# kennychenfs/KataCoffee

Hardware: AMD Instinct MI355X
Metric: self-play training rows/sec + MCTS playouts/sec, 5x5 Coffee b6c96 @600 visits (higher is better)
Workload: dtype fp16

## Files before the change

### include/katacoffee.h

```cpp
#ifndef KATACOFFEE_H
#define KATACOFFEE_H

#include <stdint.h>

#ifdef __cplusplus
extern "C" {
#endif

#define COFFEE_OK 0
#define COFFEE_EINVAL (-1)
#define COFFEE_EHIP (-2)
#define COFFEE_EIO (-3)
#define COFFEE_EINTERNAL (-4)

#define COFFEE_NUM_SPATIAL 15
#define COFFEE_NUM_GLOBAL_TARGETS 64

const char* coffee_last_error(void);
int coffee_abi_version(void);

int coffee_device_count(int* count);
int coffee_set_device(int device);
int coffee_device_compute_units(int device, int* cus);
int coffee_malloc(void** dev_ptr, uint64_t bytes);
int coffee_free(void* dev_ptr);
int coffee_memcpy(void* dst, const void* src, uint64_t bytes, int kind);
int coffee_synchronize(void);


int coffee_rules_batch(int x, int y, int win_len, int n, const uint8_t* cells, const int8_t* last_cell,
                       const int8_t* last_dir, const uint8_t* pla, uint8_t* legal, uint8_t* has_legal, void* stream);

int coffee_play_batch(int x, int y, int win_len, int n, const uint8_t* cells, const int8_t* last_cell,
                      const int8_t* last_dir, const uint8_t* pla, const int32_t* move, uint8_t* out_cells,
                      uint8_t* finished, uint8_t* winner, int32_t* max_run, uint64_t* pos_hash,
                      uint64_t* state_hash, void* stream);


int coffee_encode_batch(int x, int y, int win_len, int n, const uint8_t* cells, const int8_t* hist_cell,
                        const int8_t* hist_dir, const uint8_t* pla, const int32_t* sym, uint64_t* packed,
                        float* planes, void* stream);


typedef struct coffee_nn coffee_nn;

int coffee_model_write_random(const char* arch, uint64_t seed, const char* path );
int coffee_model_flops(const char* path, int area, double* flops);

int coffee_nn_create(const char* model_path, int x, int y, int win_len, coffee_nn** out);
#define COFFEE_NN_DEFAULT 0
#define COFFEE_NN_ACCURATE 1
#define COFFEE_NN_FAST_LAYERED 2
#define COFFEE_NN_CORRECTED 3
#define COFFEE_NN_ACCURATE_NB2 4
#define COFFEE_NN_FAST 5
int coffee_nn_create2(const char* model_path, int x, int y, int win_len, int precision, coffee_nn** out);
int coffee_nn_is_fused(coffee_nn* h, int* fused);
int coffee_nn_precision(coffee_nn* h, int* precision, float* calib_err);
int coffee_nn_forward(coffee_nn* h, int n, const uint64_t* in, float* out, void* stream);
int coffee_nn_forward2(coffee_nn* h, int n, const uint64_t* in, const int32_t* sym, float* out, void* stream);
int coffee_nn_destroy(coffee_nn* h);

int coffee_fake_net(int x, int y, int win_len, int n, const uint64_t* in, float* out, void* stream);


typedef struct coffee_search_params {
  int32_t max_visits;
  float cpuct_exploration, cpuct_exploration_log, cpuct_exploration_base;
  float fpu_reduction_max, root_fpu_reduction_max, fpu_loss_prop, root_fpu_loss_prop;
  int32_t fpu_parent_weight_by_visited_policy;
  float fpu_parent_weight_by_visited_policy_pow;
  float value_weight_exponent;
  int32_t root_noise_enabled;
  float root_dirichlet_noise_total_concentration, root_dirichlet_noise_weight;
  float root_policy_temperature, root_policy_temperature_early;
  float root_desired_per_child_visits_coeff;
  int32_t root_num_symmetries_to_sample;
  float chosen_move_temperature, chosen_move_temperature_early, chosen_move_temperature_halflife;
  float chosen_move_subtract, chosen_move_prune;
  int32_t use_lcb_for_selection;
  float lcb_stdevs, min_visit_prop_for_lcb;
  float subtree_value_bias_factor, subtree_value_bias_weight_exponent, subtree_value_bias_free_prop;
  int32_t use_graph_search;
  float cheap_search_prob;
  int32_t cheap_search_visits;
  float cheap_search_target_weight;
  int32_t reduce_visits;
  float reduce_visits_threshold;
  int32_t reduce_visits_threshold_lookback;
  int32_t reduced_visits_min;
  float reduced_visits_weight;
  float policy_surprise_data_weight;
  float value_surprise_data_weight;
  int32_t init_games_with_policy;
  float policy_init_area_prop;
  float policy_init_area_temperature;
  float early_fork_game_prob;
  float early_fork_game_expected_move_prop;
  float fork_game_prob;
  int32_t fork_game_min_choices;
  int32_t early_fork_game_max_choices;
  int32_t fork_game_max_choices;
  float side_position_prob;
  int32_t record_tree_positions;
  int32_t record_tree_threshold;
  float record_tree_target_weight;
} coffee_search_params;

void coffee_search_params_default(coffee_search_params* p);

typedef struct coffee_selfplay_config {
  int32_t x, y, win_len;
  int32_t num_games;
  int32_t node_cap;
  int32_t row_capacity;
  uint64_t seed;
  int32_t slot_base;
  int32_t use_fake_net;
  int32_t commit_interval;
  const char* model_path;
  coffee_search_params search;
  int32_t nn_cache_log2;
  int32_t nn_batch_cap;
  int32_t nn_precision;
  int32_t start_stagger;
  int32_t engines_per_device;
} coffee_selfplay_config;

typedef struct coffee_selfplay coffee_selfplay;

typedef struct coffee_selfplay_stats {
  uint64_t rounds;
  uint64_t playouts;
  uint64_t nn_evals;
  uint64_t moves;
  uint64_t games_finished;
  uint64_t rows_written;
  uint64_t rows_pending;
  uint64_t rows_dropped;
  uint64_t games_dropped;
  uint64_t errors;
  uint64_t tree_levels;
  uint64_t tree_children;
  uint64_t errors_node_pool;
  uint64_t errors_edge_pool;
  uint64_t edge_pool_peak;
  uint64_t edge_pool_cap;
  uint64_t nn_precision;
  uint64_t nn_audits;
  uint64_t nn_audit_switches;
  double nn_audit_max_diff;
} coffee_selfplay_stats;

int coffee_selfplay_create(const coffee_selfplay_config* cfg, coffee_selfplay** out);
int coffee_selfplay_step(coffee_selfplay* h, int rounds, void* stream);
int coffee_selfplay_sync(coffee_selfplay* h);
int coffee_selfplay_stats_get(coffee_selfplay* h, coffee_selfplay_stats* out);

int coffee_selfplay_drain_rows(coffee_selfplay* h, int max_rows, uint8_t* bin, float* glob, int16_t* pol,
                               float* gtgt, int8_t* value, int32_t* meta, int* n_out);
int coffee_selfplay_drain_games(coffee_selfplay* h, int max_games, int32_t* header, uint8_t* moves, int* n_out);
#define COFFEE_STAGE_DISCARD_GAMES 1
int coffee_selfplay_stage_rows(coffee_selfplay* h, void* dst, int max_rows, uint64_t* count, int flags);
int coffee_selfplay_row_capacity(coffee_selfplay* h, int* rows);
int coffee_row_bytes(int x, int y, int* bytes);
int coffee_selfplay_stream(coffee_selfplay* h, void** stream);
int coffee_selfplay_set_model(coffee_selfplay* h, const char* model_path);
int coffee_selfplay_set_model_bytes(coffee_selfplay* h, const void* data, uint64_t bytes);
int coffee_selfplay_destroy(coffee_selfplay* h);

int coffee_write_npz(const char* path, int n, int x, int y, const uint8_t* bin, const float* glob,
                     const int16_t* pol, const float* gtgt, const int8_t* value);

int coffee_selfplay_game_info(coffee_selfplay* h, int slot, int64_t* info);
int coffee_selfplay_game_tree(coffee_selfplay* h, int slot, int max_nodes, uint32_t* nodes, uint32_t* edges,
                              int* n_nodes);
int coffee_selfplay_root_policy(coffee_selfplay* h, int slot, float* out);

int coffee_debug_cdf_table(int x, int y, int win_len, float* out );
int coffee_debug_zobrist(int x, int y, int win_len, uint64_t* board, uint64_t* board2, uint64_t* player,
                         uint64_t* init, uint64_t* game_over);

int coffee_selfplay_enable_timing(coffee_selfplay* h, int enable);
int coffee_selfplay_kernel_time(coffee_selfplay* h, int which, double* ms, uint64_t* launches);
int coffee_selfplay_timed_nn_evals(coffee_selfplay* h, uint64_t* evals);

#ifdef __cplusplus
}
#endif

#endif
```

### katacoffee_amd/__init__.py

```python
import ctypes
import os
import subprocess

import numpy as np

HERE = os.path.dirname(os.path.abspath(__file__))
LIB_PATH = os.path.join(HERE, "libkatacoffee.so")
CSRC = os.path.join(HERE, "csrc")

NUM_SPATIAL = 15
COFFEE_OK = 0
PRECISIONS = {"default": 0, "accurate": 1, "fast-layered": 2, "corrected": 3, "accurate-nb2": 4, "fast": 5}
PRECISION_NAMES = {v: k for k, v in PRECISIONS.items()}

_lib = None

c_p = ctypes.c_void_p
c_i = ctypes.c_int
c_u64 = ctypes.c_uint64


class CoffeeError(RuntimeError):
    pass


class SearchParams(ctypes.Structure):
    _fields_ = [
        ("max_visits", ctypes.c_int32),
        ("cpuct_exploration", ctypes.c_float), ("cpuct_exploration_log", ctypes.c_float),
        ("cpuct_exploration_base", ctypes.c_float),
        ("fpu_reduction_max", ctypes.c_float), ("root_fpu_reduction_max", ctypes.c_float),
        ("fpu_loss_prop", ctypes.c_float), ("root_fpu_loss_prop", ctypes.c_float),
        ("fpu_parent_weight_by_visited_policy", ctypes.c_int32),
        ("fpu_parent_weight_by_visited_policy_pow", ctypes.c_float),
        ("value_weight_exponent", ctypes.c_float),
        ("root_noise_enabled", ctypes.c_int32),
        ("root_dirichlet_noise_total_concentration", ctypes.c_float),
        ("root_dirichlet_noise_weight", ctypes.c_float),
        ("root_policy_temperature", ctypes.c_float), ("root_policy_temperature_early", ctypes.c_float),
        ("root_desired_per_child_visits_coeff", ctypes.c_float),
        ("root_num_symmetries_to_sample", ctypes.c_int32),
        ("chosen_move_temperature", ctypes.c_float), ("chosen_move_temperature_early", ctypes.c_float),
        ("chosen_move_temperature_halflife", ctypes.c_float),
        ("chosen_move_subtract", ctypes.c_float), ("chosen_move_prune", ctypes.c_float),
        ("use_lcb_for_selection", ctypes.c_int32),
        ("lcb_stdevs", ctypes.c_float), ("min_visit_prop_for_lcb", ctypes.c_float),
        ("subtree_value_bias_factor", ctypes.c_float), ("subtree_value_bias_weight_exponent", ctypes.c_float),
        ("subtree_value_bias_free_prop", ctypes.c_float),
        ("use_graph_search", ctypes.c_int32),
        ("cheap_search_prob", ctypes.c_float), ("cheap_search_visits", ctypes.c_int32),
        ("cheap_search_target_weight", ctypes.c_float), ("reduce_visits", ctypes.c_int32),
        ("reduce_visits_threshold", ctypes.c_float), ("reduce_visits_threshold_lookback", ctypes.c_int32),
        ("reduced_visits_min", ctypes.c_int32), ("reduced_visits_weight", ctypes.c_float),
        ("policy_surprise_data_weight", ctypes.c_float), ("value_surprise_data_weight", ctypes.c_float),
        ("init_games_with_policy", ctypes.c_int32), ("policy_init_area_prop", ctypes.c_float),
        ("policy_init_area_temperature", ctypes.c_float),
        ("early_fork_game_prob", ctypes.c_float), ("early_fork_game_expected_move_prop", ctypes.c_float),
        ("fork_game_prob", ctypes.c_float), ("fork_game_min_choices", ctypes.c_int32),
        ("early_fork_game_max_choices", ctypes.c_int32), ("fork_game_max_choices", ctypes.c_int32),
        ("side_position_prob", ctypes.c_float),
        ("record_tree_positions", ctypes.c_int32), ("record_tree_threshold", ctypes.c_int32),
        ("record_tree_target_weight", ctypes.c_float),
    ]


class SelfplayConfig(ctypes.Structure):
    _fields_ = [
        ("x", ctypes.c_int32), ("y", ctypes.c_int32), ("win_len", ctypes.c_int32),
        ("num_games", ctypes.c_int32), ("node_cap", ctypes.c_int32), ("row_capacity", ctypes.c_int32),
        ("seed", ctypes.c_uint64), ("slot_base", ctypes.c_int32), ("use_fake_net", ctypes.c_int32),
        ("commit_interval", ctypes.c_int32),
        ("model_path", ctypes.c_char_p),
        ("search", SearchParams),
        ("nn_cache_log2", ctypes.c_int32),
        ("nn_batch_cap", ctypes.c_int32),
        ("nn_precision", ctypes.c_int32),
        ("start_stagger", ctypes.c_int32),
        ("engines_per_device", ctypes.c_int32),
    ]


class SelfplayStats(ctypes.Structure):
    _fields_ = [(n, ctypes.c_uint64) for n in
                ["rounds", "playouts", "nn_evals", "moves", "games_finished", "rows_written", "rows_pending",
                 "rows_dropped", "games_dropped", "errors", "tree_levels", "tree_children", "errors_node_pool",
                 "errors_edge_pool", "edge_pool_peak", "edge_pool_cap", "nn_precision", "nn_audits",
                 "nn_audit_switches"]] + [("nn_audit_max_diff", ctypes.c_double)]


EXPORTS = [
    "coffee_last_error", "coffee_abi_version", "coffee_device_count", "coffee_set_device", "coffee_device_compute_units", "coffee_malloc",
    "coffee_free", "coffee_memcpy", "coffee_synchronize", "coffee_rules_batch", "coffee_play_batch",
    "coffee_encode_batch", "coffee_model_write_random", "coffee_model_flops", "coffee_nn_create",
    "coffee_nn_forward", "coffee_nn_forward2", "coffee_nn_destroy", "coffee_nn_create2", "coffee_nn_is_fused", "coffee_nn_precision", "coffee_fake_net", "coffee_search_params_default",
    "coffee_selfplay_create", "coffee_selfplay_step", "coffee_selfplay_sync", "coffee_selfplay_stats_get",
    "coffee_selfplay_drain_rows", "coffee_selfplay_drain_games", "coffee_selfplay_set_model",
    "coffee_selfplay_stage_rows", "coffee_selfplay_row_capacity", "coffee_row_bytes", "coffee_selfplay_stream",
    "coffee_selfplay_set_model_bytes",
    "coffee_selfplay_destroy", "coffee_selfplay_game_info",
    "coffee_selfplay_game_tree", "coffee_selfplay_root_policy", "coffee_debug_cdf_table", "coffee_debug_zobrist",
    "coffee_selfplay_enable_timing", "coffee_selfplay_kernel_time", "coffee_selfplay_timed_nn_evals",
    "coffee_write_npz",
]


def build(jobs=8):
    subprocess.run(["make", "-s", "-j%d" % jobs, "-C", CSRC], check=True)


def lib():
    global _lib
    if _lib is None:
        if not os.path.exists(LIB_PATH):
            raise CoffeeError("libkatacoffee.so not built (run katacoffee_amd.build()); no CPU fallback exists")
        try:
            import torch
        except ImportError:
            pass
        L = ctypes.CDLL(os.environ.get("KATACOFFEE_LIB", LIB_PATH))
        L.coffee_last_error.restype = ctypes.c_char_p
        L.coffee_model_write_random.argtypes = [ctypes.c_char_p, c_u64, ctypes.c_char_p]
        L.coffee_model_flops.argtypes = [ctypes.c_char_p, c_i, c_p]
        L.coffee_nn_create.argtypes = [ctypes.c_char_p, c_i, c_i, c_i, c_p]
        L.coffee_nn_create2.argtypes = [ctypes.c_char_p, c_i, c_i, c_i, c_i, c_p]
        L.coffee_nn_is_fused.argtypes = [c_p, c_p]
        if hasattr(L, "coffee_nn_precision"):
            L.coffee_nn_precision.argtypes = [c_p, c_p, c_p]
        L.coffee_nn_forward.argtypes = [c_p, c_i, c_p, c_p, c_p]
        L.coffee_nn_forward2.argtypes = [c_p, c_i, c_p, c_p, c_p, c_p]
        L.coffee_nn_destroy.argtypes = [c_p]
        L.coffee_fake_net.argtypes = [c_i, c_i, c_i, c_i, c_p, c_p, c_p]
        L.coffee_rules_batch.argtypes = [c_i, c_i, c_i, c_i] + [c_p] * 7
        L.coffee_play_batch.argtypes = [c_i, c_i, c_i, c_i] + [c_p] * 12
        L.coffee_encode_batch.argtypes = [c_i, c_i, c_i, c_i] + [c_p] * 8
        L.coffee_search_params_default.argtypes = [c_p]
        L.coffee_search_params_default.restype = None
        L.coffee_selfplay_create.argtypes = [c_p, c_p]
        L.coffee_selfplay_step.argtypes = [c_p, c_i, c_p]
        L.coffee_selfplay_sync.argtypes = [c_p]
        L.coffee_selfplay_stats_get.argtypes = [c_p, c_p]
        L.coffee_selfplay_drain_rows.argtypes = [c_p, c_i] + [c_p] * 7
        L.coffee_selfplay_drain_games.argtypes = [c_p, c_i, c_p, c_p, c_p]
        L.coffee_selfplay_stage_rows.argtypes = [c_p, c_p, c_i, c_p, c_i]
        L.coffee_selfplay_row_capacity.argtypes = [c_p, c_p]
        L.coffee_row_bytes.argtypes = [c_i, c_i, c_p]
        L.coffee_selfplay_stream.argtypes = [c_p, c_p]
        L.coffee_selfplay_set_model.argtypes = [c_p, ctypes.c_char_p]
        L.coffee_selfplay_set_model_bytes.argtypes = [c_p, c_p, c_u64]
        L.coffee_selfplay_destroy.argtypes = [c_p]
        L.coffee_selfplay_game_info.argtypes = [c_p, c_i, c_p]
        L.coffee_selfplay_game_tree.argtypes = [c_p, c_i, c_i, c_p, c_p, c_p]
        L.coffee_selfplay_root_policy.argtypes = [c_p, c_i, c_p]
        L.coffee_selfplay_enable_timing.argtypes = [c_p, c_i]
        L.coffee_selfplay_kernel_time.argtypes = [c_p, c_i, c_p, c_p]
        L.coffee_selfplay_timed_nn_evals.argtypes = [c_p, c_p]
        L.coffee_debug_cdf_table.argtypes = [c_i, c_i, c_i, c_p]
        L.coffee_debug_zobrist.argtypes = [c_i, c_i, c_i] + [c_p] * 5
        L.coffee_write_npz.argtypes = [ctypes.c_char_p, c_i, c_i, c_i] + [c_p] * 5
        _lib = L
    return _lib


def check(rc):
    if rc != COFFEE_OK:
        msg = lib().coffee_last_error()
        raise CoffeeError("libkatacoffee error %d: %s" % (rc, msg.decode() if msg else ""))


def _ptr(a):
    return ctypes.c_void_p(a.ctypes.data)


def default_search_params(**over):
    p = SearchParams()
    lib().coffee_search_params_default(ctypes.byref(p))
    for k, v in over.items():
        setattr(p, k, v)
    return p



def _torch_cuda():
    import torch
    if not torch.cuda.is_available():
        raise CoffeeError("no GPU visible: the HIP path is the only implementation")
    return torch


def _dev(torch, a, dtype=None):
    a = np.ascontiguousarray(a if dtype is None else np.asarray(a, dtype=dtype))
    return torch.from_numpy(a).to("cuda")


def _dp(t):
    return ctypes.c_void_p(t.data_ptr())


def _sync(torch):
    torch.cuda.synchronize()


def rules_batch(X, Y, W, cells, last_cell, last_dir, pla):
    torch = _torch_cuda()
    n = len(pla)
    A = X * Y
    dc, dl, dd, dp_ = (_dev(torch, cells, np.uint8), _dev(torch, last_cell, np.int8), _dev(torch, last_dir, np.int8),
                       _dev(torch, pla, np.uint8))
    legal = torch.zeros((n, 4 * A), dtype=torch.uint8, device="cuda")
    has = torch.zeros(n, dtype=torch.uint8, device="cuda")
    _sync(torch)
    check(lib().coffee_rules_batch(X, Y, W, n, _dp(dc), _dp(dl), _dp(dd), _dp(dp_), _dp(legal), _dp(has), None))
    _sync(torch)
    return legal.cpu().numpy(), has.cpu().numpy()


def play_batch(X, Y, W, cells, last_cell, last_dir, pla, move):
    torch = _torch_cuda()
    n = len(pla)
    A = X * Y
    ins = [_dev(torch, cells, np.uint8), _dev(torch, last_cell, np.int8), _dev(torch, last_dir, np.int8),
           _dev(torch, pla, np.uint8), _dev(torch, move, np.int32)]
    out_cells = torch.zeros((n, A), dtype=torch.uint8, device="cuda")
    fin = torch.zeros(n, dtype=torch.uint8, device="cuda")
    win = torch.zeros(n, dtype=torch.uint8, device="cuda")
    mr = torch.zeros(n, dtype=torch.int32, device="cuda")
    ph = torch.zeros((n, 2), dtype=torch.int64, device="cuda")
    sh = torch.zeros((n, 2), dtype=torch.int64, device="cuda")
    _sync(torch)
    check(lib().coffee_play_batch(X, Y, W, n, *[_dp(t) for t in ins], _dp(out_cells), _dp(fin), _dp(win), _dp(mr),
                                  _dp(ph), _dp(sh), None))
    _sync(torch)
    u = lambda t: t.cpu().numpy().view(np.uint64)
    return (out_cells.cpu().numpy(), fin.cpu().numpy(), win.cpu().numpy(), mr.cpu().numpy(), u(ph), u(sh))


def encode_batch(X, Y, W, cells, hist_cell, hist_dir, pla, sym, want_planes=True):
    torch = _torch_cuda()
    n = len(pla)
    A = X * Y
    words = (NUM_SPATIAL * A + 63) // 64
    ins = [_dev(torch, cells, np.uint8), _dev(torch, hist_cell, np.int8), _dev(torch, hist_dir, np.int8),
           _dev(torch, pla, np.uint8), _dev(torch, sym, np.int32)]
    packed = torch.zeros((n, words), dtype=torch.int64, device="cuda")
    planes = torch.zeros((n, NUM_SPATIAL, A), dtype=torch.float32, device="cuda") if want_planes else None
    _sync(torch)
    check(lib().coffee_encode_batch(X, Y, W, n, *[_dp(t) for t in ins], _dp(packed),
                                    _dp(planes) if planes is not None else None, None))
    _sync(torch)
    pk = packed.cpu().numpy().view(np.uint64)
    return pk, (planes.cpu().numpy() if planes is not None else None)


def write_random_model(arch, seed, path):
    check(lib().coffee_model_write_random(arch.encode(), seed, path.encode()))


def model_flops(path, area):
    f = ctypes.c_double()
    check(lib().coffee_model_flops(path.encode(), area, ctypes.byref(f)))
    return f.value


class Network:

    def __init__(self, model_path, X, Y, W, precision="default"):
        self.X, self.Y, self.W = X, Y, W
        self.h = ctypes.c_void_p()
        check(lib().coffee_nn_create2(model_path.encode(), X, Y, W, PRECISIONS[precision], ctypes.byref(self.h)))

    @property
    def fused(self):
        f = ctypes.c_int()
        check(lib().coffee_nn_is_fused(self.h, ctypes.byref(f)))
        return bool(f.value)

    @property
    def precision(self):
        p, e = ctypes.c_int(), ctypes.c_float()
        check(lib().coffee_nn_precision(self.h, ctypes.byref(p), ctypes.byref(e)))
        return PRECISION_NAMES[p.value], float(e.value)

    def forward_device(self, n, packed_dev, out_dev, stream=None):
        check(lib().coffee_nn_forward(self.h, n, _dp(packed_dev), _dp(out_dev), stream))

    def forward(self, packed):
        torch = _torch_cuda()
        n = packed.shape[0]
        P = 4 * self.X * self.Y
        din = _dev(torch, np.ascontiguousarray(packed).view(np.int64))
        out = torch.zeros((n, P + 4), dtype=torch.float32, device="cuda")
        _sync(torch)
        self.forward_device(n, din, out)
        _sync(torch)
        return out.cpu().numpy()

    def forward_canonical(self, packed, sym):
        torch = _torch_cuda()
        n = packed.shape[0]
        P = 4 * self.X * self.Y
        din = _dev(torch, np.ascontiguousarray(packed).view(np.int64))
        dsym = _dev(torch, sym, np.int32)
        out = torch.zeros((n, P + 4), dtype=torch.float32, device="cuda")
        _sync(torch)
        check(lib().coffee_nn_forward2(self.h, n, _dp(din), _dp(dsym), _dp(out), None))
        _sync(torch)
        return out.cpu().numpy()

    def close(self):
        if self.h:
            lib().coffee_nn_destroy(self.h)
            self.h = ctypes.c_void_p()

    def __del__(self):
        try:
            self.close()
        except Exception:
            pass


def fake_net(X, Y, W, packed):
    torch = _torch_cuda()
    n = packed.shape[0]
    P = 4 * X * Y
    din = _dev(torch, np.ascontiguousarray(packed).view(np.int64))
    out = torch.zeros((n, P + 4), dtype=torch.float32, device="cuda")
    _sync(torch)
    check(lib().coffee_fake_net(X, Y, W, n, _dp(din), _dp(out), None))
    _sync(torch)
    return out.cpu().numpy()


def cdf_table(X=5, Y=5, W=4):
    out = np.zeros(2000, np.float32)
    check(lib().coffee_debug_cdf_table(X, Y, W, _ptr(out)))
    return out


def row_bytes(X, Y):
    b = ctypes.c_int()
    check(lib().coffee_row_bytes(X, Y, ctypes.byref(b)))
    return b.value


def write_npz(path, rows, X, Y):
    n = len(rows["globalInputNC"])
    arrs = [np.ascontiguousarray(rows[k], dtype=t) for k, t in
            [("binaryInputNCHWPacked", np.uint8), ("globalInputNC", np.float32), ("policyTargetsNCMove", np.int16),
             ("globalTargetsNC", np.float32), ("valueTargetsNCHW", np.int8)]]
    check(lib().coffee_write_npz(path.encode(), n, X, Y, *[_ptr(a) for a in arrs]))


def zobrist_tables(X, Y, W):
    A = X * Y
    out = dict(board=np.zeros((A, 3, 2), np.uint64), board2=np.zeros((A, 4, 2), np.uint64),
               player=np.zeros((3, 2), np.uint64), init=np.zeros(2, np.uint64), game_over=np.zeros(2, np.uint64))
    check(lib().coffee_debug_zobrist(X, Y, W, *[_ptr(out[k]) for k in ["board", "board2", "player", "init",
                                                                          "game_over"]]))
    return out


class Selfplay:

    def __init__(self, X=5, Y=5, W=4, num_games=4096, max_visits=600, seed=1, slot_base=0, model_path=None,
                 node_cap=0, row_capacity=0, commit_interval=0, nn_cache_log2=0, nn_batch_cap=0, nn_precision="default",
                 start_stagger=0, engines_per_device=0, **search_over):
        _torch_cuda()
        self.X, self.Y, self.W = X, Y, W
        self.A, self.P = X * Y, 4 * X * Y
        self.num_games = num_games
        cfg = SelfplayConfig()
        cfg.x, cfg.y, cfg.win_len = X, Y, W
        cfg.num_games = num_games
        cfg.node_cap = node_cap
        cfg.row_capacity = row_capacity
        cfg.seed = seed
        cfg.slot_base = slot_base
        cfg.use_fake_net = 1 if model_path is None else 0
        cfg.commit_interval = commit_interval
        cfg.nn_cache_log2 = nn_cache_log2
        cfg.nn_batch_cap = nn_batch_cap
        cfg.nn_precision = PRECISIONS[nn_precision]
        cfg.start_stagger = start_stagger
        cfg.engines_per_device = engines_per_device
        self._model = model_path.encode() if model_path else None
        cfg.model_path = self._model
        cfg.search = default_search_params(max_visits=max_visits, **search_over)
        self.cfg = cfg
        self.h = ctypes.c_void_p()
        check(lib().coffee_selfplay_create(ctypes.byref(cfg), ctypes.byref(self.h)))

    def step(self, rounds, stream=None):
        check(lib().coffee_selfplay_step(self.h, rounds, stream))

    def sync(self):
        check(lib().coffee_selfplay_sync(self.h))

    def stats(self):
        s = SelfplayStats()
        check(lib().coffee_selfplay_stats_get(self.h, ctypes.byref(s)))
        return {k: getattr(s, k) for k, _ in SelfplayStats._fields_}

    def drain_rows(self, max_rows=1 << 30):
        st = self.stats()
        n = min(max_rows, st["rows_pending"])
        A, P, pb = self.A, self.P, (self.A + 7) // 8
        rows = {
            "binaryInputNCHWPacked": np.zeros((n, NUM_SPATIAL, pb), np.uint8),
            "globalInputNC": np.zeros((n, 1), np.float32),
            "policyTargetsNCMove": np.zeros((n, 2, P), np.int16),
            "globalTargetsNC": np.zeros((n, 64), np.float32),
            "valueTargetsNCHW": np.zeros((n, 5, self.Y, self.X), np.int8),
            "meta": np.zeros((n, 4), np.int32),
        }
        got = ctypes.c_int()
        order = ["binaryInputNCHWPacked", "globalInputNC", "policyTargetsNCMove", "globalTargetsNC",
                 "valueTargetsNCHW", "meta"]
        check(lib().coffee_selfplay_drain_rows(self.h, n, *[_ptr(rows[k]) for k in order], ctypes.byref(got)))
        assert got.value == n
        return rows

    def row_capacity(self):
        n = ctypes.c_int()
        check(lib().coffee_selfplay_row_capacity(self.h, ctypes.byref(n)))
        return n.value

    def stream_ptr(self):
        p = ctypes.c_void_p()
        check(lib().coffee_selfplay_stream(self.h, ctypes.byref(p)))
        return p.value

    def stage_rows(self, dst, count, discard_games=True):
        assert dst.is_cuda and dst.dtype.itemsize == 1 and dst.is_contiguous()
        assert dst.dim() == 2 and dst.shape[1] == row_bytes(self.X, self.Y), \
            "dst must be [rows][row_bytes(X, Y)] uint8, got %s" % (tuple(dst.shape),)
        import torch
        assert dst.device.index == torch.cuda.current_device(), "dst must be on the engine's (current) device"
        assert count.is_pinned() and count.dtype.itemsize == 8
        check(lib().coffee_selfplay_stage_rows(self.h, ctypes.c_void_p(dst.data_ptr()), dst.shape[0],
                                               ctypes.c_void_p(count.data_ptr()), 1 if discard_games else 0))

    def drain_games(self, max_games=1 << 20):
        cap = min(max_games, 2 * self.num_games)
        header = np.zeros((cap, 4), np.int32)
        moves = np.zeros((cap, self.A, 2), np.uint8)
        got = ctypes.c_int()
        check(lib().coffee_selfplay_drain_games(self.h, cap, _ptr(header), _ptr(moves), ctypes.byref(got)))
        return header[:got.value], moves[:got.value]

    def set_model(self, model_path):
        self._model = model_path.encode()
        check(lib().coffee_selfplay_set_model(self.h, self._model))

    def set_model_bytes(self, data):
        buf = np.frombuffer(bytes(data), dtype=np.uint8)
        check(lib().coffee_selfplay_set_model_bytes(self.h, _ptr(buf), buf.size))

    def game_info(self, slot):
        info = np.zeros(16, np.int64)
        check(lib().coffee_selfplay_game_info(self.h, slot, _ptr(info)))
        keys = ["phase", "rootK", "liveCount", "rootIdx", "gameNum", "turn", "pla", "finished", "winner",
                "playouts", "nnEvals", "moves", "gamesFinished", "lastCell", "lastDir", "rngCtr"]
        return dict(zip(keys, info.tolist()))

    def game_tree(self, slot, max_nodes=4096):
        nodes = np.zeros((max_nodes, 24), np.uint32)
        edges = np.zeros((max_nodes, self.P, 3), np.uint32)
        n = ctypes.c_int()
        check(lib().coffee_selfplay_game_tree(self.h, slot, max_nodes, _ptr(nodes), _ptr(edges), ctypes.byref(n)))
        return nodes[:n.value], edges[:n.value]

    def root_policy(self, slot):
        out = np.zeros(self.P, np.float32)
        check(lib().coffee_selfplay_root_policy(self.h, slot, _ptr(out)))
        return out

    def enable_timing(self, every=1):
        check(lib().coffee_selfplay_enable_timing(self.h, int(every)))

    def timed_nn_evals(self):
        n = ctypes.c_uint64()
        check(lib().coffee_selfplay_timed_nn_evals(self.h, ctypes.byref(n)))
        return n.value

    def kernel_time(self, which):
        ms = ctypes.c_double()
        n = ctypes.c_uint64()
        check(lib().coffee_selfplay_kernel_time(self.h, which, ctypes.byref(ms), ctypes.byref(n)))
        return ms.value, n.value

    def close(self):
        if self.h:
            lib().coffee_selfplay_destroy(self.h)
            self.h = ctypes.c_void_p()

    def __del__(self):
        try:
            self.close()
        except Exception:
            pass
```

### katacoffee_amd/csrc/capi.cpp

```cpp
#include <cstring>
#include <map>
#include <mutex>
#include <string>
#include <tuple>

#include "../../include/katacoffee.h"
#include "engine.h"
#include "model.h"
#include "npzwrite.h"
#include "selfplay.h"

namespace kc {

namespace {
std::mutex gTablesMu;
std::map<std::tuple<int, int, int, int>, std::pair<DTables*, DTables*>> gTables;
}

static std::pair<DTables*, DTables*> tablesFor(int X, int Y, int W) {
  int dev = 0;
  KC_HIP(hipGetDevice(&dev));
  std::lock_guard<std::mutex> lk(gTablesMu);
  auto key = std::make_tuple(dev, X, Y, W);
  auto it = gTables.find(key);
// ... 163 lines not shown
    ModelHost m = loadModel(model_path);
    (void)deviceTables(x, y, win_len);
    coffee_nn* h = new coffee_nn{nullptr, x, y, win_len};
    try {
      h->eng = new NNEngine(m, x, y, win_len, precision);
    } catch(...) {
      delete h;
      throw;
    }
    *out = h;
  });
}

int coffee_nn_forward(coffee_nn* h, int n, const uint64_t* in, float* out, void* stream) {
  return guarded([&] {
    need(h && h->eng, "NULL handle");
    need(n >= 0, "n must be >= 0");
    need(n == 0 || (in && out), "NULL buffer");
    h->eng->forward(n, in, out, (hipStream_t)stream);
  });
}

int coffee_nn_forward2(coffee_nn* h, int n, const uint64_t* in, const int32_t* sym, float* out, void* stream) {
  return guarded([&] {
    need(h && h->eng, "NULL handle");
    need(n >= 0, "n must be >= 0");
    need(n == 0 || (in && sym && out), "NULL buffer");
    h->eng->forward(n, in, out, (hipStream_t)stream);
    launchCanonicalRows(deviceTables(h->x, h->y, h->w), n, sym, out, (hipStream_t)stream);
  });
}

int coffee_nn_is_fused(coffee_nn* h, int* fused) {
  return guarded([&] {
    need(h && h->eng && fused, "NULL argument");
    *fused = h->eng->fused() ? 1 : 0;
  });
}

int coffee_nn_precision(coffee_nn* h, int* precision, float* calib_err) {
  return guarded([&] {
    need(h && h->eng && precision, "NULL argument");
    *precision = h->eng->precision();
    if(calib_err)
      *calib_err = h->eng->calibrationError();
  });
}

int coffee_nn_destroy(coffee_nn* h) {
  return guarded([&] {
    if(h) {
      delete h->eng;
      delete h;
    }
  });
}

int coffee_fake_net(int x, int y, int win_len, int n, const uint64_t* in, float* out, void* stream) {
  return guarded([&] {
    checkGeom(x, y, win_len);
    need(n >= 0, "n must be >= 0");
    need(n == 0 || (in && out), "NULL buffer");
    launchFakeNet(deviceTables(x, y, win_len), n, in, out, (hipStream_t)stream);
  });
}

void coffee_search_params_default(coffee_search_params* p) {
  if(!p)
    return;
  p->max_visits = 600;
  p->cpuct_exploration = 1.1f;
  p->cpuct_exploration_log = 0.0f;
  p->cpuct_exploration_base = 500.0f;
  p->fpu_reduction_max = 0.2f;
  p->root_fpu_reduction_max = 0.0f;
  p->fpu_loss_prop = 0.0f;
  p->root_fpu_loss_prop = 0.0f;
  p->fpu_parent_weight_by_visited_policy = 1;
  p->fpu_parent_weight_by_visited_policy_pow = 2.0f;
  p->value_weight_exponent = 0.5f;
  p->root_noise_enabled = 1;
  p->root_dirichlet_noise_total_concentration = 10.83f;
  p->root_dirichlet_noise_weight = 0.25f;
  p->root_policy_temperature = 1.1f;
  p->root_policy_temperature_early = 1.25f;
  p->root_desired_per_child_visits_coeff = 2.0f;
  p->root_num_symmetries_to_sample = 4;
  p->chosen_move_temperature = 0.15f;
  p->chosen_move_temperature_early = 0.75f;
  p->chosen_move_temperature_halflife = 19.0f;
  p->chosen_move_subtract = 0.0f;
  p->chosen_move_prune = 1.0f;
  p->use_lcb_for_selection = 1;
  p->lcb_stdevs = 5.0f;
  p->min_visit_prop_for_lcb = 0.15f;
  p->subtree_value_bias_factor = 0.30f;
  p->subtree_value_bias_weight_exponent = 0.8f;
  p->subtree_value_bias_free_prop = 0.8f;
  p->use_graph_search = 1;
  p->cheap_search_prob = 0.0f;
  p->cheap_search_visits = 100;
  p->cheap_search_target_weight = 0.0f;
  p->reduce_visits = 0;
  p->reduce_visits_threshold = 0.9f;
  p->reduce_visits_threshold_lookback = 3;
  p->reduced_visits_min = 100;
  p->reduced_visits_weight = 0.1f;
  p->policy_surprise_data_weight = 0.0f;
  p->value_surprise_data_weight = 0.0f;
  p->init_games_with_policy = 0;
  p->policy_init_area_prop = 0.04f;
  p->policy_init_area_temperature = 1.0f;
  p->early_fork_game_prob = 0.0f;
  p->early_fork_game_expected_move_prop = 0.025f;
  p->fork_game_prob = 0.0f;
  p->fork_game_min_choices = 3;
  p->early_fork_game_max_choices = 12;
  p->fork_game_max_choices = 36;
  p->side_position_prob = 0.0f;
  p->record_tree_positions = 0;
  p->record_tree_threshold = 0;
  p->record_tree_target_weight = 0.0f;
}

struct coffee_selfplay {
  SelfplayEngine* eng;
};

int coffee_selfplay_create(const coffee_selfplay_config* cfg, coffee_selfplay** out) {
  return guarded([&] {
    need(cfg && out, "NULL argument");
    checkGeom(cfg->x, cfg->y, cfg->win_len);
    coffee_selfplay* h = new coffee_selfplay{nullptr};
    try {
      h->eng = new SelfplayEngine(*cfg);
    } catch(...) {
      delete h;
      throw;
    }
    *out = h;
  });
}

int coffee_selfplay_step(coffee_selfplay* h, int rounds, void* stream) {
  return guarded([&] {
    need(h && h->eng, "NULL handle");
    need(rounds >= 0, "rounds must be >= 0");
    h->eng->step(rounds, (hipStream_t)stream);
  });
}

int coffee_selfplay_sync(coffee_selfplay* h) {
  return guarded([&] {
    need(h && h->eng, "NULL handle");
    h->eng->sync();
  });
}

int coffee_selfplay_stats_get(coffee_selfplay* h, coffee_selfplay_stats* out) {
  return guarded([&] {
    need(h && h->eng && out, "NULL argument");
    h->eng->stats(*out);
  });
}

int coffee_selfplay_drain_rows(coffee_selfplay* h, int max_rows, uint8_t* bin, float* glob, int16_t* pol,
                               float* gtgt, int8_t* value, int32_t* meta, int* n_out) {
  return guarded([&] {
    need(h && h->eng && n_out, "NULL argument");
    *n_out = h->eng->drain(max_rows, bin, glob, pol, gtgt, value, meta);
  });
}

int coffee_row_bytes(int x, int y, int* bytes) {
  return guarded([&] {
    need(bytes != nullptr, "NULL argument");
    need(x >= 2 && y >= 2 && x <= MAX_LEN && y <= MAX_LEN, "bad shape");
    *bytes = rowBytes(x * y);
  });
}

int coffee_selfplay_row_capacity(coffee_selfplay* h, int* rows) {
  return guarded([&] {
    need(h && h->eng && rows, "NULL argument");
    *rows = h->eng->dev().rowCap;
  });
}

int coffee_selfplay_stream(coffee_selfplay* h, void** stream) {
  return guarded([&] {
    need(h && h->eng && stream, "NULL argument");
    *stream = (void*)h->eng->stream();
  });
}

int coffee_selfplay_stage_rows(coffee_selfplay* h, void* dst, int max_rows, uint64_t* count, int flags) {
  return guarded([&] {
    need(h && h->eng && dst && count, "NULL argument");
    need((flags & ~COFFEE_STAGE_DISCARD_GAMES) == 0, "unknown flags");
    h->eng->stageRows((uint8_t*)dst, max_rows, (unsigned long long*)count, (flags & COFFEE_STAGE_DISCARD_GAMES) != 0);
  });
}

int coffee_selfplay_drain_games(coffee_selfplay* h, int max_games, int32_t* header, uint8_t* moves, int* n_out) {
  return guarded([&] {
    need(h && h->eng && n_out, "NULL argument");
    need(max_games >= 0, "max_games must be >= 0");
    *n_out = h->eng->drainGames(max_games, header, moves);
  });
}

int coffee_selfplay_set_model(coffee_selfplay* h, const char* model_path) {
  return guarded([&] {
    need(h && h->eng && model_path, "NULL argument");
    h->eng->setModel(model_path);
  });
}

int coffee_selfplay_set_model_bytes(coffee_selfplay* h, const void* data, uint64_t bytes) {
  return guarded([&] {
    need(h && h->eng && data, "NULL argument");
    h->eng->setModelBytes(data, (size_t)bytes);
  });
}

int coffee_selfplay_destroy(coffee_selfplay* h) {
  return guarded([&] {
    if(h) {
      delete h->eng;
      delete h;
    }
  });
}

int coffee_write_npz(const char* path, int n, int x, int y, const uint8_t* bin, const float* glob,
                     const int16_t* pol, const float* gtgt, const int8_t* value) {
  return guarded([&] {
    need(path != nullptr, "NULL path");
    need(n >= 0 && x >= 2 && y >= 2 && x <= MAX_LEN && y <= MAX_LEN, "bad shape");
    writeNpz(path, n, x, y, bin, glob, pol, gtgt, value);
  });
}

int coffee_selfplay_game_info(coffee_selfplay* h, int slot, int64_t* info) {
  return guarded([&] {
    need(h && h->eng && info, "NULL argument");
    h->eng->gameInfo(slot, info);
  });
}

int coffee_selfplay_game_tree(coffee_selfplay* h, int slot, int max_nodes, uint32_t* nodes, uint32_t* edges,
                              int* n_nodes) {
  return guarded([&] {
    need(h && h->eng && n_nodes, "NULL argument");
    *n_nodes = h->eng->gameTree(slot, max_nodes, nodes, edges);
  });
}

int coffee_selfplay_root_policy(coffee_selfplay* h, int slot, float* out) {
  return guarded([&] {
    need(h && h->eng && out, "NULL argument");
    h->eng->rootPolicy(slot, out);
  });
}

int coffee_debug_cdf_table(int x, int y, int win_len, float* out) {
  return guarded([&] {
    need(out != nullptr, "NULL argument");
    checkGeom(x, y, win_len);
    DTables t = buildTables(x, y, win_len);
    memcpy(out, t.cdf, sizeof(float) * CDF_SIZE);
  });
}

int coffee_debug_zobrist(int x, int y, int win_len, uint64_t* board, uint64_t* board2, uint64_t* player,
                         uint64_t* init, uint64_t* game_over) {
  return guarded([&] {
    need(board && board2 && player && init && game_over, "NULL argument");
    checkGeom(x, y, win_len);
    DTables t = buildTables(x, y, win_len);
    memcpy(board, t.zBoard, sizeof(uint64_t) * t.A * 3 * 2);
    memcpy(board2, t.zBoard2, sizeof(uint64_t) * t.A * 4 * 2);
    memcpy(player, t.zPlayer, sizeof(t.zPlayer));
    memcpy(init, t.zInit, sizeof(t.zInit));
    memcpy(game_over, t.zGameOver, sizeof(t.zGameOver));
  });
}

int coffee_selfplay_enable_timing(coffee_selfplay* h, int enable) {
  return guarded([&] {
    need(h && h->eng, "NULL handle");
    need(enable >= 0, "enable must be >= 0");
    h->eng->setTiming(enable);
  });
}

int coffee_selfplay_timed_nn_evals(coffee_selfplay* h, uint64_t* evals) {
  return guarded([&] {
    need(h && h->eng && evals, "NULL argument");
    *evals = h->eng->timedNNEvals();
  });
}

int coffee_selfplay_kernel_time(coffee_selfplay* h, int which, double* ms, uint64_t* launches) {
  return guarded([&] {
    need(h && h->eng && ms && launches, "NULL argument");
    h->eng->kernelTime(which, *ms, *launches);
  });
}

}
```

### katacoffee_amd/csrc/search.h

```cpp
#pragma once
#include "kc_common.h"

namespace kc {

constexpr int MAX_DEPTH = MAX_AREA + 2;
constexpr int INLINE_EDGES = 16;
KC_HD int edgeBlockCap(int k, int P) {
  return (P > 64 && k <= 64) ? 64 - INLINE_EDGES : P - INLINE_EDGES;
}
inline int edgePoolCapFor(int cap, int P) {
  const double perEdge = (32.0 + P) / 65.0 > 48.0 / 17.0 ? (32.0 + P) / 65.0 : 48.0 / 17.0;
  return (int)(perEdge * 1.5 * cap) + 2 * P;
}
enum { ERR_NODE_POOL = 1, ERR_NO_CANDIDATE = 2, ERR_EDGE_POOL = 3 };
constexpr int MAX_LANE_ITEMS = (MAX_P + 63) / 64;

enum LeafKind {
  LEAF_NONE = 0,
  LEAF_NN = 1,
  LEAF_TERMINAL = 2,
  LEAF_CATCHUP = 3,
  LEAF_NOCHILD = 4,
  LEAF_ROOTEVAL = 5,
  LEAF_CACHED = 6,
  LEAF_INIT = 7,
  LEAF_FORK = 8,
  LEAF_SIDE = 9,
  LEAF_PENDING = 10
};

KC_HD uint32_t cacheSlot(uint64_t k0, uint64_t k1, uint32_t mask) {
  const uint64_t h = k0 ^ ((k1 << 29) | (k1 >> 35));
  return (uint32_t)(h ^ (h >> 32)) & mask;
}
enum Phase { PH_ROOTEVAL = 0, PH_SEARCH = 1, PH_COMMIT = 2, PH_INIT = 3, PH_FORK = 4, PH_SIDEEVAL = 5 };

struct SP {
  int maxVisits;
  float cpuct, cpuctLog, cpuctBase;
  float fpuRedMax, rootFpuRedMax, fpuLossProp, rootFpuLossProp;
  int fpuByVisited;
  float fpuByVisitedPow;
  float valueWeightExp;
  int rootNoise;
  float dirConc, dirWeight;
  float rootTemp, rootTempEarly;
  float rootDesiredCoeff;
  int rootSyms;
  float moveTemp, moveTempEarly, moveTempHalflife;
  float moveSubtract, movePrune;
  int useLcb;
  float lcbStdevs, minVisitPropLcb;
  float svbFactor, svbExp, svbFreeProp;
  int useGraph;
  float cheapProb;
  int cheapVisits;
  float cheapWeight;
  int reduceVisits;
  float reduceThreshold;
  int reduceLookback, reducedMin;
  float reducedWeight;
  float policySurpriseWeight, valueSurpriseWeight;
  int initPolicy;
  float initAreaProp, initTemp;
  float earlyForkProb, earlyForkMoveProp, forkProb;
  int forkMinChoices, earlyForkMaxChoices, forkMaxChoices;
  float sideProb;
  int recordTree, recordTreeThreshold;
  float recordTreeWeight;
};

inline SP cheapSearchSP(const SP& p) {
  SP c = p;
  c.rootNoise = 0;
  c.rootTemp = 1.0f;
  c.rootTempEarly = 1.0f;
  c.rootFpuLossProp = p.fpuLossProp;
  c.rootFpuRedMax = p.fpuRedMax;
  c.rootDesiredCoeff = 0.0f;
  c.rootSyms = 1;
  return c;
}

struct Node {
  uint32_t visits;
  float weightSum, weightSqSum, utilityAvg, utilitySqAvg, winLossAvg;
  float nnWin, nnLoss;
  float lastSvbDelta, lastSvbWeight;
  int32_t svbEntry;
  uint16_t numChildren;
  uint8_t nextPla;
  uint8_t flags;
  float nextPrior;
  uint16_t nextPos;
  uint16_t pad0;
  uint32_t edgeBase;
  uint32_t pad1;
};
static_assert(sizeof(Node) == 64, "Node layout");

struct Edge {
  uint32_t child, visits;
  float prior;
  uint32_t move;
};

struct GameRec {
  int32_t slot, gameNum, numMoves, winner;
  uint8_t cell[MAX_AREA], dir[MAX_AREA];
};

struct TurnRec {
  float whiteWin, whiteLoss, rawWhiteWL, rawPolicyEntropy;
  float policySurprise, policyEntropy, searchEntropy;
  uint32_t visits;
  float rootWL;
  float rootNNWin, rootNNLoss;
  float targetWeight;
  int8_t cell, dir;
  uint8_t rows;
  uint8_t gen;
  int8_t pad[4];
};
static_assert(sizeof(TurnRec) == 56, "TurnRec layout");

constexpr int MAX_SIDE = 8;

constexpr int MAX_FORK_CHOICES = 100;
struct ForkRec {
  DBoard board;
  int32_t numChoices, next, best, prefix;
  float bestWinrate;
  int32_t pad;
  uint16_t moves[MAX_FORK_CHOICES];
};

struct FinRec {
  uint64_t rngSeed, rngCtr;
  uint64_t gameHash0, gameHash1;
  unsigned long long rowBase;
  int32_t numMoves, winner, gameNum, pending;
  int32_t numRows, startTurn;
  int32_t gameMode;
  int32_t genStart, genEnd;
  int32_t pad;
};

struct GameDev {
  DBoard root;
  DBoard leaf;
  uint64_t rngSeed, rngCtr;
  uint64_t gameHash0, gameHash1;
  uint64_t playouts, nnEvals, moves, gamesFinished;
  uint64_t treeLevels, treeChildren;
  int32_t phase, rootK;
  uint32_t syms;
  int32_t cSlot;
  float cHitWin, cHitLoss;
  int32_t noNoise;
  int32_t visitLimit;
  float moveWeight;
  int32_t initLeft;
  int32_t startTurn;
  int32_t gameMode;
  int32_t sideCount, sideNext;
  int32_t sideMode;
  int32_t startDelay;
  int32_t startGen;
  int32_t leafKind, leafNode, leafSym, nnSlot;
  int32_t rootIdx, liveCount, freeTop, pathLen;
  int32_t gameNum, numTurns, svbSel, err;
  int32_t edgeSel, edgeTop;
  int32_t edgePeak, pad0;
  float accWin, accLoss, rawWin, rawLoss;
};

template <class T>
KC_HD T* asGlobal(T* p) {
#if defined(__HIP_DEVICE_COMPILE__)
  __attribute__((address_space(1))) T* q = (__attribute__((address_space(1))) T*)p;
  asm volatile("" : "+s"(q));
  return (T*)q;
#else
  return p;
#endif
}
template <class T>
struct DPtr {
  T* p;
  DPtr() = default;
  KC_HD DPtr(T* q) : p(q) {}
  KC_HD operator T*() const { return asGlobal(p); }
  KC_HD T* operator->() const { return asGlobal(p); }
};

struct SearchDev {
  DPtr<const DTables> T;
  SP sp;
  SP spCheap;
  int G, cap, ttCap, svbCap, P, A, inWords, maxTurns;
  int rowCap, slotBase;
  int startStagger;
  DPtr<int32_t> modelGen;
  uint64_t seed;
  DPtr<GameDev> games;
  DPtr<Node> nodes;
  DPtr<Edge> edges;
  DPtr<Edge> edgePool;
  int edgePoolCap;
  DPtr<uint64_t> nodeKey;
  DPtr<float> policy;
  DPtr<uint32_t> freeList;
  DPtr<uint32_t> allocBits;
  DPtr<uint64_t> ttKey;
  DPtr<int32_t> ttNode;
  DPtr<uint64_t> svbKey;
  DPtr<int64_t> svbD;
  DPtr<int64_t> svbW;
  DPtr<float> accPolicy;
  DPtr<float> rawPolicy;
  DPtr<float> rootNoised;
  DPtr<int32_t> pathNode;
  DPtr<int32_t> pathSlot;
  DPtr<TurnRec> turns;
  DPtr<int16_t> turnPol;
  DPtr<uint64_t> nnIn;
  DPtr<float> nnOut;
  DPtr<int32_t> nnNeed;
  DPtr<int32_t> nnIdx;
  DPtr<int32_t> nnCount;
  DPtr<int32_t> nnDefer;
  DPtr<uint32_t> nnBid;
  int nnCap;
  DPtr<int32_t> nnRR;
  DPtr<unsigned long long> nnTimedEvals;
  uint32_t cacheMask;
  int32_t cacheOn;
  DPtr<uint64_t> cKey;
  DPtr<float> cPol;
  DPtr<float> cVal;
  DPtr<uint32_t> cTag;
  DPtr<uint32_t> cClear;
  DPtr<int32_t> pendList;
  DPtr<int32_t> pendCount;
  DPtr<FinRec> fin;
  DPtr<ForkRec> fork;
  DPtr<DBoard> side;
  DPtr<int16_t> sidePol;
  DPtr<int32_t> commitList;
  DPtr<int32_t> commitCount;
  DPtr<uint8_t> rBin;
  DPtr<float> rGlob;
  DPtr<int16_t> rPol;
  DPtr<float> rGt;
  DPtr<int8_t> rVal;
  DPtr<int32_t> rMeta;
  DPtr<unsigned long long> rCount;
  DPtr<unsigned long long> rDropped;
  DPtr<unsigned long long> rStaged;
  int gCap;
  DPtr<GameRec> gRec;
  DPtr<unsigned long long> gCount;
  DPtr<unsigned long long> gDropped;
};

void launchSelfplayInit(const SearchDev& d, const SearchDev* dd, hipStream_t st);
void launchSelect(const SearchDev& d, const SearchDev* dd, hipStream_t st, hipEvent_t e0 = nullptr,
                  hipEvent_t e1 = nullptr, bool resetCommit = false);
void launchCompact(const SearchDev& d, const SearchDev* dd, hipStream_t st, bool accumulate, bool resolve = false);
void launchStageRows(const SearchDev& d, const SearchDev* dd, uint8_t* dst, unsigned long long* countOut,
                     bool discardGames, hipStream_t st);
int rowBytes(int A);
void launchBackup(const SearchDev& d, const SearchDev* dd, hipStream_t st, hipEvent_t e0 = nullptr,
                  hipEvent_t e1 = nullptr);
void launchBackupSelect(const SearchDev& d, const SearchDev* dd, hipStream_t st, hipEvent_t e0 = nullptr,
                        hipEvent_t e1 = nullptr);
void launchResolve(const SearchDev& d, const SearchDev* dd, hipStream_t st);
void launchCommit(const SearchDev& d, const SearchDev* dd, hipStream_t st);
void launchGameTree(const SearchDev* dd, int slot, int maxNodes, uint32_t* nodesOut, uint32_t* edgesOut,
                    int32_t* count, hipStream_t st);
size_t commitLdsBytes(int cap);

}
```

### katacoffee_amd/csrc/search.hip

```cpp
#include <hip/hip_runtime.h>
#include <hip/hip_ext.h>

#include "detmath.h"
#include "engine.h"
#include "kc_board.h"
#include "search.h"

namespace kc {

static constexpr int SVB_IDX_MOVE1 = MAX_P + 1;
static constexpr int SVB_IDX_PLA = 2 * (MAX_P + 1);
static constexpr int SVB_IDX_PAT = 2 * (MAX_P + 1) + 3;
static constexpr int BIG = 0x7fffffff;

KC_D int64_t svbQ(float x) { return llrintf(x * 4294967296.0f); }
KC_D float svbF(int64_t v) { return (float)v * (1.0f / 4294967296.0f); }

KC_D void waveSync() {
  __builtin_amdgcn_wave_barrier();
  asm volatile("" ::: "memory");
}

#ifdef KC_SEARCH_PROFILE
constexpr int SPROF_N = 32;
// ... 697 lines not shown
    int si = v.lane;
    waveArgmax(sv, si);
    const int sc = sv >= 0.0f ? bcastLane((int)e0.child, si) : -1;
    *specChild = sc;
    if(sc >= 0) {
      *specE0 = v.lane < SPEC_EDGES && v.lane < v.d.P ? v.inlineEdges(sc)[v.lane] : Edge{0u, 0u, 0.0f, 0u};
      *specN = NS[sc];
    }
  }
  const float probMass = tsum<NI>(probs, k, v.lane);
  const float total = tsum<NI>(cw, k, v.lane);
  const float fpu = fpuValue(sp, n, pla, isRoot, probMass);
  const float scaling = exploreScaling(sp, total);
  float best = -__builtin_inff();
  int bestIdx = BIG;
#pragma unroll
  for(int j = 0; j < NI; j++) {
    int i = v.lane + 64 * j;
    if((j > 0 && 64 * j >= k) || i >= k)
      continue;
    float p = pv[j];
    float val;
    if(p < 0.0f)
      val = -__builtin_inff();
    else {
      float w = cw[j];
      float u = (cvis[j] == 0 || w <= 0.0f) ? fpu : cu[j];
      if(isRoot && sp.rootDesiredCoeff > 0.0f && p > 0.0f && w < sqrtf((p * total) * sp.rootDesiredCoeff))
        val = 1e20f;
      else
        val = (scaling * p) / (1.0f + w) + (pla == 2 ? u : -u);
    }
    if(val > best) {
      best = val;
      bestIdx = i;
    }
  }
  waveArgmax(best, bestIdx);
  int bestSlot = best > -__builtin_inff() ? bestIdx : -1;
  if(bestSlot >= 0) {
    Edge me{0u, 0u, 0.0f, 0u};
    uint32_t mv = 0, mf = 0;
#pragma unroll
    for(int j = 0; j < NI; j++)
      if(j == (bestSlot >> 6)) {
        me = ev[j];
        mv = cvis[j];
        mf = cfl[j];
      }
    const int bl = bestSlot & 63;
    ce.child = (uint32_t)bcastLane((int)me.child, bl);
    ce.visits = (uint32_t)bcastLane((int)me.visits, bl);
    ce.move = (uint32_t)bcastLane((int)me.move, bl);
    ce.prior = 0.0f;
    cVisits = (uint32_t)bcastLane((int)mv, bl);
    cFlags = (uint32_t)bcastLane((int)mf, bl);
  }
  float bp = -1.0f;
  int bpos = BIG;
  if(isRoot) {
    waveSync();
    for(int pos = v.lane; pos < P; pos += 64) {
      if((hasBits[pos >> 5] >> (pos & 31)) & 1u)
        continue;
      float p = pol[pos];
      if(p < 0.0f)
        continue;
      if(p > bp) {
        bp = p;
        bpos = pos;
      }
    }
    waveArgmax(bp, bpos);
  } else if(n.nextPos != 0xFFFF) {
    bp = n.nextPrior;
    bpos = n.nextPos;
  }
  newPos = -1;
  if(bpos != BIG) {
    float val = (scaling * bp) / 1.0f + (pla == 2 ? fpu : -fpu);
    if(val > best) {
      bestSlot = k;
      newPos = bpos;
    }
  }
  return bestSlot;
}

template <int NI>
KC_D void nextExpansion(const GV& v, const float (&pv)[NI], float curPrior, int curPos, float& nPrior, int& nPos) {
  const int P = v.d.P;
  float best = -1.0f;
  int bi = BIG;
#pragma unroll
  for(int j = 0; j < NI; j++) {
    const int p = v.lane + 64 * j;
    const float x = pv[j];
    if(p < P && x >= 0.0f && (x < curPrior || (x == curPrior && p > curPos)) && x > best) {
      best = x;
      bi = p;
    }
  }
  waveArgmax(best, bi);
  nPrior = bi != BIG ? best : -1.0f;
  nPos = bi != BIG ? bi : 0xFFFF;
}

#ifndef KC_TT_EARLY
#define KC_TT_EARLY 0
#endif
template <int NI>
KC_D void descend(const GV& v, GameDev& s, uint32_t* hasBits, float* rootPol ) {
  const SP& sp = *v.sp;
  const DTables& T = v.T;
  s.pathLen = 0;
  DBoard b = s.root;
  int ni = s.rootIdx;
  uint32_t scanned = 0;
  auto loadE0 = [&](int node) {
    return v.lane < SPEC_EDGES && v.lane < v.d.P ? v.inlineEdges(node)[v.lane] : Edge{0u, 0u, 0.0f, 0u};
  };
  Edge e0 = loadE0(ni);
  Node n = v.nodes()[ni];
  const int freeIdx = s.freeTop > 0 ? (int)v.freeList()[s.freeTop - 1] : -1;
  {
    const float* rn = v.rootNoised();
    float pr[NI];
#pragma unroll
    for(int j = 0; j < NI; j++) {
      const int p = v.lane + 64 * j;
      pr[j] = p < v.d.P ? rn[p] : 0.0f;
    }
#pragma unroll
    for(int j = 0; j < NI; j++) {
      const int p = v.lane + 64 * j;
      if(p < v.d.P)
        rootPol[p] = pr[j];
    }
    waveSync();
  }
  while(true) {
    if(n.flags & 2) {
      s.leafKind = LEAF_TERMINAL;
      s.leafNode = ni;
      s.leaf = b;
      break;
    }
    const bool isRoot = ni == s.rootIdx;
    const float* pol = isRoot ? rootPol : v.pol(ni);
    int newPos = -1;
    scanned += n.numChildren;
    const unsigned long long tSel = SPROF_NOW();
    Edge ce{0u, 0u, 0.0f, 0u};
    uint32_t cVisits = 0, cFlags = 0;
    int specChild = -1;
    Edge specE0{0u, 0u, 0.0f, 0u};
    Node specN;
    int slot = KC_SPEC_NEXT ? selectBest<NI>(v, ni, n, pol, isRoot, newPos, hasBits, e0, ce, cVisits, cFlags, &specChild,
                                             &specE0, &specN)
                            : selectBest<NI>(v, ni, n, pol, isRoot, newPos, hasBits, e0, ce, cVisits, cFlags);
    SPROF_ADD(5, SPROF_NOW() - tSel);
    (void)tSel;
    if(slot < 0) {
      s.leafKind = LEAF_NOCHILD;
      s.leafNode = ni;
      break;
    }
    if(slot == n.numChildren) {
      const unsigned long long tExp = SPROF_NOW();
      (void)tExp;
      float pvn[NI];
      float rootPrior = 0.0f;
      {
        const float* pp = v.pol(ni);
#pragma unroll
        for(int j = 0; j < NI; j++) {
          const int p = v.lane + 64 * j;
          pvn[j] = !isRoot && p < v.d.P ? pp[p] : -1.0f;
        }
        if(isRoot)
          rootPrior = pp[newPos];
      }
      uint32_t ebase = n.edgeBase;
      int reserved = 0;
      if(slot == INLINE_EDGES || (slot == 64 && v.d.P > 64)) {
        const int need = edgeBlockCap(slot + 1, v.d.P);
        if(s.edgeTop + need > v.d.edgePoolCap) {
          s.err = ERR_EDGE_POOL;
          s.leafKind = LEAF_NOCHILD;
          s.leafNode = ni;
          break;
        }
        const uint32_t nb = (uint32_t)s.edgeTop;
        s.edgeTop += need;
        s.edgePeak = max(s.edgePeak, s.edgeTop);
        reserved = need;
        if(slot > INLINE_EDGES) {
          Edge* pool = v.edgePool();
          for(int i = v.lane; i < slot - INLINE_EDGES; i += 64)
            pool[nb + i] = pool[ebase + i];
        }
        ebase = nb;
      }
      const float prior = isRoot ? rootPrior : n.nextPrior;
      const int cell = newPos % T.A, dir = newPos / T.A;
      const bool svbKeyed = sp.svbFactor != 0.0f && hCell(b, 0) >= 0;
      uint64_t svbKey = 0, svbFirst = 0;
      if(svbKeyed) {
        svbKey = svbKeyOf(v, b, hDir(b, 0) * T.A + hCell(b, 0), newPos, b.pla);
        svbFirst = svbProbe(v, s.svbSel, svbKey);
      }
      playMoveWave(T, b, cell, dir);
      uint64_t k0, k1;
      stateHash(T, b, k0, k1);
      int ttSlot = -1;
      int child = sp.useGraph ? ttFind(v, k0, k1, ttSlot) : -1;
      const bool fresh = child < 0;
      uint32_t tVisits = 0u, tFlags = 0u;
      if(KC_TT_EARLY && !fresh) {
        const Node& cn = v.nodes()[child];
        tVisits = cn.visits;
        tFlags = (uint32_t)cn.flags;
      }
      float nxtPrior = -1.0f;
      int nxtPos = 0xFFFF;
      if(!isRoot)
        nextExpansion<NI>(v, pvn, n.nextPrior, n.nextPos, nxtPrior, nxtPos);
      if(fresh) {
        child = allocNode(v, s, b.pla, k0, k1, b.finished != 0, freeIdx);
        if(child < 0) {
          s.edgeTop -= reserved;
          s.leafKind = LEAF_NOCHILD;
          s.leafNode = ni;
          break;
        }
        if(svbKeyed) {
          int e = svbFindOrInsert(v, s.svbSel, svbKey, svbFirst);
          waveSync();
          if(v.lane == 0)
            v.nodes()[child].svbEntry = e;
        }
        if(sp.useGraph)
          ttInsertAt(v, ttSlot, k0, k1, child);
      }
      waveSync();
      if(v.lane == 0) {
        v.edges(ni, ebase)[slot] = Edge{(uint32_t)child, 0u, prior, (uint32_t)newPos};
        v.nodes()[ni].numChildren = (uint16_t)(slot + 1);
        v.nodes()[ni].edgeBase = ebase;
        if(!isRoot) {
          v.nodes()[ni].nextPos = (uint16_t)nxtPos;
          v.nodes()[ni].nextPrior = nxtPrior;
        }
        v.pathNode()[s.pathLen] = ni;
        v.pathSlot()[s.pathLen] = slot;
      }
      s.pathLen++;
      waveSync();
      SPROF_ADD(6, SPROF_NOW() - tExp);
      const uint32_t cv = fresh ? 0u : (KC_TT_EARLY ? tVisits : v.nodes()[child].visits);
      const uint32_t cf = fresh ? (b.finished ? 2u : 0u) : (KC_TT_EARLY ? tFlags : (uint32_t)v.nodes()[child].flags);
      if(cv > 0) {
        s.leafKind = LEAF_CATCHUP;
        s.leafNode = child;
        break;
      }
      s.leafNode = child;
      s.leaf = b;
      s.leafKind = (cf & 2) ? LEAF_TERMINAL : LEAF_NN;
      break;
    }
    const int child = (int)ce.child;
    if(v.lane == 0) {
      v.pathNode()[s.pathLen] = ni;
      v.pathSlot()[s.pathLen] = slot;
    }
    s.pathLen++;
    if(ce.visits < cVisits) {
      s.leafKind = LEAF_CATCHUP;
      s.leafNode = child;
      break;
    }
    const int mv = (int)ce.move, mover = b.pla;
    applyMove(T, b, mv % T.A, mv / T.A);
    if(cFlags & 2) {
      b.finished = 1;
      b.winner = maxRun(T, b, mv % T.A) >= T.W ? mover : 0;
    }
    ni = child;
    if(KC_SPEC_NEXT && child == specChild) {
      e0 = specE0;
      n = specN;
    } else {
      e0 = loadE0(ni);
      n = v.nodes()[ni];
    }
  }
  s.treeLevels += (uint64_t)s.pathLen;
  s.treeChildren += scanned;
}


template <int NI>
KC_D void cacheLookup(const GV& v, GameDev& s, bool fused) {
  const SearchDev& d = v.d;
  const uint64_t k0 = v.nodeKey(s.leafNode)[0], k1 = v.nodeKey(s.leafNode)[1];
  const uint32_t slot = cacheSlot(k0, k1, d.cacheMask);
  const int P = d.P;
  const float* cp = d.cPol + (size_t)slot * P;
  float pv[NI];
#pragma unroll
  for(int j = 0; j < NI; j++) {
    const int pos = v.lane + 64 * j;
    pv[j] = pos < P ? cp[pos] : 0.0f;
  }
  const float cw = d.cVal[2 * (size_t)slot], cl = d.cVal[2 * (size_t)slot + 1];
  const uint32_t tag = fused ? d.cTag[slot] : 0u;
  s.cSlot = (int32_t)slot;
  if(tag != 0u) {
    s.leafKind = LEAF_PENDING;
    if(v.lane == 0)
      d.pendList[atomicAdd(d.pendCount, 1)] = v.g;
    return;
  }
  if(d.cKey[2 * (size_t)slot] == k0 && d.cKey[2 * (size_t)slot + 1] == k1) {
    s.leafKind = LEAF_CACHED;
    s.cHitWin = cw;
    s.cHitLoss = cl;
    float* pol = v.pol(s.leafNode);
#pragma unroll
    for(int j = 0; j < NI; j++) {
      const int pos = v.lane + 64 * j;
      if(pos < P)
        pol[pos] = pv[j];
    }
  }
}

KC_D void finishSelect(const GV& v, GameDev& s, DRng& rng) {
  const SearchDev& d = v.d;
  const int g = v.g;
  if(s.leafKind == LEAF_NN)
    s.leafSym = (int)rng.below(8);
  s.rngCtr = rng.ctr;
  const bool needNN =
      s.leafKind == LEAF_NN || s.leafKind == LEAF_ROOTEVAL || s.leafKind == LEAF_INIT || s.leafKind == LEAF_FORK ||
      s.leafKind == LEAF_SIDE;
  if(v.lane == 0) {
    d.nnNeed[g] = needNN ? 1 : 0;
    if(needNN)
      d.nnBid[g] = s.leafKind == LEAF_NN && d.cacheOn ? (uint32_t)s.cSlot : ~0u;
  }
  if(needNN) {
    const int slot = g;
    s.nnSlot = slot;
    s.nnEvals++;
    encodePackedWave(v.T, s.leaf, s.leafSym, d.nnIn + (size_t)slot * d.inWords);
  }
  waveSync();
  storeGame(v, s);
}

template <int NI>
KC_D void selectBody(const SearchDev& d, const DTables& T, int g, GameDev& s, bool loaded, bool fused,
                     uint32_t* hasBits, float* rootPol) {
  GV v(d, T, g);
  SPROF_INIT();
  const unsigned long long t0 = SPROF_NOW();
  if(d.nnDefer[g]) {
    if(v.lane == 0)
      d.nnNeed[g] = 1;
    return;
  }
  if(loaded)
    bindGame(v, s);
  else
    loadGame(v, s);
  if(s.phase == PH_COMMIT || s.startDelay > 0) {
    s.leafKind = LEAF_NONE;
    if(loaded) {
      if(s.startDelay > 0)
        s.startDelay = s.startDelay - 1;
      storeGame(v, s);
      if(v.lane == 0)
        d.nnNeed[g] = 0;
      return;
    }
    if(v.lane == 0) {
      d.games[g].leafKind = LEAF_NONE;
      if(s.startDelay > 0)
        d.games[g].startDelay = s.startDelay - 1;
      d.nnNeed[g] = 0;
    }
    return;
  }
  const unsigned long long t1 = SPROF_NOW();
  (void)t0;
  (void)t1;
  DRng rng = DRng{s.rngSeed, s.rngCtr};
  if(s.phase == PH_INIT) {
    s.leafKind = LEAF_INIT;
    s.leafSym = (int)rng.below(8);
    s.leaf = s.root;
  } else if(s.phase == PH_SIDEEVAL) {
    s.leafKind = LEAF_SIDE;
    s.leafSym = (int)rng.below(8);
  } else if(s.phase == PH_FORK) {
    const ForkRec* f = d.fork + g;
    const int mv = f->moves[f->next];
    s.leaf = f->board;
    playMoveWave(v.T, s.leaf, mv % v.T.A, mv / v.T.A);
    s.leafKind = LEAF_FORK;
    s.leafSym = (int)rng.below(8);
  } else if(s.phase == PH_ROOTEVAL) {
    if(s.rootK == 0) {
      uint32_t idx = 0x76543210u;
#pragma unroll
      for(int k = 0; k < 4; k++) {
        int j = k + (int)rng.below((uint32_t)(8 - k));
        uint32_t a = (idx >> (4 * k)) & 15u, b = (idx >> (4 * j)) & 15u;
        idx = (idx & ~(15u << (4 * k)) & ~(15u << (4 * j))) | (b << (4 * k)) | (a << (4 * j));
      }
      s.syms = idx & 0xFFFFu;
    }
    s.leafKind = LEAF_ROOTEVAL;
    s.leafSym = (int)((s.syms >> (4 * s.rootK)) & 15u);
    s.leaf = s.root;
  } else {
    descend<NI>(v, s, hasBits, rootPol);
    if(s.leafKind == LEAF_NN && d.cacheOn)
      cacheLookup<NI>(v, s, fused);
  }
  const unsigned long long t2 = SPROF_NOW();
  (void)t2;
  finishSelect(v, s, rng);
  SPROF_ADD(0, 1);
  SPROF_MAX(24, SPROF_NOW() - t0);
  SPROF_MAX(25, s.pathLen);
  SPROF_ADD(1, SPROF_NOW() - t0);
  SPROF_ADD(2, t1 - t0);
  SPROF_ADD(3, t2 - t1);
  SPROF_ADD(4, s.pathLen);
  SPROF_ADD(7, SPROF_NOW() - t2);
  SPROF_FLUSH();
}

template <int NI>
__global__ void __launch_bounds__(64, NI <= 2 ? 4 : 2) kSelect(const SearchDev* __restrict__ dp, const DTables* __restrict__ Tp,
                                                                int resetCommit) {
  const SearchDev& d = *dp;
  const int g = blockIdx.x;
  if(resetCommit && g == 0 && threadIdx.x == 0)
    *d.commitCount = 0;
  if(g >= d.G)
    return;
  __shared__ uint32_t hasBits[(MAX_P + 31) / 32];
  __shared__ GameDev s;
  __shared__ float rootPol[MAX_P];
  selectBody<NI>(d, *Tp, g, s, false, false, hasBits, rootPol);
}

constexpr int RESOLVE_GRID = 64;
KC_D void clearRoundTags(const SearchDev& d, int first, int stride) {
  for(int i = first; i < d.G; i += stride) {
    const uint32_t cc = d.cClear[i];
    if(cc != 0u) {
      d.cTag[cc - 1u] = 0u;
      d.cClear[i] = 0u;
    }
  }
}
template <int NI>
KC_D void completePending(const SearchDev& d, const DTables& T, int first, int stride, GameDev& s) {
  const int np = *d.pendCount;
  for(int k = first; k < np; k += stride) {
    const int g = __builtin_amdgcn_readfirstlane(d.pendList[k]);
    GV v(d, T, g);
    loadGame(v, s);
    s.leafKind = LEAF_NN;
    cacheLookup<NI>(v, s, false);
    DRng rng = DRng{s.rngSeed, s.rngCtr};
    finishSelect(v, s, rng);
  }
}
template <int NI>
__global__ void __launch_bounds__(64) kResolve(const SearchDev* __restrict__ dp, const DTables* __restrict__ Tp) {
  const SearchDev& d = *dp;
  clearRoundTags(d, blockIdx.x * 64 + laneId(), RESOLVE_GRID * 64);
  __shared__ GameDev s;
  completePending<NI>(d, *Tp, blockIdx.x, RESOLVE_GRID, s);
}

template <int NI>
KC_D void postprocess(const GV& v, const DBoard& b, int sym, const float* out, float* polDst, float& whiteWin,
                      float& whiteLoss, float* stage, float (&pv)[NI]) {
  const DTables& T = v.T;
  const int P = T.P, A = T.A;
  if(T.X != T.Y)
    sym &= 3;
  float raw[NI + 1];
#pragma unroll
  for(int j = 0; j <= NI; j++) {
    const int i = v.lane + 64 * j;
    raw[j] = i < P + 4 ? out[i] : 0.0f;
  }
  int src[NI];
  bool legal[NI];
#pragma unroll
  for(int j = 0; j < NI; j++) {
    const int pos = v.lane + 64 * j;
    legal[j] = false;
    src[j] = 0;
    if(pos < P) {
      const int dd = pos / A, cell = pos % A;
      legal[j] = isLegal(T, b, cell, dd);
      src[j] = T.symDir[sym][dd] * A + T.symCell[sym][cell];
    }
  }
  waveSync();
#pragma unroll
  for(int j = 0; j <= NI; j++) {
    const int i = v.lane + 64 * j;
    if(i < P + 4)
      stage[i] = raw[j];
  }
  waveSync();
  float logit[NI];
  float mx = -1e25f;
  int legalCount = 0;
#pragma unroll
  for(int j = 0; j < NI; j++) {
    const int pos = v.lane + 64 * j;
    logit[j] = -1e30f;
    if(pos < P) {
      logit[j] = legal[j] ? stage[src[j]] : -1e30f;
      mx = logit[j] > mx ? logit[j] : mx;
    }
    legalCount += __popcll(ballot(legal[j]));
  }
  const float wlg = stage[P], llg = stage[P + 1];
  waveSync();
  mx = waveMax(mx);
  float e[NI];
#pragma unroll
  for(int j = 0; j < NI; j++)
    e[j] = dexp(logit[j] - mx);
  const float sum = tsum<NI>(e, P, v.lane);
#pragma unroll
  for(int j = 0; j < NI; j++) {
    int pos = v.lane + 64 * j;
    pv[j] = legal[j] ? (sum <= 0.0f ? 1.0f / (float)legalCount : e[j] / sum) : -1.0f;
    if(pos < P)
      polDst[pos] = pv[j];
  }
  float m = wlg > llg ? wlg : llg;
  float wp = dexp(wlg - m), lp = dexp(llg - m);
  float ps = wp + lp;
  wp = wp / ps;
  lp = lp / ps;
  if(b.pla == 2) {
    whiteWin = wp;
    whiteLoss = lp;
  } else {
    whiteWin = lp;
    whiteLoss = wp;
  }
}

KC_D float interpolateEarly(const DTables& T, int turn, float halflife, float earlyValue, float value) {
  float rawHalflives = (float)turn / halflife;
  float halflives = rawHalflives * (19.0f / sqrtf((float)(T.X * T.Y)));
  return value + (earlyValue - value) * dpow(0.5f, halflives);
}

KC_D float seqSum(float* lds, int n, int lane) {
  waveSync();
  float acc = 0.0f;
  if(lane == 0)
    for(int i = 0; i < n; i++)
      acc = acc + lds[i];
  return bcastLaneF(acc, 0);
}

KC_D void noiseAndTemp(const GV& v, GameDev& s, DRng& rng, const float* raw, float* out, float* scratch) {
  const SP& sp = *v.sp;
  const int P = v.d.P;
  for(int pos = v.lane; pos < P; pos += 64)
    out[pos] = raw[pos];
  waveSync();
  if(sp.rootTemp != 1.0f || sp.rootTempEarly != 1.0f) {
    float t = interpolateEarly(v.T, s.root.turn, sp.moveTempHalflife, sp.rootTempEarly, sp.rootTemp);
    float mx = 0.0f;
    for(int pos = v.lane; pos < P; pos += 64)
      mx = out[pos] > mx ? out[pos] : mx;
    mx = waveMax(mx);
    float logMax = dlog(mx);
    float invTemp = 1.0f / t;
    for(int pos = v.lane; pos < P; pos += 64) {
      float o = out[pos];
      float p = 0.0f;
      if(o > 0.0f) {
        p = dexp((dlog(o) - logMax) * invTemp);
        out[pos] = p;
      }
      scratch[pos] = p;
    }
    float sum = seqSum(scratch, P, v.lane);
    waveSync();
    for(int pos = v.lane; pos < P; pos += 64)
      if(out[pos] >= 0.0f)
        out[pos] = out[pos] / sum;
    waveSync();
  }
  if(sp.rootNoise) {
    int legalCount = 0;
    for(int base = 0; base < P; base += 64) {
      int pos = base + v.lane;
      legalCount += __popcll(ballot(pos < P && out[pos] >= 0.0f));
    }
    float* alpha = scratch;
    float* r = scratch + MAX_P;
    for(int pos = v.lane; pos < P; pos += 64)
      alpha[pos] = out[pos] >= 0.0f ? dlog(fminf(0.01f, out[pos]) + 1e-20f) : 0.0f;
    float logSum = seqSum(alpha, P, v.lane);
    float logMean = logSum / (float)legalCount;
    waveSync();
    for(int pos = v.lane; pos < P; pos += 64)
      alpha[pos] = out[pos] >= 0.0f ? fmaxf(0.0f, alpha[pos] - logMean) : 0.0f;
    float propSum = seqSum(alpha, P, v.lane);
    float uniform = 1.0f / (float)legalCount;
    waveSync();
    for(int pos = v.lane; pos < P; pos += 64)
      if(out[pos] >= 0.0f)
        alpha[pos] = propSum <= 0.0f ? uniform : 0.5f * (alpha[pos] / propSum + uniform);
    const uint64_t base = rng.next();
    for(int pos = v.lane; pos < P; pos += 64) {
      float rv = 0.0f;
      if(out[pos] >= 0.0f) {
        DRng sub{mix64(base ^ ((uint64_t)(pos + 1) * 0x9e3779b97f4a7c15ULL)), 0};
        rv = sub.gamma(alpha[pos] * sp.dirConc);
      }
      r[pos] = rv;
    }
    float rSum = seqSum(r, P, v.lane);
    waveSync();
    float w = sp.dirWeight;
    for(int pos = v.lane; pos < P; pos += 64) {
      float rr = r[pos] / rSum;
      if(out[pos] >= 0.0f)
        out[pos] = rr * w + out[pos] * (1.0f - w);
    }
    waveSync();
  }
}

template <int NI>
KC_D void firstExpansion(const GV& v, int ni, const float (&pv)[NI]) {
  float pr;
  int pos;
  nextExpansion<NI>(v, pv, __builtin_inff(), -1, pr, pos);
  if(v.lane == 0) {
    v.nodes()[ni].nextPos = (uint16_t)pos;
    v.nodes()[ni].nextPrior = pr;
  }
  waveSync();
}

KC_D bool setMoveLimits(const GV& v, GameDev& s, DRng& rng, float lastWL);
KC_D void finishGameRecord(const GV& v, const GameDev& s, DRng& rng, float* scratch);
KC_D void startGame(const GV& v, GameDev& s);
template <int NI>
KC_D void forkEval(const GV& v, GameDev& s, const float* o, float* scratch);
template <int NI>
KC_D void sideEval(const GV& v, GameDev& s, const float* o, float* scratch);

template <int NI>
KC_D bool initMove(const GV& v, GameDev& s, const float* o, float* scratch ) {
  const SP& b = v.d.sp;
  const int P = v.d.P, A = v.T.A;
  float* pol = scratch;
  float w, l;
  float pv[NI];
  postprocess<NI>(v, s.root, s.leafSym, o, pol, w, l, scratch, pv);
  waveSync();
  int* cpos = reinterpret_cast<int*>(scratch + MAX_P);
  float* cval = scratch;
  int n = 0;
  const float invT = 1.0f / b.initTemp;
  for(int base = 0; base < P; base += 64) {
    const int p = base + v.lane;
    const float q = p < P ? pol[p] : -1.0f;
    const bool ok = q > 0.0f;
    const uint64_t m = ballot(ok);
    waveSync();
    if(ok) {
      const int i = n + __popcll(m & ((1ULL << v.lane) - 1ULL));
      cpos[i] = p;
      cval[i] = b.initTemp == 1.0f ? q : dpow(q, invT);
    }
    n += __popcll(m);
    waveSync();
  }
  DRng rng{s.rngSeed, s.rngCtr};
  int idx = 0;
  if(rng.uni() < 0.0002f) {
    idx = (int)rng.below((uint32_t)n);
  } else {
    const float sum = seqSum(cval, n, v.lane);
    const float dd = rng.uni() * sum;
    idx = n - 1;
    if(v.lane == 0) {
      float acc = 0.0f;
      for(int i = 0; i < n; i++) {
        acc = acc + cval[i];
        if(acc > dd) {
          idx = i;
          break;
        }
      }
    }
    idx = bcastI(idx, 0);
  }
  s.rngCtr = rng.ctr;
  const int chosen = cpos[idx];
  waveSync();
  if(v.lane == 0) {
    TurnRec rec;
    memset(&rec, 0, sizeof(rec));
    rec.gen = (uint8_t)*v.d.modelGen;
    rec.cell = (int8_t)(chosen % A);
    rec.dir = (int8_t)(chosen / A);
    v.turns()[s.numTurns] = rec;
  }
  s.numTurns++;
  s.startTurn++;
  s.initLeft--;
  playMoveWave(v.T, s.root, chosen % A, chosen / A);
  waveSync();
  if(s.root.finished)
    return true;
  if(s.initLeft == 0) {
    DRng r2{s.rngSeed, s.rngCtr};
    setMoveLimits(v, s, r2, 0.0f);
    s.rngCtr = r2.ctr;
    s.phase = PH_ROOTEVAL;
    s.rootK = 0;
  }
  return false;
}

template <int NI>
KC_D bool backupBody(const SearchDev& d, const DTables& T, int g, GameDev& s, bool fused, float* scratch) {
  if(d.nnDefer[g])
    return false;
  GV v(d, T, g);
  SPROF_INIT();
  const unsigned long long t0 = SPROF_NOW();
  (void)t0;
  loadGame(v, s);
  if(s.leafKind == LEAF_NONE)
    return true;
  unsigned long long tPost = 0, tLeaf = 0, tPath = 0;
  (void)tPost;
  (void)tLeaf;
  (void)tPath;
  const SP& sp = *v.sp;
  const int P = d.P;
  const float* o = d.nnOut + (size_t)s.nnSlot * (P + 4);
  bool needCommit = false;
  if(s.leafKind == LEAF_INIT) {
    needCommit = initMove<NI>(v, s, o, scratch);
  } else if(s.leafKind == LEAF_FORK) {
    forkEval<NI>(v, s, o, scratch);
  } else if(s.leafKind == LEAF_SIDE) {
    sideEval<NI>(v, s, o, scratch);
  } else if(s.leafKind == LEAF_ROOTEVAL) {
    float* pol = scratch;
    float w, l;
    float pv[NI];
    postprocess<NI>(v, s.root, s.leafSym, o, pol, w, l, scratch, pv);
    waveSync();
    float* acc = v.accPolicy();
    if(s.rootK == 0) {
      for(int p = v.lane; p < P; p += 64) {
        v.rawPolicy()[p] = pol[p];
        acc[p] = 0.0f + pol[p];
      }
      s.rawWin = w;
      s.rawLoss = l;
      s.accWin = 0.0f + w;
      s.accLoss = 0.0f + l;
    } else {
      for(int p = v.lane; p < P; p += 64)
        acc[p] = acc[p] + pol[p];
      s.accWin = s.accWin + w;
      s.accLoss = s.accLoss + l;
    }
    s.rootK++;
    if(s.rootK == sp.rootSyms) {
      const float fl = (float)sp.rootSyms;
      const bool fresh = s.rootIdx < 0;
      if(fresh) {
        uint64_t k0, k1;
        stateHash(v.T, s.root, k0, k1);
        s.rootIdx = allocNode(v, s, s.root.pla, k0, k1, false);
      }
      waveSync();
      float* rp = v.pol(s.rootIdx);
      for(int p = v.lane; p < P; p += 64)
        rp[p] = acc[p] / fl;
      if(v.lane == 0) {
        Node* r = &v.nodes()[s.rootIdx];
        r->nnWin = s.accWin / fl;
        r->nnLoss = s.accLoss / fl;
        r->flags |= 1;
      }
      waveSync();
      if(fresh) {
        const Node& r = v.nodes()[s.rootIdx];
        addLeafValue(v, s, s.rootIdx, r.nnWin - r.nnLoss, false, true);
      }
      DRng rng{s.rngSeed, s.rngCtr};
      noiseAndTemp(v, s, rng, rp, v.rootNoised(), scratch);
      s.rngCtr = rng.ctr;
      s.phase = PH_SEARCH;
      needCommit = v.nodes()[s.rootIdx].visits >= (uint32_t)s.visitLimit;
    }
  } else {
    NStats leafSt{0u, 0.0f, 0.0f, 0.0f, 0.0f, 0.0f};
    bool haveLeaf = false;
    if(s.leafKind == LEAF_NN || s.leafKind == LEAF_CACHED) {
      float w, l;
      float* pol = v.pol(s.leafNode);
      const unsigned long long ta = SPROF_NOW();
      (void)ta;
      float pv[NI];
#ifdef KC_SEARCH_PROFILE
      if(v.lane == 0)
        probeLeafKey(v.nodeKey(s.leafNode)[0], v.nodeKey(s.leafNode)[1]);
#endif
      if(s.leafKind == LEAF_CACHED) {
#pragma unroll
        for(int j = 0; j < NI; j++) {
          const int pos = v.lane + 64 * j;
          pv[j] = pos < P ? pol[pos] : -1.0f;
        }
        w = s.cHitWin;
        l = s.cHitLoss;
      } else {
        postprocess<NI>(v, s.leaf, s.leafSym, o, pol, w, l, scratch, pv);
        if(d.cacheOn) {
          const uint32_t slot = (uint32_t)s.cSlot;
          if(d.cTag[slot] == (uint32_t)g + 1u) {
            float* cp = d.cPol + (size_t)slot * P;
#pragma unroll
            for(int j = 0; j < NI; j++)
              if(v.lane + 64 * j < P)
                cp[v.lane + 64 * j] = pv[j];
            if(v.lane == 0) {
              d.cVal[2 * (size_t)slot] = w;
              d.cVal[2 * (size_t)slot + 1] = l;
              d.cKey[2 * (size_t)slot] = v.nodeKey(s.leafNode)[0];
              d.cKey[2 * (size_t)slot + 1] = v.nodeKey(s.leafNode)[1];
              if(fused)
                d.cClear[g] = slot + 1u;
              else
                d.cTag[slot] = 0;
            }
          }
        }
      }
      firstExpansion<NI>(v, s.leafNode, pv);
      if(v.lane == 0) {
        Node* n = &v.nodes()[s.leafNode];
        n->nnWin = w;
        n->nnLoss = l;
        n->flags |= 1;
      }
      waveSync();
      const unsigned long long tb = SPROF_NOW();
      (void)tb;
      leafSt = addLeafValue(v, s, s.leafNode, w - l, false, true);
      haveLeaf = true;
      tPost = tb - ta;
      tLeaf = SPROF_NOW() - tb;
    } else if(s.leafKind == LEAF_TERMINAL) {
      float val = s.leaf.winner == 2 ? 1.0f : (s.leaf.winner == 1 ? -1.0f : 0.0f);
      leafSt = addLeafValue(v, s, s.leafNode, val, true, false);
      haveLeaf = true;
    } else if(s.leafKind == LEAF_NOCHILD) {
      const Node& n = v.nodes()[s.leafNode];
      leafSt = addLeafValue(v, s, s.leafNode, n.nnWin - n.nnLoss, false, false);
      haveLeaf = true;
    }
    const unsigned long long tp0 = SPROF_NOW();
    (void)tp0;
    backupPath<NI>(v, s, s.pathLen, leafSt, haveLeaf);
    tPath = SPROF_NOW() - tp0;
    s.playouts++;
    needCommit = v.nodes()[s.rootIdx].visits >= (uint32_t)s.visitLimit;
  }
  if(needCommit) {
    s.phase = PH_COMMIT;
    if(v.lane == 0)
      d.commitList[atomicAdd(d.commitCount, 1)] = g;
  }
  s.leafKind = LEAF_NONE;
  waveSync();
  if(!fused)
    storeGame(v, s);
  SPROF_ADD(10, 1);
  SPROF_MAX(26, SPROF_NOW() - t0);
  SPROF_ADD(11, SPROF_NOW() - t0);
  SPROF_ADD(12, tPost);
  SPROF_ADD(13, tPath);
  SPROF_ADD(14, tLeaf);
  SPROF_FLUSH();
  return true;
}

template <int NI>
__global__ void __launch_bounds__(64, NI <= 4 ? 4 : 3) kBackup(const SearchDev* __restrict__ dp, const DTables* __restrict__ Tp) {
  const SearchDev& d = *dp;
  const int g = blockIdx.x;
  if(g >= d.G)
    return;
  __shared__ __attribute__((aligned(16))) float scratch[3 * MAX_P];
  __shared__ GameDev s;
  backupBody<NI>(d, *Tp, g, s, false, scratch);
}

#ifndef KC_FUSED_OCC
#define KC_FUSED_OCC 4
#endif
#ifndef KC_SEARCH_PRIO
#define KC_SEARCH_PRIO 0
#endif
template <int NI>
__global__ void __launch_bounds__(64, NI <= 2 ? KC_FUSED_OCC : 2) kBackupSelect(const SearchDev* __restrict__ dp,
                                                                      const DTables* __restrict__ Tp) {
  const SearchDev& d = *dp;
  const int g = blockIdx.x;
  if(g >= d.G)
    return;
  if constexpr(KC_SEARCH_PRIO > 0)
    __builtin_amdgcn_s_setprio(KC_SEARCH_PRIO);
  __shared__ __attribute__((aligned(16))) float scratch[3 * MAX_P];
  __shared__ uint32_t hasBits[(MAX_P + 31) / 32];
  __shared__ GameDev s;
  const bool loaded = backupBody<NI>(d, *Tp, g, s, true, scratch);
  selectBody<NI>(d, *Tp, g, s, loaded, true, hasBits, scratch);
}

#ifdef KC_SEARCH_PROFILE
}
#include <algorithm>
#include <vector>
namespace kc {
extern "C" void coffee_debug_probe_table(void* keys, unsigned long long cap ) {
  unsigned long long* k = (unsigned long long*)keys;
  unsigned long long m = cap ? cap - 1 : 0;
  KC_HIP(hipMemcpyToSymbol(HIP_SYMBOL(g_probeKeys), &k, sizeof(k)));
  KC_HIP(hipMemcpyToSymbol(HIP_SYMBOL(g_probeMask), &m, sizeof(m)));
}

extern "C" void coffee_debug_search_profile(unsigned long long* out, int reset) {
  std::vector<unsigned long long> all((size_t)SPROF_MAXG * SPROF_N);
  KC_HIP(hipDeviceSynchronize());
  KC_HIP(hipMemcpyFromSymbol(all.data(), HIP_SYMBOL(g_searchProf), all.size() * 8));
  for(int i = 0; i < SPROF_N; i++)
    out[i] = 0;
  for(size_t k = 0; k < all.size(); k++) {
    const int i = (int)(k % SPROF_N);
    if(i < 24)
      out[i] += all[k];
    else if(i <= 26)
      out[i] = std::max(out[i], all[k]);
    if(i == 24)
      out[27] += all[k];
    if(i == 26)
      out[28] += all[k];
  }
  if(reset) {
    std::fill(all.begin(), all.end(), 0ull);
    KC_HIP(hipMemcpyToSymbol(HIP_SYMBOL(g_searchProf), all.data(), all.size() * 8));
  }
}
#endif


KC_D void lcbAndRadius(const SP& sp, int pla, uint32_t cVisits, float cWs, float cWsq, float cU, float cUsq,
                       uint32_t ev, float& lcb, float& radius) {
  radius = 2.0f * 1.0f * sp.lcbStdevs;
  lcb = -radius;
  float ws = childWeight(ev, cVisits, cWs);
  float wsq = childWeight(ev, cVisits, cWsq);
  if(cVisits == 0 || ws <= 0.0f || wsq <= 0.0f)
    return;
  float u = cU, usq = cUsq;
  float ess = (ws * ws) / wsq;
  float priorWeight = ws / ((ess * ess) * ess);
  usq = fmaxf(usq, u * u + 1e-8f);
  usq = (usq * ws + (usq + 1.0f) * priorWeight) / (ws + priorWeight);
  ws = ws + priorWeight;
  wsq = wsq + priorWeight * priorWeight;
  ess = (ws * ws) / wsq;
  float selfU = pla == 2 ? u : -u;
  float variance = usq - u * u;
  float stdev = sqrtf(variance / ess);
  radius = stdev * sp.lcbStdevs;
  lcb = selfU - radius;
}

template <int NI>
KC_D int playSelectionValuesAt(const GV& v, const SP& sp, const GameDev& s, int ri, const float* pol, bool isRoot,
                               float scaleMaxToAtLeast, bool allowDirect, int* posOut, float* vals, bool useLcb) {
  const Node& n = v.nodes()[ri];
  const int k = n.numChildren;
  const int pla = n.nextPla;
  const NodeEdges E = v.edges(ri, n.edgeBase);
  float cw[NI], val[NI];
  uint32_t ev[NI];
  int posv[NI];
  uint32_t cvis[NI];
  float cws[NI], cwsq[NI], cu[NI], cusq[NI];
#pragma unroll
  for(int j = 0; j < NI; j++) {
    int i = v.lane + 64 * j;
    cw[j] = val[j] = 0.0f;
    ev[j] = 0;
    posv[j] = 0;
    cvis[j] = 0;
    cws[j] = cwsq[j] = cu[j] = cusq[j] = 0.0f;
    if(i < k) {
      Edge e = E[i];
      const Node& c = v.nodes()[e.child];
      cvis[j] = c.visits;
      cws[j] = c.weightSum;
      cwsq[j] = c.weightSqSum;
      cu[j] = c.utilityAvg;
      cusq[j] = c.utilitySqAvg;
      ev[j] = e.visits;
      cw[j] = childWeight(e.visits, cvis[j], cws[j]);
      posv[j] = (int)e.move;
      val[j] = cw[j];
    }
  }
  const float total = tsum<NI>(cw, k, v.lane);
  int numChildren = k;
  float maxGood = -1e30f;
  int bestIdx = BIG;
#pragma unroll
  for(int j = 0; j < NI; j++) {
    int i = v.lane + 64 * j;
    if(i >= k)
      continue;
    float evf = (float)ev[j];
    float gdn = val[j] * fmaxf(0.0f, evf - 1.0f) / fmaxf(1.0f, evf) + 2.0f * pol[posv[j]];
    if(gdn > maxGood) {
      maxGood = gdn;
      bestIdx = i;
    }
  }
  waveArgmax(maxGood, bestIdx);
  if(bestIdx == BIG)
    bestIdx = 0;
  const int bestLane = bestIdx & 63, bestJ = bestIdx >> 6;
  float bestWeight = -1e30f;
  if(k > 0) {
    float bw = 0.0f;
#pragma unroll
    for(int j = 0; j < NI; j++)
      if(j == bestJ)
        bw = cw[j];
    bestWeight = bcastLaneF(bw, bestLane);
  }
  if(isRoot && k > 0) {
    const float fpu = fpuValue(sp, n, pla, true, 1.0f);
    const float scaling = exploreScaling(sp, total);
    float bp = 0.0f, bu = 0.0f;
    uint32_t bvis = 0;
#pragma unroll
    for(int j = 0; j < NI; j++)
      if(j == bestJ) {
        bp = pol[posv[j]];
        bu = cu[j];
        bvis = cvis[j];
      }
    bp = bcastLaneF(bp, bestLane);
    bu = bcastLaneF(bu, bestLane);
    bvis = (uint32_t)bcastLane((int)bvis, bestLane);
    const float bw = bestWeight;
    const float buu = (bvis == 0 || bw <= 0.0f) ? fpu : bu;
    const float bestValue = bp < 0.0f ? -__builtin_inff() : (scaling * bp) / (1.0f + bw) + (pla == 2 ? buu : -buu);
#pragma unroll
    for(int j = 0; j < NI; j++) {
      int i = v.lane + 64 * j;
      if(i >= k || i == bestIdx)
        continue;
      float w = cw[j];
      float reduced;
      if(cvis[j] == 0 || w <= 0.0f)
        reduced = 0.0f;
      else {
        float p = pol[posv[j]];
        float wanted;
        if(p < 0.0f)
          wanted = 0.0f;
        else {
          float valueComponent = pla == 2 ? cu[j] : -cu[j];
          float exploreComponent = bestValue - valueComponent;
          float exploreComponentScaling = scaling * p;
          if(exploreComponent <= 0.0f)
            wanted = __builtin_inff();
          else {
            wanted = exploreComponentScaling / exploreComponent - 1.0f;
            if(wanted < 0.0f)
              wanted = 0.0f;
          }
        }
        reduced = w > wanted ? wanted : w;
      }
      val[j] = ceilf(reduced);
    }
  }
  if(useLcb && k > 0) {
    float lcb[NI], rad[NI];
    float bestLcb = -1e10f;
    int bestLcbIdx = BIG;
#pragma unroll
    for(int j = 0; j < NI; j++) {
      int i = v.lane + 64 * j;
      lcb[j] = rad[j] = 0.0f;
      if(i >= k)
        continue;
      lcbAndRadius(sp, pla, cvis[j], cws[j], cwsq[j], cu[j], cusq[j], ev[j], lcb[j], rad[j]);
      float w = val[j];
      if(w > 0.0f && w >= sp.minVisitPropLcb * bestWeight && lcb[j] > bestLcb) {
        bestLcb = lcb[j];
        bestLcbIdx = i;
      }
    }
    waveArgmax(bestLcb, bestLcbIdx);
    if(bestLcbIdx != BIG) {
      float adj = 0.0f;
#pragma unroll
      for(int j = 0; j < NI; j++)
        if(j == (bestLcbIdx >> 6))
          adj = val[j];
      adj = bcastLaneF(adj, bestLcbIdx & 63);
      float lb = adj;
#pragma unroll
      for(int j = 0; j < NI; j++) {
        int i = v.lane + 64 * j;
        if(i >= k || i == bestLcbIdx)
          continue;
        float excess = bestLcb - lcb[j];
        if(excess < 0.0f)
          continue;
        float rf = (rad[j] + excess) / (rad[j] + 0.20f * excess);
        float lbound = (rf * rf) * val[j];
        if(lbound > lb)
          lb = lbound;
      }
      lb = waveMax(lb);
#pragma unroll
      for(int j = 0; j < NI; j++)
        if(v.lane + 64 * j == bestLcbIdx)
          val[j] = lb;
    }
  }
#pragma unroll
  for(int j = 0; j < NI; j++) {
    int i = v.lane + 64 * j;
    if(i < k) {
      posOut[i] = posv[j];
      vals[i] = val[j];
    }
  }
  waveSync();
  if(numChildren == 0) {
    if(!allowDirect || !isRoot)
      return 0;
    const int P = v.d.P;
    for(int base = 0; base < P; base += 64) {
      int p = base + v.lane;
      bool ok = p < P && isLegal(v.T, s.root, p % v.T.A, p / v.T.A) && pol[p] >= 0.0f;
      uint64_t m = ballot(ok);
      if(ok) {
        int idx = numChildren + __popcll(m & ((1ULL << v.lane) - 1ULL));
        posOut[idx] = p;
        vals[idx] = pol[p];
      }
      numChildren += __popcll(m);
    }
    waveSync();
    if(numChildren == 0)
      return 0;
  }
  float mx = 0.0f;
  for(int i = v.lane; i < numChildren; i += 64)
    mx = vals[i] > mx ? vals[i] : mx;
  mx = waveMax(mx);
  if(mx <= 0.0f)
    return 0;
  const float amountToSubtract = fminf(sp.moveSubtract, mx / 64.0f);
  const float amountToPrune = fminf(sp.movePrune, mx / 64.0f);
  const float newMax = mx - amountToSubtract;
  for(int i = v.lane; i < numChildren; i += 64) {
    float x = vals[i];
    if(x < amountToPrune)
      x = 0.0f;
    else {
      x = x - amountToSubtract;
      if(x <= 0.0f)
        x = 0.0f;
    }
    if(newMax < scaleMaxToAtLeast)
      x = x * (scaleMaxToAtLeast / newMax);
    vals[i] = x;
  }
  waveSync();
  return numChildren;
}

template <int NI>
KC_D int playSelectionValues(const GV& v, const SP& sp, const GameDev& s, float scaleMaxToAtLeast, bool allowDirect,
                             int* posOut, float* vals, bool useLcb) {
  return playSelectionValuesAt<NI>(v, sp, s, s.rootIdx, v.rootNoised(), true, scaleMaxToAtLeast, allowDirect, posOut,
                                   vals, useLcb);
}

KC_D int chooseIndex(const GV& v, DRng& rng, const float* vals, int n, float temperature, float* pr) {
  float mx = 0.0f;
  for(int i = v.lane; i < n; i += 64)
    mx = vals[i] > mx ? vals[i] : mx;
  mx = waveMax(mx);
  if(temperature <= 1.0e-4f) {
    float best = -__builtin_inff();
    int bi = BIG;
    for(int i = v.lane; i < n; i += 64)
      if(vals[i] > best) {
        best = vals[i];
        bi = i;
      }
    waveArgmax(best, bi);
    return bi == BIG ? 0 : bi;
  }
  const float logMax = dlog(mx);
  for(int i = v.lane; i < n; i += 64)
    pr[i] = vals[i] <= 0.0f ? 0.0f : dexp((dlog(vals[i]) - logMax) / temperature);
  const float sum = seqSum(pr, n, v.lane);
  const float dd = rng.uni() * sum;
  int chosen = n - 1;
// ... 936 lines not shown
  FinRec* fp = d.fin + g;
  if(fp->pending != 1)
    return;
  const FinRec f = *fp;
  const DTables& T = *Tp;
  const int wave = threadIdx.x >> 6, lane = threadIdx.x & 63;
  GV v(d, T, g);
  __shared__ DBoard boards[MAX_AREA + 1];
  __shared__ float tWin[MAX_AREA + 1], tLoss[MAX_AREA + 1];
  __shared__ int8_t finRun[MAX_AREA];
  __shared__ uint8_t hMask[2 * MAX_AREA];
  __shared__ uint8_t rowTurn[2 * MAX_AREA];
  __shared__ uint8_t tCell[MAX_AREA], tDir[MAX_AREA], tRows[MAX_AREA];
  const int numMoves = f.numMoves, numRows = min(f.numRows, 2 * MAX_AREA);
  const int A = T.A, P = T.P, pb = (A + 7) / 8;
  const TurnRec* tr = v.turns();
  const float finalWin = f.winner == 2 ? 1.0f : (f.winner == 1 ? 0.0f : 0.5f);
  for(int t = threadIdx.x; t < numMoves; t += 64 * ROWS_WAVES) {
    const TurnRec rec = tr[t];
    tWin[t] = rec.whiteWin;
    tLoss[t] = rec.whiteLoss;
    tCell[t] = (uint8_t)rec.cell;
    tDir[t] = (uint8_t)rec.dir;
    tRows[t] = rec.rows;
  }
  __syncthreads();
  if(threadIdx.x == 0) {
    tWin[numMoves] = finalWin;
    tLoss[numMoves] = 1.0f - finalWin;
    DBoard b;
    boardInit(T, b);
    boards[0] = b;
    for(int t = 0; t < numMoves; t++) {
      applyMove(T, b, tCell[t], tDir[t]);
      boards[t + 1] = b;
    }
    int j = 0;
    for(int t = 0; t < numMoves; t++)
      for(int c = 0; c < (int)tRows[t] && j < 2 * MAX_AREA; c++)
        rowTurn[j++] = (uint8_t)t;
    DRng rng{f.rngSeed, f.rngCtr};
    for(int r = 0; r < numRows; r++) {
      bool h = true;
      uint32_t hm = 0;
      for(int i = 0; i < 5; i++) {
        h = h && rng.uni() < 0.98f;
        hm |= (h ? 1u : 0u) << i;
      }
      hMask[r] = (uint8_t)hm;
    }
  }
  __syncthreads();
  const DBoard& fin = boards[numMoves];
  for(int c = threadIdx.x; c < A; c += 64 * ROWS_WAVES)
    finRun[c] = colorAt(fin, c) == 0 ? 0 : (int8_t)maxRun(T, fin, c);
  __syncthreads();
  const float nowF1 = 1.0f / (1.0f + (float)A * 0.176f), nowF2 = 1.0f / (1.0f + (float)A * 0.056f),
              nowF3 = 1.0f / (1.0f + (float)A * 0.016f);
  for(int row = wave; row < numRows; row += ROWS_WAVES) {
    const int t = rowTurn[row];
    const uint32_t hm = hMask[row];
    const size_t r = (size_t)f.rowBase + row;
    const DBoard& b = boards[t];
    const int pla = b.pla, opp = 3 - pla;
    packRowBinWave(T, b, d.rBin + r * NUM_SPATIAL * pb);
    if(lane == 0)
      d.rGlob[r] = (float)T.W;
    const int16_t* p0 = v.turnPol(t);
    const int16_t* p1 = t + 1 < numMoves ? v.turnPol(t + 1) : nullptr;
    int16_t* pol = d.rPol + r * 2 * P;
    for(int p = lane; p < P; p += 64) {
      pol[p] = p0[p];
      pol[P + p] = p1 ? p1[p] : (int16_t)1;
    }
    float gval = 0.0f;
    const int li = lane;
    if(li < 10) {
      const int fi = li >> 1;
      const float nf = fi == 0 ? 0.0f : (fi == 1 ? nowF1 : (fi == 2 ? nowF2 : (fi == 3 ? nowF3 : 1.0f)));
      float win = 0.0f, loss = 0.0f, left = 1.0f;
      for(int i = t; i <= numMoves; i++) {
        float now;
        if(i == numMoves) {
          now = left;
          left = 0.0f;
        } else {
          now = left * nf;
          left = left * (1.0f - nf);
        }
        win = win + now * (pla == 2 ? tWin[i] : tLoss[i]);
        loss = loss + now * (pla == 2 ? tLoss[i] : tWin[i]);
      }
      gval = (li & 1) ? loss : win;
    } else if(li == 22) {
      float sum = 0.0f;
      for(int i = t + 1; i <= numMoves; i++) {
        float prevWL = tWin[i - 1] - tLoss[i - 1], nextWL = tWin[i] - tLoss[i];
        float var = (nextWL - prevWL) * (nextWL - prevWL);
        sum = sum + (float)(i - t) * var;
      }
      gval = sum;
    } else if(li == 25 || li == 26 || li == 27 || li == 33 || li == 63) {
      gval = 1.0f;
    } else if(li == 28) {
      gval = t + 1 < numMoves ? 1.0f : 0.0f;
    } else if(li == 30) {
      gval = tr[t].policySurprise;
    } else if(li == 31) {
      gval = tr[t].policyEntropy;
    } else if(li == 32) {
      gval = tr[t].searchEntropy;
    } else if(li >= 36 && li <= 40) {
      gval = ((hm >> (li - 36)) & 1u) ? 1.0f : 0.0f;
    } else if(li == 41) {
      gval = (float)(f.gameHash0 & 0x3FFFFF);
    } else if(li == 42) {
      gval = (float)((f.gameHash0 >> 22) & 0x3FFFFF);
    } else if(li == 43) {
      gval = (float)((f.gameHash0 >> 44) & 0xFFFFF);
    } else if(li == 44) {
      gval = (float)(f.gameHash1 & 0x3FFFFF);
    } else if(li == 45) {
      gval = (float)((f.gameHash1 >> 22) & 0x3FFFFF);
    } else if(li == 46) {
      gval = (float)((f.gameHash1 >> 44) & 0xFFFFF);
    } else if(li == 51) {
      gval = (float)t;
    } else if(li == 53) {
      gval = (float)f.startTurn;
    } else if(li == 49) {
      gval = f.genEnd != f.genStart ? 1.0f : 0.0f;
    } else if(li == 50) {
      gval = (float)(uint8_t)((uint32_t)f.genEnd - (uint32_t)tr[t].gen);
    } else if(li == 55) {
      gval = (float)f.gameMode;
    } else if(li == 57) {
      gval = pla == 2 ? tr[t].rawWhiteWL : -tr[t].rawWhiteWL;
    } else if(li == 59) {
      gval = tr[t].rawPolicyEntropy;
    } else if(li == 60) {
      gval = (float)tr[t].visits;
    }
    d.rGt[r * 64 + li] = gval;
    int8_t* vt = d.rVal + r * 5 * A;
    const DBoard& b2 = boards[min(t + 2, numMoves)];
    const DBoard& b3 = boards[min(t + 6, numMoves)];
    for(int c = lane; c < A; c += 64) {
      int fc = colorAt(fin, c), c2 = colorAt(b2, c), c3 = colorAt(b3, c);
      vt[c] = fc == pla ? 1 : (fc == opp ? -1 : 0);
      vt[A + c] = 0;
      vt[2 * A + c] = c2 == pla ? 1 : (c2 == opp ? -1 : 0);
      vt[3 * A + c] = c3 == pla ? 1 : (c3 == opp ? -1 : 0);
      vt[4 * A + c] = finRun[c];
    }
    if(lane < 4) {
      int m = lane == 0 ? d.slotBase + g : (lane == 1 ? f.gameNum : (lane == 2 ? t : numMoves));
      d.rMeta[r * 4 + lane] = m;
    }
  }
  __syncthreads();
  if(threadIdx.x == 0)
    fp->pending = 0;
}

template <int NI>
__global__ void __launch_bounds__(64) kCommit(const SearchDev* __restrict__ dp, const DTables* __restrict__ Tp) {
  const SearchDev& d = *dp;
  if((int)blockIdx.x >= *d.commitCount)
    return;
  const int g = d.commitList[blockIdx.x];
  extern __shared__ __attribute__((aligned(16))) char lds[];
  int* posv = reinterpret_cast<int*>(lds);
  float* vals = reinterpret_cast<float*>(posv + MAX_P);
  float* tmp = vals + MAX_P;
  float* tmp2 = tmp + MAX_P;
  int* qtail = reinterpret_cast<int*>(tmp2 + MAX_P);
  uint32_t* liveBits = reinterpret_cast<uint32_t*>(qtail + 4);
  uint16_t* queue = reinterpret_cast<uint16_t*>(liveBits + d.cap / 32);
  __shared__ GameDev s;
  GV v(d, *Tp, g);
  SPROF_INIT();
  [[maybe_unused]] const unsigned long long t0 = SPROF_NOW();
  loadGame(v, s);
  const SP& sp = d.sp;
  const int P = d.P, A = d.A;
  DRng rng{s.rngSeed, s.rngCtr};
  if(s.root.finished) {
    finishGameRecord(v, s, rng, reinterpret_cast<float*>(lds) + 2 * MAX_P);
    s.gamesFinished++;
    s.gameNum++;
    s.sideNext = 0;
    afterGame(v, s, rng, reinterpret_cast<uint16_t*>(lds));
    waveSync();
    storeGame(v, s);
    return;
  }
  const bool side = s.sideMode != 0;
  int n = playSelectionValues<NI>(v, *v.sp, s, 0.0f, true, posv, vals, side ? sp.useLcb != 0 : false);
  if(n <= 0) {
    s.err = ERR_NO_CANDIDATE;
    n = 1;
    posv[0] = 0;
  }
  const float temp = interpolateEarly(v.T, s.root.turn, sp.moveTempHalflife, sp.moveTempEarly, sp.moveTemp);
  int ci = chooseIndex(v, rng, vals, n, temp, tmp);
  waveSync();
  const int chosen = posv[ci];
  const Node& r = v.nodes()[s.rootIdx];
  TurnRec rec;
  valueTargets(r, rec);
  rec.visits = r.visits;
  rec.rootNNWin = r.nnWin;
  rec.rootNNLoss = r.nnLoss;
  rec.targetWeight = s.moveWeight;
  rec.rows = 0;
  rec.gen = (uint8_t)*v.d.modelGen;
  const int t = s.numTurns;
  int16_t* pt = side ? d.sidePol + (size_t)g * P : v.turnPol(t);
  waveSync();
  searchTargets<NI>(v, sp, s, s.rootIdx, v.rootNoised(), true, pt, rec, posv, vals, tmp, tmp2);
  rawStats(v, s.rawWin, s.rawLoss, v.rawPolicy(), rec, tmp);
  const bool recordTree = sp.recordTree != 0 && sp.recordTreeWeight > 0.0f;
  if(side) {
    emitSideRow(v, s, rec, rng, s.root, s.gameNum - 1);
    if(recordTree)
      recordTreePositions<NI>(v, sp, s, rng, -1, -1, r.visits, s.gameNum - 1, posv, vals, tmp, tmp2);
    if(rng.uni() < 0.25f) {
      DBoard b2 = s.root;
      playMoveWave(v.T, b2, chosen % A, chosen / A);
      if(!b2.finished) {
        s.leaf = b2;
        s.phase = PH_SIDEEVAL;
        s.rngCtr = rng.ctr;
        waveSync();
        storeGame(v, s);
        return;
      }
    }
    s.sideNext++;
    afterGame(v, s, rng, reinterpret_cast<uint16_t*>(posv));
    waveSync();
    storeGame(v, s);
    return;
  }
  int forkMove = -1;
  if(sp.sideProb > 0.0f && rng.uni() < sp.sideProb) {
    const int fm = forkingMove(v, rng, v.pol(s.rootIdx), s.root, chosen, posv, vals, tmp);
    forkMove = fm;
    if(fm >= 0) {
      DBoard b2 = s.root;
      playMoveWave(v.T, b2, fm % A, fm / A);
      pushSide(v, s, b2);
    }
  }
  if(recordTree) {
    waveSync();
    recordTreePositions<NI>(v, sp, s, rng, chosen, forkMove, r.visits, s.gameNum, posv, vals, tmp, tmp2);
  }
  rec.cell = (int8_t)(chosen % A);
  rec.dir = (int8_t)(chosen / A);
  for(int i = 0; i < 5; i++)
    rec.pad[i] = 0;
  waveSync();
  if(v.lane == 0)
    v.turns()[t] = rec;
  s.numTurns++;
  [[maybe_unused]] const unsigned long long t1 = SPROF_NOW();
  SPROF_ADD(18, t1 - t0);
  playMoveWave(v.T, s.root, chosen % A, chosen / A);
  s.moves++;
  waveSync();
  if(s.root.finished) {
    [[maybe_unused]] const unsigned long long t3 = SPROF_NOW();
    finishGameRecord(v, s, rng, tmp);
    [[maybe_unused]] const unsigned long long t4 = SPROF_NOW();
    s.gamesFinished++;
    s.gameNum++;
    s.sideNext = 0;
    waveSync();
    afterGame(v, s, rng, reinterpret_cast<uint16_t*>(posv));
    SPROF_ADD(20, t4 - t3);
    SPROF_ADD(21, SPROF_NOW() - t4);
    SPROF_ADD(23, 1);
  } else {
    if(setMoveLimits(v, s, rng, rec.rootWL))
      clearTables(v, s);
    else
      reuseTree(v, s, chosen, liveBits, queue, qtail);
    [[maybe_unused]] const unsigned long long t2 = SPROF_NOW();
    SPROF_ADD(19, t2 - t1);
    SPROF_ADD(22, s.liveCount);
    s.rngCtr = rng.ctr;
    s.phase = PH_ROOTEVAL;
    s.rootK = 0;
  }
  waveSync();
  storeGame(v, s);
  SPROF_ADD(16, 1);
  SPROF_ADD(17, SPROF_NOW() - t0);
  SPROF_FLUSH();
}

constexpr int CP_CH = 32;
constexpr int CP_RESOLVE_WAVES = 4;
template <int NI, bool RESOLVE>
__global__ void __launch_bounds__(1024) kCompact(const SearchDev* __restrict__ dp, const DTables* __restrict__ Tp,
                                                 int accumulate) {
  const SearchDev& d = *dp;
  __shared__ uint32_t wsum[16], wpre[17];
  const int nt = blockDim.x, nw = nt >> 6;
  const int t = threadIdx.x, lane = t & 63, w = t >> 6;
  if constexpr(RESOLVE) {
    __shared__ GameDev rs[CP_RESOLVE_WAVES];
    clearRoundTags(d, t, nt);
    if(w < CP_RESOLVE_WAVES)
      completePending<NI>(d, *Tp, w, CP_RESOLVE_WAVES, rs[w]);
    __syncthreads();
  }
  const int nch = (d.G + 63) >> 6;
  const int cpw = (nch + nw - 1) / nw;
  const int g0 = w * cpw * 64 + lane;
  const int p = *d.nnRR;
  const bool vec = cpw <= CP_CH;
  uint64_t need = 0;
  uint32_t bids[CP_CH];
  if(vec) {
#pragma unroll
    for(int k = 0; k < CP_CH; k++) {
      bids[k] = ~0u;
      if(k < cpw) {
        const int i = g0 + 64 * k;
        const int ic = i < d.G ? i : 0;
        bids[k] = d.nnBid[ic];
        need |= (uint64_t)(i < d.G && d.nnNeed[ic] ? 1u : 0u) << k;
      }
    }
  } else {
    for(int k = 0; k < cpw; k++) {
      const int i = g0 + 64 * k;
      need |= (uint64_t)(i < d.G && d.nnNeed[i] ? 1u : 0u) << k;
    }
  }
  const uint64_t atOrPast = p <= g0 ? ~0ull : (p - g0 > 64 * 63 ? 0ull : ~0ull << ((p - g0 + 63) / 64));
  uint32_t c = ((uint32_t)__popcll(need & atOrPast) << 16) + (uint32_t)__popcll(need & ~atOrPast);
#pragma unroll
  for(int off = 32; off >= 1; off >>= 1)
    c += (uint32_t)__shfl_xor((int)c, off, 64);
  if(lane == 0)
    wsum[w] = c;
  __syncthreads();
  if(t < 64) {
    uint32_t x = t < nw ? wsum[t] : 0u, xi = x;
#pragma unroll
    for(int off = 1; off < 16; off <<= 1) {
      const uint32_t v = (uint32_t)__shfl_up((int)xi, off, 64);
      if(t >= off)
        xi += v;
    }
    if(t < 16)
      wpre[t] = xi - x;
    if(t == 15)
      wpre[16] = xi;
  }
  __syncthreads();
  const uint32_t all = wpre[16], excl = wpre[w];
  const int totalHi = (int)(all >> 16), total = totalHi + (int)(all & 0xFFFFu), cap = d.nnCap;
  int oh = (int)(excl >> 16), ol = totalHi + (int)(excl & 0xFFFFu);
  const uint64_t below = (1ull << lane) - 1ull;
  auto chunk = [&](int k, uint32_t bid) {
    const int i = g0 + 64 * k;
    const bool nd = (need >> k) & 1u;
    const uint64_t b = ballot(nd), ge = ballot(nd && i >= p);
    if(nd) {
      const int pos = i >= p ? oh + __popcll(ge & below) : ol + __popcll(b & ~ge & below);
      const bool in = pos < cap;
      if(in) {
        d.nnIdx[pos] = i;
        if(bid != ~0u)
          atomicMax(&d.cTag[bid], (uint32_t)i + 1u);
      }
      d.nnDefer[i] = in ? 0 : 1;
      if(total > cap && pos == cap - 1)
        *d.nnRR = i + 1 < d.G ? i + 1 : 0;
    } else if(i < d.G) {
      d.nnDefer[i] = 0;
    }
    oh += __popcll(ge);
    ol += __popcll(b & ~ge);
  };
  if(vec) {
#pragma unroll
    for(int k = 0; k < CP_CH; k++)
      if(k < cpw)
        chunk(k, bids[k]);
  } else {
    for(int k = 0; k < cpw; k++) {
      const int i = g0 + 64 * k;
      chunk(k, i < d.G ? d.nnBid[i] : ~0u);
    }
  }
  if(t == nt - 1) {
    const int count = min(total, cap);
    *d.nnCount = count;
    *d.pendCount = 0;
    if(accumulate)
      *d.nnTimedEvals += (unsigned long long)count;
  }
}

__global__ void __launch_bounds__(64) kInit(const SearchDev* __restrict__ dp, const DTables* __restrict__ Tp) {
  const SearchDev& d = *dp;
  const int g = blockIdx.x;
  if(g >= d.G)
    return;
  __shared__ GameDev s;
  GV v(d, *Tp, g);
  for(int i = v.lane; i < (int)(sizeof(GameDev) / 4); i += 64)
    reinterpret_cast<uint32_t*>(&s)[i] = 0;
  waveSync();
  s.svbSel = 0;
  s.gameNum = 0;
  startGame(v, s);
  s.startDelay = d.startStagger > 0
                     ? (int32_t)(mix64(d.seed ^ 0x5a5a5a5a5a5a5a5aULL ^ (uint64_t)(d.slotBase + g)) %
                                 (uint64_t)d.startStagger)
                     : 0;
  waveSync();
  storeGame(v, s);
}

__global__ void kGameTree(const SearchDev* __restrict__ dp, int g, int maxNodes, uint32_t* nodesOut,
                          uint32_t* edgesOut, int32_t* count) {
  const SearchDev& d = *dp;
  if(threadIdx.x != 0)
    return;
  const GameDev& s = d.games[g];
  const Node* NS = d.nodes + (size_t)g * d.cap;
  if(s.rootIdx < 0) {
    *count = 0;
    return;
  }
  int n = 0;
  int head = 0;
  nodesOut[23] = (uint32_t)s.rootIdx;
  n = 1;
  while(head < n && head < maxNodes) {
    const int idx = (int)nodesOut[(size_t)head * 24 + 23];
    const Node& x = NS[idx];
    uint32_t* o = nodesOut + (size_t)head * 24;
    o[0] = x.visits;
    o[1] = f2u(x.weightSum);
    o[2] = f2u(x.weightSqSum);
    o[3] = f2u(x.utilityAvg);
    o[4] = f2u(x.utilitySqAvg);
    o[5] = f2u(x.winLossAvg);
    o[6] = f2u(x.nnWin);
    o[7] = f2u(x.nnLoss);
    o[8] = f2u(x.lastSvbDelta);
    o[9] = f2u(x.lastSvbWeight);
    o[10] = (uint32_t)x.numChildren | ((uint32_t)x.nextPla << 16) | ((uint32_t)x.flags << 24);
    const uint64_t* nk = d.nodeKey + ((size_t)g * d.cap + idx) * 2;
    o[11] = (uint32_t)nk[0];
    o[12] = (uint32_t)(nk[0] >> 32);
    o[13] = (uint32_t)nk[1];
    o[14] = (uint32_t)(nk[1] >> 32);
    uint64_t sk = 0;
    int64_t sd = 0, sw = 0;
    if(x.svbEntry >= 0) {
      size_t e = ((size_t)g * 2 + s.svbSel) * d.svbCap + x.svbEntry;
      sk = d.svbKey[e];
      sd = d.svbD[e];
      sw = d.svbW[e];
    }
    o[15] = (uint32_t)sk;
    o[16] = (uint32_t)(sk >> 32);
    o[17] = (uint32_t)(uint64_t)sd;
    o[18] = (uint32_t)((uint64_t)sd >> 32);
    o[19] = (uint32_t)(uint64_t)sw;
    o[20] = (uint32_t)((uint64_t)sw >> 32);
    o[21] = 0;
    o[22] = 0;
    const NodeEdges E{d.edges + ((size_t)g * d.cap + idx) * INLINE_EDGES,
                      d.edgePool + ((size_t)g * 2 + d.games[g].edgeSel) * d.edgePoolCap + x.edgeBase};
    for(int i = 0; i < x.numChildren; i++) {
      const int c = (int)E[i].child;
      int ci = -1;
      for(int q = 0; q < n; q++)
        if((int)nodesOut[(size_t)q * 24 + 23] == c) {
          ci = q;
          break;
        }
      if(ci < 0 && n < maxNodes) {
        nodesOut[(size_t)n * 24 + 23] = (uint32_t)c;
        ci = n++;
      }
      uint32_t* eo = edgesOut + ((size_t)head * d.P + i) * 3;
      eo[0] = (uint32_t)ci;
      eo[1] = E[i].visits;
      eo[2] = E[i].move;
    }
    head++;
  }
  for(int q = 0; q < n; q++)
    nodesOut[(size_t)q * 24 + 23] = 0;
  *count = n;
}

static int laneItems(int P) { return P <= 128 ? 2 : (P <= 256 ? 4 : 7); }

__global__ void __launch_bounds__(256) kStageRows(const SearchDev* __restrict__ dp, uint8_t* __restrict__ dst,
                                                  int rb) {
  const SearchDev& d = *dp;
  const int A = d.A, P = d.P, pb = (A + 7) / 8;
  const unsigned long long n = *d.rCount;
  const int lane = threadIdx.x & 63;
  const int sz[6] = {NUM_SPATIAL * pb, 4, 4 * P, 256, 5 * A, 16};
  for(unsigned long long r = blockIdx.x * 4ull + (threadIdx.x >> 6); r < n; r += gridDim.x * 4ull) {
    const uint8_t* src[6] = {d.rBin + r * sz[0], reinterpret_cast<const uint8_t*>(d.rGlob + r),
                             reinterpret_cast<const uint8_t*>(d.rPol + r * 2 * P),
                             reinterpret_cast<const uint8_t*>(d.rGt + r * 64), reinterpret_cast<const uint8_t*>((const int8_t*)d.rVal) + r * sz[4],
                             reinterpret_cast<const uint8_t*>(d.rMeta + r * 4)};
    uint8_t* o = dst + r * (unsigned long long)rb;
#pragma unroll
    for(int f = 0; f < 6; f++) {
      for(int i = lane; i < sz[f]; i += 64)
        o[i] = src[f][i];
      o += sz[f];
    }
  }
}

__global__ void kStageDone(const SearchDev* __restrict__ dp, int discardGames) {
  const SearchDev& d = *dp;
  *d.rStaged += *d.rCount;
  *d.rCount = 0;
  if(discardGames)
    *d.gCount = 0;
}

void launchStageRows(const SearchDev& d, const SearchDev* dd, uint8_t* dst, unsigned long long* countOut,
                     bool discardGames, hipStream_t st) {
  hipLaunchKernelGGL(kStageRows, dim3(1024), dim3(256), 0, st, dd, dst, rowBytes(d.A));
  KC_HIP(hipGetLastError());
  KC_HIP(hipMemcpyAsync(countOut, d.rCount, 8, hipMemcpyDeviceToHost, st));
  hipLaunchKernelGGL(kStageDone, dim3(1), dim3(1), 0, st, dd, discardGames ? 1 : 0);
  KC_HIP(hipGetLastError());
}

void launchSelfplayInit(const SearchDev& d, const SearchDev* dd, hipStream_t st) {
  hipLaunchKernelGGL(kInit, dim3(d.G), dim3(64), 0, st, dd, d.T);
  KC_HIP(hipGetLastError());
}

void launchCompact(const SearchDev& d, const SearchDev* dd, hipStream_t st, bool accumulate, bool resolve) {
  const int nt = d.G <= 4 * 64 * CP_CH ? 256 : 1024;
  const DTables* T = d.T;
  const int a = accumulate ? 1 : 0;
  if(!resolve)
    hipLaunchKernelGGL((kCompact<2, false>), dim3(1), dim3(nt), 0, st, dd, T, a);
  else
    switch(laneItems(d.P)) {
      case 2: hipLaunchKernelGGL((kCompact<2, true>), dim3(1), dim3(nt), 0, st, dd, T, a); break;
      case 4: hipLaunchKernelGGL((kCompact<4, true>), dim3(1), dim3(nt), 0, st, dd, T, a); break;
      default: hipLaunchKernelGGL((kCompact<7, true>), dim3(1), dim3(nt), 0, st, dd, T, a); break;
    }
  KC_HIP(hipGetLastError());
}

template <class K, class... Args>
static void launchEv(K kernel, dim3 grid, dim3 block, uint32_t lds, hipStream_t st, hipEvent_t e0, hipEvent_t e1,
                     Args... args) {
  if(e0)
    hipExtLaunchKernelGGL(kernel, grid, block, lds, st, e0, e1, 0, args...);
  else
    hipLaunchKernelGGL(kernel, grid, block, lds, st, args...);
}

void launchSelect(const SearchDev& d, const SearchDev* dd, hipStream_t st, hipEvent_t e0, hipEvent_t e1,
                  bool resetCommit) {
  const DTables* T = d.T;
  const int rc = resetCommit ? 1 : 0;
  switch(laneItems(d.P)) {
    case 2: launchEv(kSelect<2>, dim3(d.G), dim3(64), 0, st, e0, e1, dd, T, rc); break;
    case 4: launchEv(kSelect<4>, dim3(d.G), dim3(64), 0, st, e0, e1, dd, T, rc); break;
    default: launchEv(kSelect<7>, dim3(d.G), dim3(64), 0, st, e0, e1, dd, T, rc); break;
  }
  KC_HIP(hipGetLastError());
}

void launchBackup(const SearchDev& d, const SearchDev* dd, hipStream_t st, hipEvent_t e0, hipEvent_t e1) {
  const DTables* T = d.T;
  switch(laneItems(d.P)) {
    case 2: launchEv(kBackup<2>, dim3(d.G), dim3(64), 0, st, e0, e1, dd, T); break;
    case 4: launchEv(kBackup<4>, dim3(d.G), dim3(64), 0, st, e0, e1, dd, T); break;
    default: launchEv(kBackup<7>, dim3(d.G), dim3(64), 0, st, e0, e1, dd, T); break;
  }
  KC_HIP(hipGetLastError());
}

void launchBackupSelect(const SearchDev& d, const SearchDev* dd, hipStream_t st, hipEvent_t e0, hipEvent_t e1) {
  const DTables* T = d.T;
  switch(laneItems(d.P)) {
    case 2: launchEv(kBackupSelect<2>, dim3(d.G), dim3(64), 0, st, e0, e1, dd, T); break;
    case 4: launchEv(kBackupSelect<4>, dim3(d.G), dim3(64), 0, st, e0, e1, dd, T); break;
    default: launchEv(kBackupSelect<7>, dim3(d.G), dim3(64), 0, st, e0, e1, dd, T); break;
  }
  KC_HIP(hipGetLastError());
}

void launchResolve(const SearchDev& d, const SearchDev* dd, hipStream_t st) {
  const DTables* T = d.T;
  switch(laneItems(d.P)) {
    case 2: hipLaunchKernelGGL(kResolve<2>, dim3(RESOLVE_GRID), dim3(64), 0, st, dd, T); break;
    case 4: hipLaunchKernelGGL(kResolve<4>, dim3(RESOLVE_GRID), dim3(64), 0, st, dd, T); break;
    default: hipLaunchKernelGGL(kResolve<7>, dim3(RESOLVE_GRID), dim3(64), 0, st, dd, T); break;
  }
  KC_HIP(hipGetLastError());
}

void launchCommit(const SearchDev& d, const SearchDev* dd, hipStream_t st) {
  const size_t lds = commitLdsBytes(d.cap);
  switch(laneItems(d.P)) {
    case 2: hipLaunchKernelGGL(kCommit<2>, dim3(d.G), dim3(64), lds, st, dd, d.T); break;
    case 4: hipLaunchKernelGGL(kCommit<4>, dim3(d.G), dim3(64), lds, st, dd, d.T); break;
    default: hipLaunchKernelGGL(kCommit<7>, dim3(d.G), dim3(64), lds, st, dd, d.T); break;
  }
  KC_HIP(hipGetLastError());
  hipLaunchKernelGGL(kRows, dim3(d.G), dim3(64 * ROWS_WAVES), 0, st, dd, d.T);
  KC_HIP(hipGetLastError());
}

void launchGameTree(const SearchDev* dd, int slot, int maxNodes, uint32_t* nodesOut, uint32_t* edgesOut,
                    int32_t* count, hipStream_t st) {
  hipLaunchKernelGGL(kGameTree, dim3(1), dim3(64), 0, st, dd, slot, maxNodes, nodesOut, edgesOut, count);
  KC_HIP(hipGetLastError());
}

}
```

### katacoffee_amd/csrc/selfplay.cpp

```cpp
#include "selfplay.h"

#include <algorithm>
#include <cstring>

namespace kc {

static int nextPow2(int v) {
  int p = 1;
  while(p < v)
    p <<= 1;
  return p;
}

SP toSP(const coffee_search_params& p) {
  SP s;
  s.maxVisits = p.max_visits;
  s.cpuct = p.cpuct_exploration;
  s.cpuctLog = p.cpuct_exploration_log;
  s.cpuctBase = p.cpuct_exploration_base;
  s.fpuRedMax = p.fpu_reduction_max;
  s.rootFpuRedMax = p.root_fpu_reduction_max;
  s.fpuLossProp = p.fpu_loss_prop;
  s.rootFpuLossProp = p.root_fpu_loss_prop;
  s.fpuByVisited = p.fpu_parent_weight_by_visited_policy;
  s.fpuByVisitedPow = p.fpu_parent_weight_by_visited_policy_pow;
  s.valueWeightExp = p.value_weight_exponent;
  s.rootNoise = p.root_noise_enabled;
  s.dirConc = p.root_dirichlet_noise_total_concentration;
  s.dirWeight = p.root_dirichlet_noise_weight;
  s.rootTemp = p.root_policy_temperature;
  s.rootTempEarly = p.root_policy_temperature_early;
  s.rootDesiredCoeff = p.root_desired_per_child_visits_coeff;
  s.rootSyms = p.root_num_symmetries_to_sample;
  s.moveTemp = p.chosen_move_temperature;
  s.moveTempEarly = p.chosen_move_temperature_early;
  s.moveTempHalflife = p.chosen_move_temperature_halflife;
  s.moveSubtract = p.chosen_move_subtract;
  s.movePrune = p.chosen_move_prune;
  s.useLcb = p.use_lcb_for_selection;
  s.lcbStdevs = p.lcb_stdevs;
  s.minVisitPropLcb = p.min_visit_prop_for_lcb;
  s.svbFactor = p.subtree_value_bias_factor;
  s.svbExp = p.subtree_value_bias_weight_exponent;
  s.svbFreeProp = p.subtree_value_bias_free_prop;
  s.useGraph = p.use_graph_search;
  s.cheapProb = p.cheap_search_prob;
  s.cheapVisits = p.cheap_search_visits;
  s.cheapWeight = p.cheap_search_target_weight;
  s.reduceVisits = p.reduce_visits;
  s.reduceThreshold = p.reduce_visits_threshold;
  s.reduceLookback = p.reduce_visits_threshold_lookback;
  s.reducedMin = p.reduced_visits_min;
  s.reducedWeight = p.reduced_visits_weight;
  s.policySurpriseWeight = p.policy_surprise_data_weight;
  s.valueSurpriseWeight = p.value_surprise_data_weight;
  s.initPolicy = p.init_games_with_policy;
  s.initAreaProp = p.policy_init_area_prop;
  s.initTemp = p.policy_init_area_temperature;
  s.earlyForkProb = p.early_fork_game_prob;
  s.earlyForkMoveProp = p.early_fork_game_expected_move_prop;
  s.forkProb = p.fork_game_prob;
  s.forkMinChoices = p.fork_game_min_choices;
  s.earlyForkMaxChoices = p.early_fork_game_max_choices;
  s.forkMaxChoices = p.fork_game_max_choices;
  s.sideProb = p.side_position_prob;
  s.recordTree = p.record_tree_positions;
  s.recordTreeThreshold = p.record_tree_threshold;
  s.recordTreeWeight = p.record_tree_target_weight;
  return s;
}

int rowBytes(int A) {
  const int pb = (A + 7) / 8;
  return NUM_SPATIAL * pb + 4 + 2 * 4 * A * 2 + 64 * 4 + 5 * A + 16;
}

size_t commitLdsBytes(int cap) {
  size_t b = (size_t)MAX_P * 4 * 4 + 16;
  b += (size_t)(cap / 32) * 4 + (size_t)cap * 2;
  return (b + 15) / 16 * 16;
}

template <class T>
static T* devAlloc(std::vector<void*>& owned, size_t count, bool zero = true) {
  void* p = nullptr;
  size_t bytes = std::max<size_t>(count * sizeof(T), 16);
  KC_HIP(hipMalloc(&p, bytes));
  owned.push_back(p);
  if(zero)
    KC_HIP(hipMemset(p, 0, bytes));
  return reinterpret_cast<T*>(p);
}

SelfplayEngine::SelfplayEngine(const coffee_selfplay_config& c) {
  if(c.num_games <= 0)
    throw std::invalid_argument("num_games must be positive");
  if(c.num_games > 65535)
    throw std::invalid_argument("num_games must be <= 65535 per device");
  const coffee_search_params& sp = c.search;
  if(sp.max_visits < 1 || sp.root_num_symmetries_to_sample < 1 || sp.root_num_symmetries_to_sample > 4)
    throw std::invalid_argument("search params: max_visits >= 1 and 1 <= root_num_symmetries_to_sample <= 4");
  if(sp.cheap_search_prob > 0.0f && (sp.cheap_search_visits <= 0 || sp.cheap_search_visits > sp.max_visits))
    throw std::invalid_argument("cheap_search_visits must be in [1, max_visits]");
  if(sp.reduce_visits && (sp.reduced_visits_min <= 0 || sp.reduced_visits_min > sp.max_visits))
    throw std::invalid_argument("reduced_visits_min must be in [1, max_visits]");
  if(sp.reduce_visits && (sp.reduce_visits_threshold < 0.0f || sp.reduce_visits_threshold >= 1.0f ||
                          sp.reduce_visits_threshold_lookback < 1 || sp.reduce_visits_threshold_lookback > 100))
    throw std::invalid_argument("reduce_visits_threshold must be in [0, 1) and lookback in [1, 100]");
  auto unit = [](float x) { return x >= 0.0f && x <= 1.0f; };
  if(!unit(sp.cheap_search_prob) || !unit(sp.cheap_search_target_weight) || !unit(sp.reduced_visits_weight) ||
     !unit(sp.policy_surprise_data_weight) || !unit(sp.value_surprise_data_weight) ||
     sp.policy_surprise_data_weight + sp.value_surprise_data_weight > 1.0f)
    throw std::invalid_argument("play settings: probabilities and weights in [0, 1], surprise weights sum <= 1");
  if(sp.init_games_with_policy && (!unit(sp.policy_init_area_prop) || sp.policy_init_area_temperature < 0.1f ||
                                   sp.policy_init_area_temperature > 5.0f))
    throw std::invalid_argument("policy_init_area_prop in [0, 1], policy_init_area_temperature in [0.1, 5]");
  if(sp.early_fork_game_prob < 0.0f || sp.early_fork_game_prob > 0.5f || sp.fork_game_prob < 0.0f ||
     sp.fork_game_prob > 0.5f || !unit(sp.early_fork_game_expected_move_prop) || sp.fork_game_min_choices < 1 ||
     sp.early_fork_game_max_choices < sp.fork_game_min_choices || sp.fork_game_max_choices < sp.fork_game_min_choices ||
     sp.early_fork_game_max_choices > MAX_FORK_CHOICES || sp.fork_game_max_choices > MAX_FORK_CHOICES)
    throw std::invalid_argument("fork settings: probabilities in [0, 0.5], min <= max choices <= 100");
  if(!unit(sp.side_position_prob))
    throw std::invalid_argument("side_position_prob must be in [0, 1]");
  if(sp.record_tree_positions && sp.record_tree_target_weight > 1.0f)
    throw std::invalid_argument("record_tree_target_weight > 1");
  const DTables& ht = hostTables(c.x, c.y, c.win_len);
  T_ = deviceTables(c.x, c.y, c.win_len);
  commitInterval_ = c.commit_interval > 0 ? c.commit_interval : 8;
  int cap = c.node_cap > 0 ? c.node_cap : std::max(2048, 3 * sp.max_visits);
  cap = (cap + 63) / 64 * 64;
  if(cap > 65535)
    throw std::invalid_argument("node_cap must be <= 65535");
  if(cap < sp.max_visits + 4)
    throw std::invalid_argument("node_cap must exceed max_visits + 3");
  const int G = c.num_games, P = ht.P, A = ht.A;
  const int ttCap = nextPow2(2 * cap);
  const int rowCap = c.row_capacity > 0 ? c.row_capacity : 4 * G * A;
  if(!c.use_fake_net) {
    if(!c.model_path)
      throw std::invalid_argument("model_path required unless use_fake_net");
    model_.reset(new ModelHost(loadModel(c.model_path)));
    nn_.reset(new NNEngine(*model_, c.x, c.y, c.win_len, c.nn_precision));
  }
  nnPath_ = c.nn_precision;
  xLen_ = c.x;
  yLen_ = c.y;
  winLen_ = c.win_len;
  SearchDev& d = hd_;
  memset(&d, 0, sizeof(d));
  d.T = T_;
  d.sp = toSP(sp);
  d.spCheap = cheapSearchSP(d.sp);
  d.G = G;
  d.cap = cap;
  d.ttCap = ttCap;
  d.svbCap = ttCap;
  d.P = P;
  d.A = A;
  d.inWords = ht.inWords;
  d.maxTurns = A + 1;
  d.rowCap = rowCap;
  d.slotBase = c.slot_base;
  if(c.start_stagger < 0)
    throw std::invalid_argument("start_stagger must be >= 0");
  d.startStagger = c.start_stagger;
  d.seed = c.seed;
  d.games = devAlloc<GameDev>(owned_, G);
  d.nodes = devAlloc<Node>(owned_, (size_t)G * cap, false);
  d.edges = devAlloc<Edge>(owned_, (size_t)G * cap * INLINE_EDGES, false);
  d.edgePoolCap = edgePoolCapFor(cap, P);
  d.edgePool = devAlloc<Edge>(owned_, (size_t)G * 2 * d.edgePoolCap, false);
  d.policy = devAlloc<float>(owned_, (size_t)G * cap * P, false);
  d.nodeKey = devAlloc<uint64_t>(owned_, (size_t)G * cap * 2, false);
  d.freeList = devAlloc<uint32_t>(owned_, (size_t)G * cap, false);
  d.allocBits = devAlloc<uint32_t>(owned_, (size_t)G * (cap / 32));
  d.ttKey = devAlloc<uint64_t>(owned_, (size_t)G * ttCap * 2, false);
  d.ttNode = devAlloc<int32_t>(owned_, (size_t)G * ttCap, false);
  d.svbKey = devAlloc<uint64_t>(owned_, (size_t)G * 2 * ttCap);
  d.svbD = devAlloc<int64_t>(owned_, (size_t)G * 2 * ttCap);
  d.svbW = devAlloc<int64_t>(owned_, (size_t)G * 2 * ttCap);
  d.accPolicy = devAlloc<float>(owned_, (size_t)G * P);
  d.rawPolicy = devAlloc<float>(owned_, (size_t)G * P);
  d.rootNoised = devAlloc<float>(owned_, (size_t)G * P);
  d.pathNode = devAlloc<int32_t>(owned_, (size_t)G * MAX_DEPTH);
  d.pathSlot = devAlloc<int32_t>(owned_, (size_t)G * MAX_DEPTH);
  d.turns = devAlloc<TurnRec>(owned_, (size_t)G * d.maxTurns);
  d.turnPol = devAlloc<int16_t>(owned_, (size_t)G * d.maxTurns * P);
  d.nnIn = devAlloc<uint64_t>(owned_, (size_t)G * ht.inWords);
  d.nnOut = devAlloc<float>(owned_, (size_t)G * (P + 4));
  d.fin = devAlloc<FinRec>(owned_, G);
  d.fork = devAlloc<ForkRec>(owned_, G);
  d.side = devAlloc<DBoard>(owned_, (size_t)G * MAX_SIDE);
  d.sidePol = devAlloc<int16_t>(owned_, (size_t)G * P);
  d.commitList = devAlloc<int32_t>(owned_, G);
  d.nnTimedEvals = devAlloc<unsigned long long>(owned_, 1);
  d.commitCount = devAlloc<int32_t>(owned_, 1);
  const int pb = (A + 7) / 8;
  d.rBin = devAlloc<uint8_t>(owned_, (size_t)rowCap * NUM_SPATIAL * pb, false);
  d.rGlob = devAlloc<float>(owned_, (size_t)rowCap, false);
  d.rPol = devAlloc<int16_t>(owned_, (size_t)rowCap * 2 * P, false);
  d.rGt = devAlloc<float>(owned_, (size_t)rowCap * 64, false);
  d.rVal = devAlloc<int8_t>(owned_, (size_t)rowCap * 5 * A, false);
  d.rMeta = devAlloc<int32_t>(owned_, (size_t)rowCap * 4, false);
  d.rCount = devAlloc<unsigned long long>(owned_, 1);
  d.rDropped = devAlloc<unsigned long long>(owned_, 1);
  d.rStaged = devAlloc<unsigned long long>(owned_, 1);
  d.nnNeed = devAlloc<int32_t>(owned_, G);
  d.nnDefer = devAlloc<int32_t>(owned_, G);
  d.nnBid = devAlloc<uint32_t>(owned_, G);
  d.nnRR = devAlloc<int32_t>(owned_, 1);
  if(c.nn_batch_cap < 0)
    throw std::invalid_argument("nn_batch_cap must be >= 0");
  if(c.engines_per_device < 0)
    throw std::invalid_argument("engines_per_device must be >= 0");
  userCap_ = c.nn_batch_cap;
  enginesPerDevice_ = std::max(1, c.engines_per_device);
  {
    int dev = 0;
    KC_HIP(hipGetDevice(&dev));
    KC_HIP(hipDeviceGetAttribute(&cus_, hipDeviceAttributeMultiprocessorCount, dev));
    cus_ = std::max(1, cus_);
  }
  d.nnCap = nnCapFor(G);
  d.nnIdx = devAlloc<int32_t>(owned_, G);
  d.modelGen = devAlloc<int32_t>(owned_, 1);
  d.nnCount = devAlloc<int32_t>(owned_, 1);
  if(c.nn_cache_log2 < 0 || c.nn_cache_log2 > 26)
    throw std::invalid_argument("nn_cache_log2 must be in 0..26");
  d.cacheOn = c.nn_cache_log2 > 0 ? 1 : 0;
  {
    const size_t entries = d.cacheOn ? (size_t)1 << c.nn_cache_log2 : 1;
    d.cacheMask = (uint32_t)(entries - 1);
    d.cKey = devAlloc<uint64_t>(owned_, entries * 2);
    d.cPol = devAlloc<float>(owned_, entries * P, false);
    d.cVal = devAlloc<float>(owned_, entries * 2, false);
    d.cTag = devAlloc<uint32_t>(owned_, entries);
  }
  d.cClear = devAlloc<uint32_t>(owned_, G);
  d.pendList = devAlloc<int32_t>(owned_, G, false);
  d.pendCount = devAlloc<int32_t>(owned_, 1);
  {
    const char* f = getenv("COFFEE_FUSED_ROUNDS");
    fuseRounds_ = f && f[0] == '0' ? 0 : (f && f[0] == '1' ? 1 : -1);
    const char* r = getenv("COFFEE_SEPARATE_RESOLVE");
    resolveInCompact_ = !(r && r[0] == '1');
  }
  {
    const char* e = getenv("COFFEE_NN_AUDIT_EVERY");
    if(e)
      auditEvery_ = std::max(0, atoi(e));
    const char* t = getenv("COFFEE_NN_AUDIT_TOL");
    if(t)
      auditTol_ = (float)atof(t);
  }
  auditOut_ = devAlloc<float>(owned_, (size_t)G * (P + 4), false);
  auditMax_ = devAlloc<unsigned>(owned_, 1);
  d.gCap = 2 * G;
  d.gRec = devAlloc<GameRec>(owned_, (size_t)d.gCap, false);
  d.gCount = devAlloc<unsigned long long>(owned_, 1);
  d.gDropped = devAlloc<unsigned long long>(owned_, 1);
  dd_ = devAlloc<SearchDev>(owned_, 1);
  KC_HIP(hipMemcpy(dd_, &d, sizeof(SearchDev), hipMemcpyHostToDevice));
  KC_HIP(hipStreamCreateWithFlags(&stream_, hipStreamNonBlocking));
  const size_t lds = commitLdsBytes(cap);
  if(lds > 64 * 1024)
    throw std::invalid_argument("node_cap too large for the commit kernel's LDS");
  launchSelfplayInit(d, dd_, stream_);
  KC_HIP(hipStreamSynchronize(stream_));
}

SelfplayEngine::~SelfplayEngine() {
  if(stream_)
    (void)hipStreamSynchronize(stream_);
  for(const PendingTiming& p : pending_) {
    (void)hipEventDestroy(p.a);
    (void)hipEventDestroy(p.b);
  }
  for(hipEvent_t e : evPool_)
    (void)hipEventDestroy(e);
  nn_.reset();
  for(void* p : owned_)
    (void)hipFree(p);
  if(stream_)
    (void)hipStreamDestroy(stream_);
}

hipEvent_t SelfplayEngine::takeEvent() {
  if(evPool_.empty()) {
    hipEvent_t e;
    KC_HIP(hipEventCreate(&e));
    return e;
  }
  hipEvent_t e = evPool_.back();
  evPool_.pop_back();
  return e;
}

void SelfplayEngine::timed(int which, hipStream_t st, const std::function<void()>& f, bool on) {
  if(!on) {
    f();
    return;
  }
  hipEvent_t a = takeEvent(), b = takeEvent();
  KC_HIP(hipEventRecord(a, st));
  f();
  KC_HIP(hipEventRecord(b, st));
  pending_.push_back({which, a, b});
}

void SelfplayEngine::timedKernel(int which, bool on, const std::function<void(hipEvent_t, hipEvent_t)>& f) {
  if(!on) {
    f(nullptr, nullptr);
    return;
  }
  hipEvent_t a = takeEvent(), b = takeEvent();
  f(a, b);
  pending_.push_back({which, a, b});
}

void SelfplayEngine::resolveTiming() {
  for(const PendingTiming& p : pending_) {
    KC_HIP(hipEventSynchronize(p.b));
    float ms = 0.0f;
    KC_HIP(hipEventElapsedTime(&ms, p.a, p.b));
    kernelMs_[p.which] += ms;
    kernelLaunches_[p.which]++;
    evPool_.push_back(p.a);
    evPool_.push_back(p.b);
  }
  pending_.clear();
}

bool SelfplayEngine::fuseNow() const {
  if(fuseRounds_ >= 0)
    return fuseRounds_ == 1;
  return !nn_ || (nn_->fused() && nn_->precision() == NN_FAST);
}

void SelfplayEngine::step(int rounds, hipStream_t st) {
  if(!st)
    st = stream_;
  const SearchDev& d = hd_;
  const bool fuse = fuseNow();
  bool selected = false;
  for(int r = 0; r < rounds; r++) {
    const bool t1 = sampleNow(1);
    if(selected) {
      if(!resolveInCompact_)
        launchResolve(d, dd_, st);
    } else {
      const bool t0 = sampleNow(0);
      timedKernel(0, t0, [&](hipEvent_t a, hipEvent_t b) { launchSelect(d, dd_, st, a, b, commitReset_); });
    }
    commitReset_ = false;
    launchCompact(d, dd_, st, t1, selected && resolveInCompact_);
    timedKernel(1, t1, [&](hipEvent_t a, hipEvent_t b) {
      const int rows = std::min(d.G, d.nnCap);
      if(nn_) {
        nn_->forward(rows, d.nnIn, d.nnOut, st, d.nnCount, d.nnIdx, a, b);
      } else {
        if(a)
          KC_HIP(hipEventRecord(a, st));
        launchFakeNet(T_, rows, d.nnIn, d.nnOut, st, d.nnCount, d.nnIdx);
        if(b)
          KC_HIP(hipEventRecord(b, st));
      }
    });
    if(nn_ && nnPath_ == NN_DEFAULT && auditEvery_ > 0 && nn_->precision() == NN_CORRECTED &&
       nnLaunches_++ % (uint64_t)auditEvery_ == 0) {
      nn_->audit(std::min(d.G, d.nnCap), d.nnIn, d.nnOut, auditOut_, auditMax_, st, d.nnCount, d.nnIdx);
      audits_++;
    }
    const bool commitNow = (rounds_ + 1) % (uint64_t)commitInterval_ == 0 || r == rounds - 1;
    if(fuse && !commitNow) {
      const bool t4 = sampleNow(4);
      timedKernel(4, t4, [&](hipEvent_t a, hipEvent_t b) { launchBackupSelect(d, dd_, st, a, b); });
      selected = true;
    } else {
      const bool t2 = sampleNow(2);
      timedKernel(2, t2, [&](hipEvent_t a, hipEvent_t b) { launchBackup(d, dd_, st, a, b); });
      selected = false;
    }
    rounds_++;
    if(commitNow) {
      const bool t3 = sampleNow(3);
      timed(3, st, [&] { launchCommit(d, dd_, st); }, t3);
      commitReset_ = true;
    }
  }
}

void SelfplayEngine::sync() {
  KC_HIP(hipStreamSynchronize(stream_));
  resolveTiming();
  auditCheck();
}

void SelfplayEngine::auditCheck() {
  if(!nn_ || audits_ == 0)
    return;
  unsigned bits = 0;
  KC_HIP(hipMemcpy(&bits, auditMax_, 4, hipMemcpyDeviceToHost));
  float m;
  memcpy(&m, &bits, 4);
  auditSeen_ = std::max(auditSeen_, m);
  if(!(auditSeen_ <= auditTol_) && nn_->precision() == NN_CORRECTED && nnPath_ == NN_DEFAULT) {
    nn_.reset(new NNEngine(*model_, xLen_, yLen_, winLen_, NN_ACCURATE));
    auditSwitches_++;
    const int cap = nnCapFor(hd_.G);
    if(cap != hd_.nnCap) {
      hd_.nnCap = cap;
      KC_HIP(hipMemcpy(&dd_->nnCap, &cap, sizeof(int), hipMemcpyHostToDevice));
    }
    if(hd_.cacheOn)
      KC_HIP(hipMemsetAsync(hd_.cKey, 0, sizeof(uint64_t) * 2 * ((size_t)hd_.cacheMask + 1), stream_));
    KC_HIP(hipStreamSynchronize(stream_));
  }
}

void SelfplayEngine::stats(coffee_selfplay_stats& out) {
  sync();
  std::vector<GameDev> g(hd_.G);
  KC_HIP(hipMemcpy(g.data(), hd_.games, sizeof(GameDev) * hd_.G, hipMemcpyDeviceToHost));
  memset(&out, 0, sizeof(out));
  out.rounds = rounds_;
  for(const GameDev& x : g) {
    out.playouts += x.playouts;
    out.nn_evals += x.nnEvals;
    out.moves += x.moves;
    out.games_finished += x.gamesFinished;
    out.errors += x.err != 0 ? 1 : 0;
    out.errors_node_pool += x.err == ERR_NODE_POOL ? 1 : 0;
    out.errors_edge_pool += x.err == ERR_EDGE_POOL ? 1 : 0;
    out.edge_pool_peak = std::max<uint64_t>(out.edge_pool_peak, (uint64_t)x.edgePeak);
    out.tree_levels += x.treeLevels;
    out.tree_children += x.treeChildren;
  }
  unsigned long long cnt = 0, dropped = 0;
  KC_HIP(hipMemcpy(&cnt, hd_.rCount, 8, hipMemcpyDeviceToHost));
  KC_HIP(hipMemcpy(&dropped, hd_.rDropped, 8, hipMemcpyDeviceToHost));
  unsigned long long staged = 0;
  KC_HIP(hipMemcpy(&staged, hd_.rStaged, 8, hipMemcpyDeviceToHost));
  out.rows_pending = cnt;
  out.rows_written = rowsDrained_ + staged + cnt;
  out.rows_dropped = dropped;
  unsigned long long gdrop = 0;
  KC_HIP(hipMemcpy(&gdrop, hd_.gDropped, 8, hipMemcpyDeviceToHost));
  out.games_dropped = gdrop;
  out.edge_pool_cap = (uint64_t)hd_.edgePoolCap;
  out.nn_precision = nn_ ? (uint64_t)nn_->precision() : 0;
  out.nn_audits = audits_;
  out.nn_audit_switches = (uint64_t)auditSwitches_;
  out.nn_audit_max_diff = auditSeen_;
  if(out.errors)
    throw InternalError("self-play device invariant violated in " + std::to_string(out.errors) +
                        " game slot(s): " + std::to_string(out.errors_node_pool) + " node pool exhausted, " +
                        std::to_string(out.errors_edge_pool) + " edge pool exhausted, " +
                        std::to_string(out.errors - out.errors_node_pool - out.errors_edge_pool) +
                        " without a move candidate (raise node_cap)");
}

int SelfplayEngine::drain(int maxRows, uint8_t* bin, float* glob, int16_t* pol, float* gt, int8_t* val,
                          int32_t* meta) {
  sync();
  unsigned long long cnt = 0;
  KC_HIP(hipMemcpy(&cnt, hd_.rCount, 8, hipMemcpyDeviceToHost));
  const int n = (int)std::min<unsigned long long>(cnt, (unsigned long long)std::max(maxRows, 0));
  const int A = hd_.A, P = hd_.P, pb = (A + 7) / 8;
  auto cp = [&](void* dst, const void* src, size_t rowBytes) {
    if(dst && n > 0)
      KC_HIP(hipMemcpy(dst, src, rowBytes * n, hipMemcpyDeviceToHost));
  };
  cp(bin, hd_.rBin, (size_t)NUM_SPATIAL * pb);
  cp(glob, hd_.rGlob, 4);
  cp(pol, hd_.rPol, (size_t)2 * P * 2);
  cp(gt, hd_.rGt, 64 * 4);
  cp(val, hd_.rVal, (size_t)5 * A);
  cp(meta, hd_.rMeta, 16);
  if(n > 0 && (unsigned long long)n < cnt) {
    const size_t rest = cnt - n;
    auto mv = [&](void* base, size_t rowBytes) {
      for(size_t off = 0; off < rest; off += (size_t)n) {
        const size_t k = std::min(rest - off, (size_t)n);
        KC_HIP(hipMemcpy((char*)base + rowBytes * off, (char*)base + rowBytes * (n + off), rowBytes * k,
                         hipMemcpyDeviceToDevice));
      }
    };
    mv(hd_.rBin, (size_t)NUM_SPATIAL * pb);
    mv(hd_.rGlob, 4);
    mv(hd_.rPol, (size_t)2 * P * 2);
    mv(hd_.rGt, 256);
    mv(hd_.rVal, (size_t)5 * A);
    mv(hd_.rMeta, 16);
  }
  unsigned long long left = cnt - (unsigned long long)n;
  KC_HIP(hipMemcpy(hd_.rCount, &left, 8, hipMemcpyHostToDevice));
  rowsDrained_ += n;
  return n;
}

void SelfplayEngine::stageRows(uint8_t* dst, int maxRows, unsigned long long* countOut, bool discardGames) {
  if(maxRows < hd_.rowCap)
    throw std::invalid_argument("stage_rows: the destination must hold the row capacity (" +
                                std::to_string(hd_.rowCap) + " rows)");
  launchStageRows(hd_, dd_, dst, countOut, discardGames, stream_);
  size_t keep = 0;
  for(size_t i = 0; i < pending_.size(); i++) {
    const PendingTiming& p = pending_[i];
    if(hipEventQuery(p.b) == hipSuccess) {
      float ms = 0.0f;
      KC_HIP(hipEventElapsedTime(&ms, p.a, p.b));
      kernelMs_[p.which] += ms;
      kernelLaunches_[p.which]++;
      evPool_.push_back(p.a);
      evPool_.push_back(p.b);
    } else {
      pending_[keep++] = p;
    }
  }
  pending_.resize(keep);
}

int SelfplayEngine::drainGames(int maxGames, int32_t* header, uint8_t* moves) {
  sync();
  unsigned long long cnt = 0;
  KC_HIP(hipMemcpy(&cnt, hd_.gCount, 8, hipMemcpyDeviceToHost));
  const int n = (int)std::min<unsigned long long>(cnt, (unsigned long long)std::max(maxGames, 0));
  if(n > 0) {
    std::vector<GameRec> recs(n);
    KC_HIP(hipMemcpy(recs.data(), hd_.gRec, sizeof(GameRec) * n, hipMemcpyDeviceToHost));
    const int A = hd_.A;
    for(int i = 0; i < n; i++) {
      const GameRec& r = recs[i];
      if(header) {
        header[4 * i + 0] = r.slot;
        header[4 * i + 1] = r.gameNum;
        header[4 * i + 2] = r.numMoves;
        header[4 * i + 3] = r.winner;
      }
      if(moves)
        for(int t = 0; t < A; t++) {
          moves[((size_t)i * A + t) * 2 + 0] = t < r.numMoves ? r.cell[t] : 0xFF;
          moves[((size_t)i * A + t) * 2 + 1] = t < r.numMoves ? r.dir[t] : 0xFF;
        }
    }
    const size_t rest = cnt - n;
    for(size_t off = 0; off < rest; off += (size_t)n) {
      const size_t k = std::min(rest - off, (size_t)n);
      KC_HIP(hipMemcpy(hd_.gRec + off, hd_.gRec + n + off, sizeof(GameRec) * k, hipMemcpyDeviceToDevice));
    }
  }
  unsigned long long left = cnt - (unsigned long long)n;
  KC_HIP(hipMemcpy(hd_.gCount, &left, 8, hipMemcpyHostToDevice));
  return n;
}

int SelfplayEngine::nnCapFor(int G) const {
  if(userCap_ > 0)
    return userCap_;
  if(!nn_)
    return std::min(G, cus_ * NN_BOARDS_PER_WG);
  if(!nn_->fused())
    return G;
  return std::min(G, nn_->batchCap(cus_, enginesPerDevice_));
}

void SelfplayEngine::setModel(const char* path) {
  if(!nn_)
    throw std::invalid_argument("engine runs the stand-in network (use_fake_net)");
  switchModel(loadModel(path));
}

void SelfplayEngine::setModelBytes(const void* data, size_t bytes) {
  if(!nn_)
    throw std::invalid_argument("engine runs the stand-in network (use_fake_net)");
  switchModel(loadModelBytes(data, bytes, "<model bytes>"));
}

void SelfplayEngine::switchModel(const ModelHost& m) {
  std::unique_ptr<NNEngine> next(new NNEngine(m, xLen_, yLen_, winLen_, nnPath_));
  std::unique_ptr<ModelHost> keep(new ModelHost(m));
  sync();
  nn_ = std::move(next);
  model_ = std::move(keep);
  auditSeen_ = 0.0f;
  KC_HIP(hipMemset(auditMax_, 0, 4));
  const int cap = nnCapFor(hd_.G);
  if(cap != hd_.nnCap) {
    hd_.nnCap = cap;
    KC_HIP(hipMemcpy(&dd_->nnCap, &cap, sizeof(int), hipMemcpyHostToDevice));
  }
  modelGen_++;
  KC_HIP(hipMemcpy(hd_.modelGen, &modelGen_, sizeof(int32_t), hipMemcpyHostToDevice));
  if(hd_.cacheOn)
    KC_HIP(hipMemsetAsync(hd_.cKey, 0, sizeof(uint64_t) * 2 * ((size_t)hd_.cacheMask + 1), stream_));
}

void SelfplayEngine::gameInfo(int slot, int64_t* info) {
  if(slot < 0 || slot >= hd_.G)
    throw std::invalid_argument("slot out of range");
  sync();
  GameDev g;
  KC_HIP(hipMemcpy(&g, hd_.games + slot, sizeof(GameDev), hipMemcpyDeviceToHost));
  int64_t v[16] = {g.phase, g.rootK, g.liveCount, g.rootIdx, g.gameNum, g.root.turn, g.root.pla,
                   g.root.finished, g.root.winner, (int64_t)g.playouts, (int64_t)g.nnEvals, (int64_t)g.moves,
                   (int64_t)g.gamesFinished, g.root.lastCell, g.root.lastDir, (int64_t)g.rngCtr};
  memcpy(info, v, sizeof(v));
}

int SelfplayEngine::gameTree(int slot, int maxNodes, uint32_t* nodes, uint32_t* edges) {
  if(slot < 0 || slot >= hd_.G || maxNodes <= 0)
    throw std::invalid_argument("slot/max_nodes out of range");
  sync();
  std::vector<void*> tmp;
  uint32_t* dn = devAlloc<uint32_t>(tmp, (size_t)maxNodes * 24, false);
  uint32_t* de = devAlloc<uint32_t>(tmp, (size_t)maxNodes * hd_.P * 3, false);
  int32_t* dc = devAlloc<int32_t>(tmp, 1, false);
  KC_HIP(hipMemsetAsync(dn, 0, (size_t)maxNodes * 24 * 4, stream_));
  KC_HIP(hipMemsetAsync(de, 0, (size_t)maxNodes * hd_.P * 3 * 4, stream_));
  KC_HIP(hipMemsetAsync(dc, 0, 4, stream_));
  launchGameTree(dd_, slot, maxNodes, dn, de, dc, stream_);
  KC_HIP(hipStreamSynchronize(stream_));
  int n = 0;
  KC_HIP(hipMemcpy(&n, dc, 4, hipMemcpyDeviceToHost));
  if(nodes)
    KC_HIP(hipMemcpy(nodes, dn, (size_t)maxNodes * 24 * 4, hipMemcpyDeviceToHost));
  if(edges)
    KC_HIP(hipMemcpy(edges, de, (size_t)maxNodes * hd_.P * 3 * 4, hipMemcpyDeviceToHost));
  for(void* p : tmp)
    (void)hipFree(p);
  return n;
}

void SelfplayEngine::rootPolicy(int slot, float* out) {
  if(slot < 0 || slot >= hd_.G)
    throw std::invalid_argument("slot out of range");
  sync();
  KC_HIP(hipMemcpy(out, hd_.rootNoised + (size_t)slot * hd_.P, sizeof(float) * hd_.P, hipMemcpyDeviceToHost));
}

uint64_t SelfplayEngine::timedNNEvals() {
  sync();
  unsigned long long v = 0;
  KC_HIP(hipMemcpy(&v, hd_.nnTimedEvals, 8, hipMemcpyDeviceToHost));
  return v;
}

void SelfplayEngine::kernelTime(int which, double& ms, uint64_t& launches) {
  resolveTiming();
  if(which < 0 || which > 4)
    throw std::invalid_argument("which must be 0..4");
  ms = kernelMs_[which];
  launches = kernelLaunches_[which];
}

}
```

### katacoffee_amd/csrc/selfplay.h

```cpp
#pragma once
#include <functional>
#include <memory>
#include <vector>

#include "../../include/katacoffee.h"
#include "engine.h"
#include "search.h"

namespace kc {

SP toSP(const coffee_search_params& p);

class SelfplayEngine {
 public:
  explicit SelfplayEngine(const coffee_selfplay_config& c);
  ~SelfplayEngine();
  void step(int rounds, hipStream_t st);
  void sync();
  void stats(coffee_selfplay_stats& out);
  int drain(int maxRows, uint8_t* bin, float* glob, int16_t* pol, float* gt, int8_t* val, int32_t* meta);
  int drainGames(int maxGames, int32_t* header, uint8_t* moves);
  void stageRows(uint8_t* dst, int maxRows, unsigned long long* countOut, bool discardGames);
  hipStream_t stream() const { return stream_; }
  void setModel(const char* path);
  void setModelBytes(const void* data, size_t bytes);
  void gameInfo(int slot, int64_t* info);
  int gameTree(int slot, int maxNodes, uint32_t* nodes, uint32_t* edges);
  void rootPolicy(int slot, float* out);
  void setTiming(int every) { timingEvery_ = every > 0 ? every : 0; }
  void kernelTime(int which, double& ms, uint64_t& launches);
  uint64_t timedNNEvals();
  const SearchDev& dev() const { return hd_; }
  bool nnFused() const { return nn_ && nn_->fused(); }

 private:
  struct PendingTiming {
    int which;
    hipEvent_t a, b;
  };
  void switchModel(const ModelHost& m);
  void timed(int which, hipStream_t st, const std::function<void()>& f, bool on);
  void timedKernel(int which, bool on, const std::function<void(hipEvent_t, hipEvent_t)>& f);
  bool sampleNow(int which) { return timingEvery_ > 0 && groupLaunches_[which]++ % (uint64_t)timingEvery_ == 0; }
  hipEvent_t takeEvent();
  void resolveTiming();
  std::vector<PendingTiming> pending_;
  std::vector<hipEvent_t> evPool_;
  const DTables* T_ = nullptr;
  std::unique_ptr<NNEngine> nn_;
  SearchDev hd_;
  SearchDev* dd_ = nullptr;
  std::vector<void*> owned_;
  hipStream_t stream_ = nullptr;
  int commitInterval_ = 8;
  int xLen_ = 0, yLen_ = 0, winLen_ = 0;
  int nnPath_ = 0;
  int userCap_ = 0;
  int enginesPerDevice_ = 1;
  int cus_ = 1;
  int nnCapFor(int G) const;
  int32_t modelGen_ = 0;
  uint64_t rounds_ = 0;
  bool commitReset_ = false;
  uint64_t rowsDrained_ = 0;
  int timingEvery_ = 0;
  uint64_t groupLaunches_[5] = {0, 0, 0, 0, 0};
  double kernelMs_[5] = {0, 0, 0, 0, 0};
  uint64_t kernelLaunches_[5] = {0, 0, 0, 0, 0};
  int fuseRounds_ = -1;
  bool fuseNow() const;
  bool resolveInCompact_ = true;
  void auditCheck();
  std::unique_ptr<ModelHost> model_;
  float* auditOut_ = nullptr;
  unsigned* auditMax_ = nullptr;
  int auditEvery_ = 128;
  float auditTol_ = NNEngine::NN_AUTO_TOL;
  uint64_t nnLaunches_ = 0;
  uint64_t audits_ = 0;
  float auditSeen_ = 0.0f;
  int auditSwitches_ = 0;
};

}
```

Baseline: 28010.

## Replace pending-leaf resolve pass with round-stamped cache bids resolved in select

Cache tags now carry a round stamp plus the winning game, and bidders publish their leaf key and symmetry in double-buffered per-game slots. A later game hitting a slot claimed in the same round reads the winner's NN output directly in select instead of being queued for a separate resolve step inside compact. This removes the pending list, the tag-clearing pass, and the resolve work in the single-block compact kernel, and makes the round-robin pointer double-buffered. The cost is 64-bit tags, extra key publishing, a debug counter atomic, and reliance on the host-side round value staying consistent with what the kernels see.

```diff
diff --git a/include/katacoffee.h b/include/katacoffee.h
--- a/include/katacoffee.h
+++ b/include/katacoffee.h
@@ -185,6 +185,8 @@
 int coffee_selfplay_kernel_time(coffee_selfplay* h, int which, double* ms, uint64_t* launches);
 int coffee_selfplay_timed_nn_evals(coffee_selfplay* h, uint64_t* evals);
 
+int coffee_debug_selfplay_counters(coffee_selfplay* h, uint64_t* out);
+
 #ifdef __cplusplus
 }
 #endif
diff --git a/katacoffee_amd/__init__.py b/katacoffee_amd/__init__.py
--- a/katacoffee_amd/__init__.py
+++ b/katacoffee_amd/__init__.py
@@ -100,7 +100,7 @@
     "coffee_selfplay_destroy", "coffee_selfplay_game_info",
     "coffee_selfplay_game_tree", "coffee_selfplay_root_policy", "coffee_debug_cdf_table", "coffee_debug_zobrist",
     "coffee_selfplay_enable_timing", "coffee_selfplay_kernel_time", "coffee_selfplay_timed_nn_evals",
-    "coffee_write_npz",
+    "coffee_write_npz", "coffee_debug_selfplay_counters",
 ]
 
 
@@ -154,6 +154,8 @@
         L.coffee_selfplay_enable_timing.argtypes = [c_p, c_i]
         L.coffee_selfplay_kernel_time.argtypes = [c_p, c_i, c_p, c_p]
         L.coffee_selfplay_timed_nn_evals.argtypes = [c_p, c_p]
+        if hasattr(L, "coffee_debug_selfplay_counters"):
+            L.coffee_debug_selfplay_counters.argtypes = [c_p, c_p]
         L.coffee_debug_cdf_table.argtypes = [c_i, c_i, c_i, c_p]
         L.coffee_debug_zobrist.argtypes = [c_i, c_i, c_i] + [c_p] * 5
         L.coffee_write_npz.argtypes = [ctypes.c_char_p, c_i, c_i, c_i] + [c_p] * 5
@@ -482,6 +484,12 @@
         check(lib().coffee_selfplay_timed_nn_evals(self.h, ctypes.byref(n)))
         return n.value
 
+    def debug_counters(self):
+        out = np.zeros(4, np.uint64)
+        check(lib().coffee_debug_selfplay_counters(self.h, _ptr(out)))
+        keys = ["same_round_key_equal", "same_round_key_different", "deferred_now", "round_robin"]
+        return dict(zip(keys, out.tolist()))
+
     def kernel_time(self, which):
         ms = ctypes.c_double()
         n = ctypes.c_uint64()
diff --git a/katacoffee_amd/csrc/capi.cpp b/katacoffee_amd/csrc/capi.cpp
--- a/katacoffee_amd/csrc/capi.cpp
+++ b/katacoffee_amd/csrc/capi.cpp
@@ -489,6 +489,16 @@
   });
 }
 
+int coffee_debug_selfplay_counters(coffee_selfplay* h, uint64_t* out) {
+  return guarded([&] {
+    need(h && h->eng && out, "NULL argument");
+    unsigned long long v[4];
+    h->eng->debugCounters(v);
+    for(int i = 0; i < 4; i++)
+      out[i] = v[i];
+  });
+}
+
 int coffee_selfplay_kernel_time(coffee_selfplay* h, int which, double* ms, uint64_t* launches) {
   return guarded([&] {
     need(h && h->eng && ms && launches, "NULL argument");
diff --git a/katacoffee_amd/csrc/search.h b/katacoffee_amd/csrc/search.h
--- a/katacoffee_amd/csrc/search.h
+++ b/katacoffee_amd/csrc/search.h
@@ -25,13 +25,16 @@
   LEAF_CACHED = 6,
   LEAF_INIT = 7,
   LEAF_FORK = 8,
-  LEAF_SIDE = 9,
-  LEAF_PENDING = 10
+  LEAF_SIDE = 9
 };
 
 KC_HD uint32_t cacheSlot(uint64_t k0, uint64_t k1, uint32_t mask) {
   const uint64_t h = k0 ^ ((k1 << 29) | (k1 >> 35));
   return (uint32_t)(h ^ (h >> 32)) & mask;
+}
+constexpr int BID_GAME_BITS = 20;
+KC_HD unsigned long long bidStamp(uint64_t round, int g) {
+  return ((unsigned long long)round << BID_GAME_BITS) | (unsigned long long)(g + 1);
 }
 enum Phase { PH_ROOTEVAL = 0, PH_SEARCH = 1, PH_COMMIT = 2, PH_INIT = 3, PH_FORK = 4, PH_SIDEEVAL = 5 };
 
@@ -239,10 +242,11 @@
   DPtr<uint64_t> cKey;
   DPtr<float> cPol;
   DPtr<float> cVal;
-  DPtr<uint32_t> cTag;
-  DPtr<uint32_t> cClear;
-  DPtr<int32_t> pendList;
-  DPtr<int32_t> pendCount;
+  DPtr<unsigned long long> cTag;
+  DPtr<uint64_t> bidKey;
+  DPtr<int32_t> bidSym;
+  DPtr<unsigned long long> sameRound;
+  uint64_t round;
   DPtr<FinRec> fin;
   DPtr<ForkRec> fork;
   DPtr<DBoard> side;
@@ -275,7 +279,6 @@
                   hipEvent_t e1 = nullptr);
 void launchBackupSelect(const SearchDev& d, const SearchDev* dd, hipStream_t st, hipEvent_t e0 = nullptr,
                         hipEvent_t e1 = nullptr);
-void launchResolve(const SearchDev& d, const SearchDev* dd, hipStream_t st);
 void launchCommit(const SearchDev& d, const SearchDev* dd, hipStream_t st);
 void launchGameTree(const SearchDev* dd, int slot, int maxNodes, uint32_t* nodesOut, uint32_t* edgesOut,
                     int32_t* count, hipStream_t st);
diff --git a/katacoffee_amd/csrc/search.hip b/katacoffee_amd/csrc/search.hip
--- a/katacoffee_amd/csrc/search.hip
+++ b/katacoffee_amd/csrc/search.hip
@@ -1023,7 +1023,11 @@
 
 
 template <int NI>
-KC_D void cacheLookup(const GV& v, GameDev& s, bool fused) {
+KC_D void postprocess(const GV& v, const DBoard& b, int sym, const float* out, float* polDst, float& whiteWin,
+                      float& whiteLoss, float* stage, float (&pv)[NI]);
+
+template <int NI>
+KC_D void cacheLookup(const GV& v, GameDev& s, bool fused, uint64_t round, float* stage) {
   const SearchDev& d = v.d;
   const uint64_t k0 = v.nodeKey(s.leafNode)[0], k1 = v.nodeKey(s.leafNode)[1];
   const uint32_t slot = cacheSlot(k0, k1, d.cacheMask);
@@ -1036,12 +1040,21 @@
     pv[j] = pos < P ? cp[pos] : 0.0f;
   }
   const float cw = d.cVal[2 * (size_t)slot], cl = d.cVal[2 * (size_t)slot + 1];
-  const uint32_t tag = fused ? d.cTag[slot] : 0u;
+  const unsigned long long tag = fused ? d.cTag[slot] : 0ull;
   s.cSlot = (int32_t)slot;
-  if(tag != 0u) {
-    s.leafKind = LEAF_PENDING;
+  if(tag != 0ull && (tag >> BID_GAME_BITS) == round) {
+    const int wg = (int)(tag & ((1ull << BID_GAME_BITS) - 1ull)) - 1;
+    const size_t pub = (size_t)(round & 1u) * d.G + wg;
+    const bool same = d.bidKey[2 * pub] == k0 && d.bidKey[2 * pub + 1] == k1;
     if(v.lane == 0)
-      d.pendList[atomicAdd(d.pendCount, 1)] = v.g;
+      atomicAdd(&d.sameRound[same ? 0 : 1], 1ull);
+    if(same) {
+      s.leafKind = LEAF_CACHED;
+      float w, l;
+      postprocess<NI>(v, s.leaf, d.bidSym[pub], d.nnOut + (size_t)wg * (P + 4), v.pol(s.leafNode), w, l, stage, pv);
+      s.cHitWin = w;
+      s.cHitLoss = l;
+    }
     return;
   }
   if(d.cKey[2 * (size_t)slot] == k0 && d.cKey[2 * (size_t)slot + 1] == k1) {
@@ -1058,7 +1071,7 @@
   }
 }
 
-KC_D void finishSelect(const GV& v, GameDev& s, DRng& rng) {
+KC_D void finishSelect(const GV& v, GameDev& s, DRng& rng, uint64_t round) {
   const SearchDev& d = v.d;
   const int g = v.g;
   if(s.leafKind == LEAF_NN)
@@ -1069,8 +1082,16 @@
       s.leafKind == LEAF_SIDE;
   if(v.lane == 0) {
     d.nnNeed[g] = needNN ? 1 : 0;
-    if(needNN)
-      d.nnBid[g] = s.leafKind == LEAF_NN && d.cacheOn ? (uint32_t)s.cSlot : ~0u;
+    if(needNN) {
+      const bool bids = s.leafKind == LEAF_NN && d.cacheOn;
+      d.nnBid[g] = bids ? (uint32_t)s.cSlot : ~0u;
+      if(bids) {
+        const size_t pub = (size_t)(round & 1u) * d.G + g;
+        d.bidKey[2 * pub] = v.nodeKey(s.leafNode)[0];
+        d.bidKey[2 * pub + 1] = v.nodeKey(s.leafNode)[1];
+        d.bidSym[pub] = s.leafSym;
+      }
+    }
   }
   if(needNN) {
     const int slot = g;
@@ -1084,13 +1105,20 @@
 
 template <int NI>
 KC_D void selectBody(const SearchDev& d, const DTables& T, int g, GameDev& s, bool loaded, bool fused,
-                     uint32_t* hasBits, float* rootPol) {
+                     uint32_t* hasBits, float* rootPol, uint64_t round) {
   GV v(d, T, g);
   SPROF_INIT();
   const unsigned long long t0 = SPROF_NOW();
   if(d.nnDefer[g]) {
-    if(v.lane == 0)
+    if(v.lane == 0) {
       d.nnNeed[g] = 1;
+      if(d.cacheOn) {
+        const size_t from = (size_t)((round + 1u) & 1u) * d.G + g, to = (size_t)(round & 1u) * d.G + g;
+        d.bidKey[2 * to] = d.bidKey[2 * from];
+        d.bidKey[2 * to + 1] = d.bidKey[2 * from + 1];
+        d.bidSym[to] = d.bidSym[from];
+      }
+    }
     return;
   }
   if(loaded)
@@ -1150,11 +1178,11 @@
   } else {
     descend<NI>(v, s, hasBits, rootPol);
     if(s.leafKind == LEAF_NN && d.cacheOn)
-      cacheLookup<NI>(v, s, fused);
+      cacheLookup<NI>(v, s, fused, round - 1u, rootPol);
   }
   const unsigned long long t2 = SPROF_NOW();
   (void)t2;
-  finishSelect(v, s, rng);
+  finishSelect(v, s, rng, round);
   SPROF_ADD(0, 1);
   SPROF_MAX(24, SPROF_NOW() - t0);
   SPROF_MAX(25, s.pathLen);
@@ -1168,7 +1196,7 @@
 
 template <int NI>
 __global__ void __launch_bounds__(64, NI <= 2 ? 4 : 2) kSelect(const SearchDev* __restrict__ dp, const DTables* __restrict__ Tp,
-                                                                int resetCommit) {
+                                                                int resetCommit, uint64_t round) {
   const SearchDev& d = *dp;
   const int g = blockIdx.x;
   if(resetCommit && g == 0 && threadIdx.x == 0)
@@ -1178,38 +1206,7 @@
   __shared__ uint32_t hasBits[(MAX_P + 31) / 32];
   __shared__ GameDev s;
   __shared__ float rootPol[MAX_P];
-  selectBody<NI>(d, *Tp, g, s, false, false, hasBits, rootPol);
-}
-
-constexpr int RESOLVE_GRID = 64;
-KC_D void clearRoundTags(const SearchDev& d, int first, int stride) {
-  for(int i = first; i < d.G; i += stride) {
-    const uint32_t cc = d.cClear[i];
-    if(cc != 0u) {
-      d.cTag[cc - 1u] = 0u;
-      d.cClear[i] = 0u;
-    }
-  }
-}
-template <int NI>
-KC_D void completePending(const SearchDev& d, const DTables& T, int first, int stride, GameDev& s) {
-  const int np = *d.pendCount;
-  for(int k = first; k < np; k += stride) {
-    const int g = __builtin_amdgcn_readfirstlane(d.pendList[k]);
-    GV v(d, T, g);
-    loadGame(v, s);
-    s.leafKind = LEAF_NN;
-    cacheLookup<NI>(v, s, false);
-    DRng rng = DRng{s.rngSeed, s.rngCtr};
-    finishSelect(v, s, rng);
-  }
-}
-template <int NI>
-__global__ void __launch_bounds__(64) kResolve(const SearchDev* __restrict__ dp, const DTables* __restrict__ Tp) {
-  const SearchDev& d = *dp;
-  clearRoundTags(d, blockIdx.x * 64 + laneId(), RESOLVE_GRID * 64);
-  __shared__ GameDev s;
-  completePending<NI>(d, *Tp, blockIdx.x, RESOLVE_GRID, s);
+  selectBody<NI>(d, *Tp, g, s, false, false, hasBits, rootPol, round);
 }
 
 template <int NI>
@@ -1471,7 +1468,8 @@
 }
 
 template <int NI>
-KC_D bool backupBody(const SearchDev& d, const DTables& T, int g, GameDev& s, bool fused, float* scratch) {
+KC_D bool backupBody(const SearchDev& d, const DTables& T, int g, GameDev& s, bool fused, float* scratch,
+                     uint64_t round) {
   if(d.nnDefer[g])
     return false;
   GV v(d, T, g);
@@ -1572,7 +1570,7 @@
         postprocess<NI>(v, s.leaf, s.leafSym, o, pol, w, l, scratch, pv);
         if(d.cacheOn) {
           const uint32_t slot = (uint32_t)s.cSlot;
-          if(d.cTag[slot] == (uint32_t)g + 1u) {
+          if(d.cTag[slot] == bidStamp(round, g)) {
             float* cp = d.cPol + (size_t)slot * P;
 #pragma unroll
             for(int j = 0; j < NI; j++)
@@ -1583,10 +1581,6 @@
               d.cVal[2 * (size_t)slot + 1] = l;
               d.cKey[2 * (size_t)slot] = v.nodeKey(s.leafNode)[0];
               d.cKey[2 * (size_t)slot + 1] = v.nodeKey(s.leafNode)[1];
-              if(fused)
-                d.cClear[g] = slot + 1u;
-              else
-                d.cTag[slot] = 0;
             }
           }
         }
@@ -1641,14 +1635,15 @@
 }
 
 template <int NI>
-__global__ void __launch_bounds__(64, NI <= 4 ? 4 : 3) kBackup(const SearchDev* __restrict__ dp, const DTables* __restrict__ Tp) {
+__global__ void __launch_bounds__(64, NI <= 4 ? 4 : 3) kBackup(const SearchDev* __restrict__ dp, const DTables* __restrict__ Tp,
+                                                                          uint64_t round) {
   const SearchDev& d = *dp;
   const int g = blockIdx.x;
   if(g >= d.G)
     return;
   __shared__ __attribute__((aligned(16))) float scratch[3 * MAX_P];
   __shared__ GameDev s;
-  backupBody<NI>(d, *Tp, g, s, false, scratch);
+  backupBody<NI>(d, *Tp, g, s, false, scratch, round);
 }
 
 #ifndef KC_FUSED_OCC
@@ -1659,7 +1654,8 @@
 #endif
 template <int NI>
 __global__ void __launch_bounds__(64, NI <= 2 ? KC_FUSED_OCC : 2) kBackupSelect(const SearchDev* __restrict__ dp,
-                                                                      const DTables* __restrict__ Tp) {
+                                                                      const DTables* __restrict__ Tp,
+                                                                      uint64_t round) {
   const SearchDev& d = *dp;
   const int g = blockIdx.x;
   if(g >= d.G)
@@ -1669,8 +1665,8 @@
   __shared__ __attribute__((aligned(16))) float scratch[3 * MAX_P];
   __shared__ uint32_t hasBits[(MAX_P + 31) / 32];
   __shared__ GameDev s;
-  const bool loaded = backupBody<NI>(d, *Tp, g, s, true, scratch);
-  selectBody<NI>(d, *Tp, g, s, loaded, true, hasBits, scratch);
+  const bool loaded = backupBody<NI>(d, *Tp, g, s, true, scratch, round);
+  selectBody<NI>(d, *Tp, g, s, loaded, true, hasBits, scratch, round + 1u);
 }
 
 #ifdef KC_SEARCH_PROFILE
@@ -3213,25 +3209,16 @@
 }
 
 constexpr int CP_CH = 32;
-constexpr int CP_RESOLVE_WAVES = 4;
-template <int NI, bool RESOLVE>
-__global__ void __launch_bounds__(1024) kCompact(const SearchDev* __restrict__ dp, const DTables* __restrict__ Tp,
-                                                 int accumulate) {
+__global__ void __launch_bounds__(1024) kCompact(const SearchDev* __restrict__ dp, int accumulate, uint64_t round) {
   const SearchDev& d = *dp;
   __shared__ uint32_t wsum[16], wpre[17];
   const int nt = blockDim.x, nw = nt >> 6;
   const int t = threadIdx.x, lane = t & 63, w = t >> 6;
-  if constexpr(RESOLVE) {
-    __shared__ GameDev rs[CP_RESOLVE_WAVES];
-    clearRoundTags(d, t, nt);
-    if(w < CP_RESOLVE_WAVES)
-      completePending<NI>(d, *Tp, w, CP_RESOLVE_WAVES, rs[w]);
-    __syncthreads();
-  }
   const int nch = (d.G + 63) >> 6;
   const int cpw = (nch + nw - 1) / nw;
   const int g0 = w * cpw * 64 + lane;
-  const int p = *d.nnRR;
+  const int p = d.nnRR[round & 1u];
+  int32_t* rrNext = d.nnRR + ((round + 1u) & 1u);
   const bool vec = cpw <= CP_CH;
   uint64_t need = 0;
   uint32_t bids[CP_CH];
@@ -3288,11 +3275,11 @@
       if(in) {
         d.nnIdx[pos] = i;
         if(bid != ~0u)
-          atomicMax(&d.cTag[bid], (uint32_t)i + 1u);
+          atomicMax(&d.cTag[bid], bidStamp(round, i));
       }
       d.nnDefer[i] = in ? 0 : 1;
       if(total > cap && pos == cap - 1)
-        *d.nnRR = i + 1 < d.G ? i + 1 : 0;
+        *rrNext = i + 1 < d.G ? i + 1 : 0;
     } else if(i < d.G) {
       d.nnDefer[i] = 0;
     }
@@ -3313,7 +3300,8 @@
   if(t == nt - 1) {
     const int count = min(total, cap);
     *d.nnCount = count;
-    *d.pendCount = 0;
+    if(total <= cap)
+      *rrNext = p;
     if(accumulate)
       *d.nnTimedEvals += (unsigned long long)count;
   }
@@ -3463,18 +3451,9 @@
   KC_HIP(hipGetLastError());
 }
 
-void launchCompact(const SearchDev& d, const SearchDev* dd, hipStream_t st, bool accumulate, bool resolve) {
+void launchCompact(const SearchDev& d, const SearchDev* dd, hipStream_t st, bool accumulate, bool) {
   const int nt = d.G <= 4 * 64 * CP_CH ? 256 : 1024;
-  const DTables* T = d.T;
-  const int a = accumulate ? 1 : 0;
-  if(!resolve)
-    hipLaunchKernelGGL((kCompact<2, false>), dim3(1), dim3(nt), 0, st, dd, T, a);
-  else
-    switch(laneItems(d.P)) {
-      case 2: hipLaunchKernelGGL((kCompact<2, true>), dim3(1), dim3(nt), 0, st, dd, T, a); break;
-      case 4: hipLaunchKernelGGL((kCompact<4, true>), dim3(1), dim3(nt), 0, st, dd, T, a); break;
-      default: hipLaunchKernelGGL((kCompact<7, true>), dim3(1), dim3(nt), 0, st, dd, T, a); break;
-    }
+  hipLaunchKernelGGL(kCompact, dim3(1), dim3(nt), 0, st, dd, accumulate ? 1 : 0, d.round);
   KC_HIP(hipGetLastError());
 }
 
@@ -3492,9 +3471,9 @@
   const DTables* T = d.T;
   const int rc = resetCommit ? 1 : 0;
   switch(laneItems(d.P)) {
-    case 2: launchEv(kSelect<2>, dim3(d.G), dim3(64), 0, st, e0, e1, dd, T, rc); break;
-    case 4: launchEv(kSelect<4>, dim3(d.G), dim3(64), 0, st, e0, e1, dd, T, rc); break;
-    default: launchEv(kSelect<7>, dim3(d.G), dim3(64), 0, st, e0, e1, dd, T, rc); break;
+    case 2: launchEv(kSelect<2>, dim3(d.G), dim3(64), 0, st, e0, e1, dd, T, rc, d.round); break;
+    case 4: launchEv(kSelect<4>, dim3(d.G), dim3(64), 0, st, e0, e1, dd, T, rc, d.round); break;
+    default: launchEv(kSelect<7>, dim3(d.G), dim3(64), 0, st, e0, e1, dd, T, rc, d.round); break;
   }
   KC_HIP(hipGetLastError());
 }
@@ -3502,9 +3481,9 @@
 void launchBackup(const SearchDev& d, const SearchDev* dd, hipStream_t st, hipEvent_t e0, hipEvent_t e1) {
   const DTables* T = d.T;
   switch(laneItems(d.P)) {
-    case 2: launchEv(kBackup<2>, dim3(d.G), dim3(64), 0, st, e0, e1, dd, T); break;
-    case 4: launchEv(kBackup<4>, dim3(d.G), dim3(64), 0, st, e0, e1, dd, T); break;
-    default: launchEv(kBackup<7>, dim3(d.G), dim3(64), 0, st, e0, e1, dd, T); break;
+    case 2: launchEv(kBackup<2>, dim3(d.G), dim3(64), 0, st, e0, e1, dd, T, d.round); break;
+    case 4: launchEv(kBackup<4>, dim3(d.G), dim3(64), 0, st, e0, e1, dd, T, d.round); break;
+    default: launchEv(kBackup<7>, dim3(d.G), dim3(64), 0, st, e0, e1, dd, T, d.round); break;
   }
   KC_HIP(hipGetLastError());
 }
@@ -3512,19 +3491,9 @@
 void launchBackupSelect(const SearchDev& d, const SearchDev* dd, hipStream_t st, hipEvent_t e0, hipEvent_t e1) {
   const DTables* T = d.T;
   switch(laneItems(d.P)) {
-    case 2: launchEv(kBackupSelect<2>, dim3(d.G), dim3(64), 0, st, e0, e1, dd, T); break;
-    case 4: launchEv(kBackupSelect<4>, dim3(d.G), dim3(64), 0, st, e0, e1, dd, T); break;
-    default: launchEv(kBackupSelect<7>, dim3(d.G), dim3(64), 0, st, e0, e1, dd, T); break;
-  }
-  KC_HIP(hipGetLastError());
-}
-
-void launchResolve(const SearchDev& d, const SearchDev* dd, hipStream_t st) {
-  const DTables* T = d.T;
-  switch(laneItems(d.P)) {
-    case 2: hipLaunchKernelGGL(kResolve<2>, dim3(RESOLVE_GRID), dim3(64), 0, st, dd, T); break;
-    case 4: hipLaunchKernelGGL(kResolve<4>, dim3(RESOLVE_GRID), dim3(64), 0, st, dd, T); break;
-    default: hipLaunchKernelGGL(kResolve<7>, dim3(RESOLVE_GRID), dim3(64), 0, st, dd, T); break;
+    case 2: launchEv(kBackupSelect<2>, dim3(d.G), dim3(64), 0, st, e0, e1, dd, T, d.round); break;
+    case 4: launchEv(kBackupSelect<4>, dim3(d.G), dim3(64), 0, st, e0, e1, dd, T, d.round); break;
+    default: launchEv(kBackupSelect<7>, dim3(d.G), dim3(64), 0, st, e0, e1, dd, T, d.round); break;
   }
   KC_HIP(hipGetLastError());
 }
diff --git a/katacoffee_amd/csrc/selfplay.cpp b/katacoffee_amd/csrc/selfplay.cpp
--- a/katacoffee_amd/csrc/selfplay.cpp
+++ b/katacoffee_amd/csrc/selfplay.cpp
@@ -208,7 +208,7 @@
   d.nnNeed = devAlloc<int32_t>(owned_, G);
   d.nnDefer = devAlloc<int32_t>(owned_, G);
   d.nnBid = devAlloc<uint32_t>(owned_, G);
-  d.nnRR = devAlloc<int32_t>(owned_, 1);
+  d.nnRR = devAlloc<int32_t>(owned_, 2);
   if(c.nn_batch_cap < 0)
     throw std::invalid_argument("nn_batch_cap must be >= 0");
   if(c.engines_per_device < 0)
@@ -234,16 +234,14 @@
     d.cKey = devAlloc<uint64_t>(owned_, entries * 2);
     d.cPol = devAlloc<float>(owned_, entries * P, false);
     d.cVal = devAlloc<float>(owned_, entries * 2, false);
-    d.cTag = devAlloc<uint32_t>(owned_, entries);
-  }
-  d.cClear = devAlloc<uint32_t>(owned_, G);
-  d.pendList = devAlloc<int32_t>(owned_, G, false);
-  d.pendCount = devAlloc<int32_t>(owned_, 1);
+    d.cTag = devAlloc<unsigned long long>(owned_, entries);
+  }
+  d.bidKey = devAlloc<uint64_t>(owned_, (size_t)2 * G * 2);
+  d.bidSym = devAlloc<int32_t>(owned_, (size_t)2 * G);
+  d.sameRound = devAlloc<unsigned long long>(owned_, 2);
   {
     const char* f = getenv("COFFEE_FUSED_ROUNDS");
     fuseRounds_ = f && f[0] == '0' ? 0 : (f && f[0] == '1' ? 1 : -1);
-    const char* r = getenv("COFFEE_SEPARATE_RESOLVE");
-    resolveInCompact_ = !(r && r[0] == '1');
   }
   {
     const char* e = getenv("COFFEE_NN_AUDIT_EVERY");
@@ -344,16 +342,14 @@
   const bool fuse = fuseNow();
   bool selected = false;
   for(int r = 0; r < rounds; r++) {
+    hd_.round = rounds_;
     const bool t1 = sampleNow(1);
-    if(selected) {
-      if(!resolveInCompact_)
-        launchResolve(d, dd_, st);
-    } else {
+    if(!selected) {
       const bool t0 = sampleNow(0);
       timedKernel(0, t0, [&](hipEvent_t a, hipEvent_t b) { launchSelect(d, dd_, st, a, b, commitReset_); });
     }
     commitReset_ = false;
-    launchCompact(d, dd_, st, t1, selected && resolveInCompact_);
+    launchCompact(d, dd_, st, t1, false);
     timedKernel(1, t1, [&](hipEvent_t a, hipEvent_t b) {
       const int rows = std::min(d.G, d.nnCap);
       if(nn_) {
@@ -584,7 +580,7 @@
   nn_ = std::move(next);
   model_ = std::move(keep);
   auditSeen_ = 0.0f;
-  KC_HIP(hipMemset(auditMax_, 0, 4));
+  KC_HIP(hipMemsetAsync(auditMax_, 0, 4, stream_));
   const int cap = nnCapFor(hd_.G);
   if(cap != hd_.nnCap) {
     hd_.nnCap = cap;
@@ -646,6 +642,19 @@
   return v;
 }
 
+void SelfplayEngine::debugCounters(unsigned long long out[4]) {
+  sync();
+  KC_HIP(hipMemcpy(out, hd_.sameRound, 16, hipMemcpyDeviceToHost));
+  std::vector<int32_t> defer(hd_.G);
+  KC_HIP(hipMemcpy(defer.data(), hd_.nnDefer, sizeof(int32_t) * hd_.G, hipMemcpyDeviceToHost));
+  out[2] = 0;
+  for(int32_t x : defer)
+    out[2] += x != 0 ? 1 : 0;
+  int32_t rr = 0;
+  KC_HIP(hipMemcpy(&rr, hd_.nnRR + (rounds_ & 1u), sizeof(int32_t), hipMemcpyDeviceToHost));
+  out[3] = (unsigned long long)rr;
+}
+
 void SelfplayEngine::kernelTime(int which, double& ms, uint64_t& launches) {
   resolveTiming();
   if(which < 0 || which > 4)
diff --git a/katacoffee_amd/csrc/selfplay.h b/katacoffee_amd/csrc/selfplay.h
--- a/katacoffee_amd/csrc/selfplay.h
+++ b/katacoffee_amd/csrc/selfplay.h
@@ -31,6 +31,7 @@
   void kernelTime(int which, double& ms, uint64_t& launches);
   uint64_t timedNNEvals();
   const SearchDev& dev() const { return hd_; }
+  void debugCounters(unsigned long long out[4]);
   bool nnFused() const { return nn_ && nn_->fused(); }
 
  private:
@@ -69,7 +70,6 @@
   uint64_t kernelLaunches_[5] = {0, 0, 0, 0, 0};
   int fuseRounds_ = -1;
   bool fuseNow() const;
-  bool resolveInCompact_ = true;
   void auditCheck();
   std::unique_ptr<ModelHost> model_;
   float* auditOut_ = nullptr;
```

New measurement: 28270 (median of 3 runs). No clear change (+0.9%).
